# SitaoLuan/ACM-GNN

Measured on AMD Instinct MI355X. Metric: edges/sec ACM-GCN fwd+bwd on twitch-gamer, higher is better.
Workload: dtype f32; 1 GPU; twitch-gamer-shaped Chung-Lu graph: 168114 nodes, 6797557 undirected edges, nnz(A_low)=13763228, F_in=7, hidden=64, classes=2; 2-layer acmgcnp (variant=0, structure_info=0, attention LayerNorm on), dropout 0.1 (counter-based, masks regenerated in the kernels), AdamW (fused); step = fwd + NLL loss + bwd + optimizer update; parallelism=single-gpu, node_order=degree, launch=hipGraph replay of the captured step (1 consecutive steps per graph), operator_form=pattern-only P + row scale (shared by A_low and A_low^T), full=False, input_pipeline=True, checked=False

## Files before the change

acm_gnn_amd/_lib.py:

```python
import ctypes as C
import os
import threading

from . import build as _build

c_f32p = C.POINTER(C.c_float)
c_i32p = C.POINTER(C.c_int32)

ACM_OK = 0
STATUS_NAMES = {1: "ACM_EINVAL", 2: "ACM_ESHAPE", 3: "ACM_EHIP", 4: "ACM_EUNSUPPORTED", 5: "ACM_ENOMEM"}
ABI_VERSION = 28

EXPORTED_SYMBOLS = (
    "acm_version", "acm_last_error", "acm_tuning_get", "acm_tuning_set", "acm_csr_create", "acm_csr_transpose", "acm_csr_slice_rows",
    "acm_csr_destroy", "acm_csr_info", "acm_csr_build_streams", "acm_csr_build_item_streams", "acm_spmm_workspace_bytes", "acm_gemm_workspace_bytes",
    "acm_gemm", "acm_gemm_blocks", "acm_gemm_drop", "acm_proj3", "acm_gemm_split", "acm_proj_fwd", "acm_proj_fwd_at", "acm_proj_bwd_workspace_bytes", "acm_proj_bwd", "acm_spmm", "acm_spmm_v", "acm_spmm_ex", "acm_cast_bf16", "acm_conv_fwd", "acm_conv_bwd_local_workspace_bytes",
    "acm_conv_bwd_local", "acm_conv_bwd_spmm", "acm_conv_agg_fwd", "acm_conv_agg_bwd_workspace_bytes",
    "acm_conv_agg_bwd", "acm_nll_loss_workspace_bytes", "acm_nll_loss", "acm_adam_step", "acm_dropout",
    "acm_reduce_flush", "acm_conv_fwd_tail_workspace_bytes", "acm_conv_fwd_tail", "acm_shard_plan",
    "acm_conv_acmii_fwd_workspace_bytes", "acm_conv_acmii_fwd", "acm_linear_fwd", "acm_bias_act", "acm_bias_act_bwd_workspace_bytes", "acm_bias_act_bwd",
    "acm_acmii_table_bytes", "acm_acmii_table", "acm_conv_acmii_v_fwd", "acm_conv_acmii_v_bwd_workspace_bytes", "acm_conv_acmii_v_bwd",
    "acm_linear_bwd_workspace_bytes", "acm_linear_bwd", "acm_linear_fwd_add", "acm_linear_bwd_recompute",
    "acm_small_step_workspace_bytes", "acm_small_step", "acm_conv_head_fwd", "acm_conv_aggw_fwd", "acm_conv_aggw_bwd_workspace_bytes", "acm_conv_aggw_bwd",
    "acm_eval_metrics_workspace_bytes", "acm_eval_metrics",
)


class Dropout(C.Structure):
    _fields_ = [("p", C.c_float), ("tag", C.c_int32), ("seed", C.c_uint64), ("step", C.c_void_p),
                ("row_offset", C.c_int64), ("step_offset", C.c_int64)]


class CsrInfo(C.Structure):
    _fields_ = [("n_rows", C.c_int64), ("n_cols", C.c_int64), ("nnz", C.c_int64),
                ("n_items", C.c_int64), ("n_long_rows", C.c_int64), ("n_partial_slots", C.c_int64),
                ("chunk", C.c_int32), ("max_degree", C.c_int32),
                ("indptr", C.c_void_p), ("indices", C.c_void_p), ("vals", C.c_void_p),
                ("src_pos", C.c_void_p),
                ("stream_steps", C.c_int64), ("stream_slices", C.c_int64),
                ("stream_waves", C.c_int32), ("stream_long_rows", C.c_int32),
                ("item_stream_waves", C.c_int32), ("reserved", C.c_int32), ("item_stream_batches", C.c_int64)]


class ConvFwd(C.Structure):
    _fields_ = [("f_out", C.c_int32), ("n_channels", C.c_int32), ("relu_after", C.c_int32),
                ("relu_mlp", C.c_int32), ("layernorm", C.c_int32), ("scale", C.c_float),
                ("row_offset", C.c_int64),
                ("g_low", C.c_void_p), ("ld_g_low", C.c_int64),
                ("g_high", C.c_void_p), ("ld_g_high", C.c_int64),
                ("g_struc", C.c_void_p), ("ld_g_struc", C.c_int64),
                ("s_high", C.c_void_p), ("ld_s_high", C.c_int64),
                ("s_mlp", C.c_void_p), ("ld_s_mlp", C.c_int64),
                ("s_struc", C.c_void_p), ("ld_s_struc", C.c_int64),
                ("deg", C.c_void_p),
                ("att_vec", C.c_void_p * 4), ("ln_weight", C.c_void_p * 4), ("ln_bias", C.c_void_p * 4),
                ("att_mix", C.c_void_p),
                ("out", C.c_void_p), ("ld_out", C.c_int64),
                ("pre", C.c_void_p), ("ld_pre", C.c_int64),
                ("att", C.c_void_p), ("post_scale", C.c_void_p), ("ld_post_scale", C.c_int64), ("post_relu", C.c_int32),
                ("gather_bf16", C.c_int32), ("row_scale", C.c_void_p), ("post_drop", Dropout)]


class ConvBwdLocal(C.Structure):
    _fields_ = [("f_out", C.c_int32), ("n_channels", C.c_int32), ("relu_after", C.c_int32),
                ("relu_mlp", C.c_int32), ("layernorm", C.c_int32), ("scale", C.c_float),
                ("grad_out", C.c_void_p), ("ld_grad_out", C.c_int64),
                ("pre", C.c_void_p), ("ld_pre", C.c_int64),
                ("s_mlp", C.c_void_p), ("ld_s_mlp", C.c_int64),
                ("deg", C.c_void_p),
                ("att_vec", C.c_void_p * 4), ("ln_weight", C.c_void_p * 4), ("ln_bias", C.c_void_p * 4),
                ("att_mix", C.c_void_p),
                ("g_low", C.c_void_p), ("ld_g_low", C.c_int64),
                ("g_high", C.c_void_p), ("ld_g_high", C.c_int64),
                ("g_mlp", C.c_void_p), ("ld_g_mlp", C.c_int64),
                ("g_struc", C.c_void_p), ("ld_g_struc", C.c_int64),
                ("d_att_vec", C.c_void_p * 4), ("d_ln_weight", C.c_void_p * 4),
                ("d_ln_bias", C.c_void_p * 4), ("d_att_mix", C.c_void_p),
                ("post_scale", C.c_void_p), ("ld_post_scale", C.c_int64), ("post_relu", C.c_int32),
                ("g_scale", C.c_void_p), ("post_drop", Dropout), ("defer", C.c_void_p)]


class ConvBwdSpmm(C.Structure):
    _fields_ = [("f_out", C.c_int32), ("row_offset", C.c_int64),
                ("g_low", C.c_void_p), ("ld_g_low", C.c_int64),
                ("g_high", C.c_void_p), ("ld_g_high", C.c_int64),
                ("g_struc", C.c_void_p), ("ld_g_struc", C.c_int64),
                ("s_high", C.c_void_p), ("ld_s_high", C.c_int64),
                ("s_struc", C.c_void_p), ("ld_s_struc", C.c_int64),
                ("inv_deg", C.c_void_p),
                ("mask_low", C.c_void_p), ("ld_mask_low", C.c_int64),
                ("mask_high", C.c_void_p), ("ld_mask_high", C.c_int64),
                ("dz_low", C.c_void_p), ("ld_dz_low", C.c_int64),
                ("dz_high", C.c_void_p), ("ld_dz_high", C.c_int64),
                ("d_struc", C.c_void_p), ("ld_d_struc", C.c_int64), ("self_scale", C.c_void_p),
                ("gather_bf16", C.c_int32)]


class ConvAggFwd(C.Structure):
    _fields_ = [("f_in", C.c_int32), ("f_pad", C.c_int32), ("f_out", C.c_int32), ("relu_after", C.c_int32),
                ("relu_mlp", C.c_int32), ("layernorm", C.c_int32), ("scale", C.c_float),
                ("xg", C.c_void_p), ("ld_xg", C.c_int64),
                ("xs", C.c_void_p), ("ld_xs", C.c_int64),
                ("w_low", C.c_void_p), ("w_high", C.c_void_p), ("w_mlp", C.c_void_p), ("ld_w", C.c_int64),
                ("att_vec", C.c_void_p * 4), ("ln_weight", C.c_void_p * 4), ("ln_bias", C.c_void_p * 4),
                ("att_mix", C.c_void_p),
                ("out", C.c_void_p), ("ld_out", C.c_int64),
                ("agg", C.c_void_p), ("ld_agg", C.c_int64),
                ("att", C.c_void_p), ("post_scale", C.c_void_p), ("ld_post_scale", C.c_int64), ("post_relu", C.c_int32),
                ("n_channels", C.c_int32), ("sg", C.c_void_p), ("ld_sg", C.c_int64), ("sg_bf16", C.c_int32),
                ("ss", C.c_void_p), ("ld_ss", C.c_int64), ("deg", C.c_void_p),
                ("ps", C.c_void_p), ("ld_ps", C.c_int64), ("row_scale", C.c_void_p), ("post_drop", Dropout),
                ("head_stats", C.c_void_p), ("ld_head_stats", C.c_int64),
                ("next_w_low", C.c_void_p), ("next_w_high", C.c_void_p), ("next_w_mlp", C.c_void_p), ("next_ld_w", C.c_int64),
                ("next_f", C.c_int32), ("next_relu", C.c_int32),
                ("next_zlh", C.c_void_p), ("ld_next_zlh", C.c_int64), ("next_zi", C.c_void_p), ("ld_next_zi", C.c_int64),
                ("agg_given", C.c_int32), ("reserved0", C.c_int32),
                ("agg_copy", C.c_void_p), ("ld_agg_copy", C.c_int64), ("xs_copy", C.c_void_p), ("ld_xs_copy", C.c_int64),
                ("next_x", C.c_void_p), ("ld_next_x", C.c_int64), ("next_drop", Dropout)]


class ConvAggBwd(C.Structure):
    _fields_ = [("f_in", C.c_int32), ("f_pad", C.c_int32), ("f_out", C.c_int32), ("relu_after", C.c_int32),
                ("relu_mlp", C.c_int32), ("layernorm", C.c_int32), ("scale", C.c_float),
                ("grad_out", C.c_void_p), ("ld_grad_out", C.c_int64),
                ("agg", C.c_void_p), ("ld_agg", C.c_int64),
                ("xs", C.c_void_p), ("ld_xs", C.c_int64),
                ("w_low", C.c_void_p), ("w_high", C.c_void_p), ("w_mlp", C.c_void_p), ("ld_w", C.c_int64),
                ("att_vec", C.c_void_p * 4), ("ln_weight", C.c_void_p * 4), ("ln_bias", C.c_void_p * 4),
                ("att_mix", C.c_void_p),
                ("d_params", C.c_void_p), ("post_scale", C.c_void_p), ("ld_post_scale", C.c_int64), ("post_relu", C.c_int32),
                ("n_channels", C.c_int32), ("ps", C.c_void_p), ("ld_ps", C.c_int64),
                ("ss", C.c_void_p), ("ld_ss", C.c_int64), ("deg", C.c_void_p),
                ("g_struc", C.c_void_p), ("ld_g_struc", C.c_int64), ("g_struc_scale", C.c_void_p),
                ("post_drop", Dropout), ("defer", C.c_void_p),
                ("head_stats", C.c_void_p), ("ld_head_stats", C.c_int64),
                ("out", C.c_void_p), ("ld_out", C.c_int64),
                ("next_a", C.c_void_p), ("next_xg", C.c_void_p), ("ld_next_xg", C.c_int64),
                ("next_row_scale", C.c_void_p), ("next_agg", C.c_void_p), ("ld_next_agg", C.c_int64),
                ("proj_dz", C.c_void_p), ("ld_proj_dz", C.c_int64),
                ("proj_w_low", C.c_void_p), ("proj_w_high", C.c_void_p), ("proj_w_mlp", C.c_void_p), ("proj_ld_w", C.c_int64),
                ("proj_f", C.c_int32), ("proj_d_w", C.c_void_p)]


class ConvAcmiiFwd(C.Structure):
    _fields_ = [("f_in", C.c_int32), ("f_pad", C.c_int32), ("f_out", C.c_int32), ("layernorm", C.c_int32),
                ("scale", C.c_float),
                ("xg", C.c_void_p), ("ld_xg", C.c_int64), ("xs", C.c_void_p), ("ld_xs", C.c_int64),
                ("w_low", C.c_void_p), ("w_high", C.c_void_p), ("w_mlp", C.c_void_p), ("ld_w", C.c_int64),
                ("att_vec", C.c_void_p * 4), ("ln_weight", C.c_void_p * 4), ("ln_bias", C.c_void_p * 4),
                ("att_mix", C.c_void_p),
                ("out", C.c_void_p), ("ld_out", C.c_int64), ("pre", C.c_void_p), ("ld_pre", C.c_int64),
                ("att", C.c_void_p), ("zlh", C.c_void_p), ("ld_zlh", C.c_int64), ("zi", C.c_void_p), ("ld_zi", C.c_int64),
                ("post_scale", C.c_void_p), ("ld_post_scale", C.c_int64), ("post_relu", C.c_int32),
                ("row_scale", C.c_void_p), ("post_drop", Dropout),
                ("n_channels", C.c_int32), ("ps", C.c_void_p), ("ld_ps", C.c_int64), ("ss", C.c_void_p), ("ld_ss", C.c_int64),
                ("deg", C.c_void_p)]


class ConvAcmiiBwd(C.Structure):
    _fields_ = [("f_in", C.c_int32), ("table", C.c_void_p),
                ("g_low", C.c_void_p), ("ld_g_low", C.c_int64), ("g_high", C.c_void_p), ("ld_g_high", C.c_int64),
                ("g_mlp", C.c_void_p), ("ld_g_mlp", C.c_int64), ("x", C.c_void_p), ("ld_x", C.c_int64),
                ("self_offset", C.c_int64), ("row_scale", C.c_void_p),
                ("d_w_low", C.c_void_p), ("d_w_high", C.c_void_p), ("d_w_mlp", C.c_void_p), ("ld_dw", C.c_int64),
                ("defer", C.c_void_p)]


class Loss(C.Structure):
    _fields_ = [("n_classes", C.c_int32), ("labels", C.c_void_p), ("row_weight", C.c_void_p),
                ("loss", C.c_void_p), ("dlogits", C.c_void_p), ("ld_dlogits", C.c_int64)]


class ReduceSeg(C.Structure):
    _fields_ = [("partial", C.c_void_p), ("nblk", C.c_int32), ("row_stride", C.c_int32),
                ("q0", C.c_int32), ("len", C.c_int32), ("dst", C.c_void_p),
                ("inner", C.c_int32), ("col_block", C.c_int32),
                ("outer_stride", C.c_int64), ("block_stride", C.c_int64),
                ("elem_stride", C.c_int32), ("reserved", C.c_int32)]


class ReduceList(C.Structure):
    _fields_ = [("n", C.c_int32), ("cap", C.c_int32), ("segs", C.POINTER(ReduceSeg))]


class SpmmOpts(C.Structure):
    _fields_ = [("vals", C.c_void_p), ("row_scale", C.c_void_p), ("sub", C.c_void_p), ("ld_sub", C.c_int64),
                ("sub_scale", C.c_void_p), ("relu", C.c_int32), ("g_bf16", C.c_int32)]


class AdamTensor(C.Structure):
    _fields_ = [("param", C.c_void_p), ("grad", C.c_void_p), ("exp_avg", C.c_void_p), ("exp_avg_sq", C.c_void_p),
                ("step", C.c_void_p), ("numel", C.c_int64)]


class AdamConfig(C.Structure):
    _fields_ = [("lr", C.c_double), ("beta1", C.c_double), ("beta2", C.c_double), ("eps", C.c_double),
                ("weight_decay", C.c_double), ("decoupled", C.c_int32), ("also_advance", C.c_void_p),
                ("arrive", C.c_void_p), ("pending", C.c_void_p)]


SMALL_ROLES = 17
SR_W_LOW, SR_W_HIGH, SR_W_MLP, SR_V_LOW, SR_V_HIGH, SR_V_MLP, SR_V_STRUC = range(7)
SR_LNW_LOW, SR_LNW_HIGH, SR_LNW_MLP, SR_LNW_STRUC, SR_LNB_LOW, SR_LNB_HIGH, SR_LNB_MLP, SR_LNB_STRUC, SR_MIX, SR_STRUC = range(7, 17)


class SmallStep(C.Structure):
    _fields_ = [("n_classes", C.c_int32), ("n_channels", C.c_int32), ("relu_before", C.c_int32), ("layernorm", C.c_int32),
                ("scale", C.c_float), ("train", C.c_int32), ("update", C.c_int32), ("reserved0", C.c_int32),
                ("t", (AdamTensor * SMALL_ROLES) * 2),
                ("x_vals", C.c_void_p), ("xt_src_pos", C.c_void_p), ("xt_vals", C.c_void_p), ("f_in", C.c_int32), ("reserved1", C.c_int32), ("drop_in", Dropout), ("drop_hidden", Dropout),
                ("row_scale", C.c_void_p), ("labels", C.c_void_p), ("row_weight", C.c_void_p), ("loss", C.c_void_p),
                ("logits", C.c_void_p), ("att1", C.c_void_p), ("att2", C.c_void_p),
                ("lr", C.c_double), ("beta1", C.c_double), ("beta2", C.c_double), ("eps", C.c_double),
                ("weight_decay", C.c_double), ("decoupled", C.c_int32), ("also_advance", C.c_void_p), ("arrive", C.c_void_p),
                ("workspace", C.c_void_p), ("workspace_bytes", C.c_size_t)]


_lib = None
_lock = threading.Lock()


def _declare(lib):
    vp, i64, i32, sz = C.c_void_p, C.c_int64, C.c_int, C.c_size_t
    lib.acm_version.restype = C.c_int
# ... 15 lines not shown
    lib.acm_acmii_table.argtypes = [i64, i32, vp, i64, vp, vp, i64, vp, sz, vp]
    lib.acm_conv_acmii_v_fwd.argtypes = [vp, C.POINTER(ConvAcmiiFwd), vp, vp, sz, vp]
    lib.acm_conv_acmii_v_bwd_workspace_bytes.argtypes = [vp, C.POINTER(sz)]
    lib.acm_conv_acmii_v_bwd.argtypes = [vp, C.POINTER(ConvAcmiiBwd), vp, sz, vp]
    lib.acm_linear_fwd.argtypes = [i64, i64, i64, vp, i64, vp, i64, vp, i32, vp, vp, i64, vp, sz, vp]
    lib.acm_bias_act.argtypes = [i64, i32, vp, i64, vp, i32, vp, vp]
    lib.acm_linear_bwd_workspace_bytes.argtypes = [i64, i32, i32, C.POINTER(sz)]
    lib.acm_linear_bwd.argtypes = [i64, i32, i32, vp, i64, vp, i64, vp, i64, C.c_float, i32, vp, i64, vp, vp, sz, vp, vp]
    lib.acm_linear_fwd_add.argtypes = [i64, i32, i32, vp, i64, vp, i64, vp, i32, vp, vp, i64, vp, i64, vp]
    lib.acm_linear_bwd_recompute.argtypes = [i64, i32, i32, vp, i64, vp, i64, vp, i32, vp, vp, i64, vp, i64, vp, vp, sz, vp, vp]
    lib.acm_bias_act_bwd_workspace_bytes.argtypes = [i64, i32, C.POINTER(sz)]
    lib.acm_bias_act_bwd.argtypes = [i64, i32, vp, i64, vp, i64, C.c_float, i32, vp, i64, vp, vp, sz, vp, vp]
    lib.acm_spmm_workspace_bytes.argtypes = [vp, i32, C.POINTER(sz)]
    lib.acm_gemm_workspace_bytes.argtypes = [i32, i32, i64, i64, i64, C.POINTER(sz)]
    lib.acm_gemm.argtypes = [i32, i32, i64, i64, i64, vp, i64, vp, i64, vp, i64, i32, vp, sz, vp]
    lib.acm_proj_bwd_workspace_bytes.argtypes = [i64, i64, i32, C.POINTER(sz)]
    lib.acm_proj_fwd.argtypes = [i64, i64, i32, vp, i64, vp, vp, vp, i64, i32, vp, i64, vp, i64, vp]
    lib.acm_proj_fwd_at.argtypes = [i64, i64, i32, vp, i64, vp, vp, vp, i64, i32, vp, i64, i64, vp, i64, vp]
    lib.acm_proj_bwd.argtypes = [i64, i64, i32, vp, i64, vp, i64, vp, vp, vp, i64, vp, i64, vp, i64, i64, i64, vp, sz, vp, vp]
    lib.acm_gemm_split.argtypes = [i32, i32, i64, i64, i64, vp, i64, vp, i64, vp, i64, i64, vp, i64, i32, vp, sz, vp]
    lib.acm_gemm_blocks.argtypes = [i32, i32, i64, i64, i64, vp, i64, vp, i64, vp, i64, i64, i64, i32, vp, sz, vp]
    lib.acm_gemm_drop.argtypes = [i32, i32, i64, i64, i64, vp, i64, vp, i64, vp, i64, i64, i64, i32, C.POINTER(Dropout), vp, sz, vp]
    lib.acm_proj3.argtypes = [i64, i64, vp, i64, vp, vp, vp, i64, i64, i64, vp, i64, i64, vp, i64, i32, C.POINTER(Dropout), vp]
    lib.acm_spmm.argtypes = [vp, vp, i64, i32, vp, i64, vp, sz, vp]
    lib.acm_spmm_v.argtypes = [vp, vp, vp, i64, i32, vp, i64, i32, vp, sz, vp]
    lib.acm_adam_step.argtypes = [i32, vp, vp, vp]
    lib.acm_dropout.argtypes = [i64, i64, vp, i64, vp, i64, i64, vp, vp]
    lib.acm_spmm_ex.argtypes = [vp, vp, i64, i32, vp, i64, vp, vp, sz, vp]
    lib.acm_cast_bf16.argtypes = [i64, i64, vp, i64, vp, i64, vp]
    lib.acm_conv_fwd.argtypes = [vp, C.POINTER(ConvFwd), vp, sz, vp]
    lib.acm_conv_head_fwd.argtypes = [i64, C.POINTER(ConvFwd), vp]
    lib.acm_conv_aggw_bwd_workspace_bytes.argtypes = [i64, i64, C.POINTER(C.c_size_t)]
    lib.acm_conv_aggw_bwd.argtypes = [i64, i64, i64, vp, i64, vp, i64, C.POINTER(ConvBwdLocal), vp, vp, vp, i64, vp, C.c_size_t, vp]
    lib.acm_conv_aggw_fwd.argtypes = [i64, i64, i64, vp, i64, vp, i64, vp, vp, vp, i64, vp, i64, C.POINTER(ConvFwd), vp]
    lib.acm_conv_bwd_local_workspace_bytes.argtypes = [i64, i32, i32, C.POINTER(sz)]
    lib.acm_conv_bwd_local.argtypes = [i64, C.POINTER(ConvBwdLocal), vp, sz, vp]
    lib.acm_conv_bwd_spmm.argtypes = [vp, C.POINTER(ConvBwdSpmm), vp, sz, vp]
    lib.acm_conv_agg_fwd.argtypes = [vp, C.POINTER(ConvAggFwd), vp, sz, vp]
    lib.acm_conv_agg_bwd_workspace_bytes.argtypes = [i64, i32, i32, C.POINTER(sz)]
    lib.acm_conv_agg_bwd.argtypes = [i64, C.POINTER(ConvAggBwd), vp, sz, vp]
    lib.acm_nll_loss_workspace_bytes.argtypes = [i64, C.POINTER(sz)]
    lib.acm_nll_loss.argtypes = [i64, i32, vp, i64, vp, vp, vp, vp, i64, vp, sz, vp, vp]
    lib.acm_eval_metrics_workspace_bytes.argtypes = [i64, i32, C.POINTER(sz)]
    lib.acm_eval_metrics.argtypes = [i64, i32, vp, i64, vp, vp, i64, i32, i32, vp, vp, sz, vp]
    lib.acm_reduce_flush.argtypes = [vp, vp]
    lib.acm_conv_fwd_tail_workspace_bytes.argtypes = [i64, i32, i32, C.POINTER(sz)]
    lib.acm_conv_fwd_tail.argtypes = [vp, C.POINTER(ConvFwd), C.POINTER(Loss), C.POINTER(ConvBwdLocal), vp, sz, vp, sz, vp]
    lib.acm_small_step_workspace_bytes.argtypes = [vp, vp, vp, C.POINTER(sz)]
    lib.acm_small_step.argtypes = [vp, vp, vp, C.POINTER(SmallStep), vp]
    for name in EXPORTED_SYMBOLS:
        fn = getattr(lib, name)
        if name not in ("acm_version", "acm_last_error", "acm_csr_destroy"):
            fn.restype = C.c_int


def library_path():
    return os.environ.get("ACM_HIP_LIBRARY", _build.LIB_PATH)


def load(build_if_missing=True):
    global _lib
    with _lock:
        if _lib is not None:
            return _lib
        path = library_path()
        if "ACM_HIP_LIBRARY" not in os.environ and build_if_missing:
            try:
                if _build.is_stale():
                    _build.build_library()
            except Exception as exc:
                if not os.path.exists(path):
                    raise RuntimeError(f"libacm_hip.so is not built and cannot be built here: {exc}")
        if not os.path.exists(path):
            raise RuntimeError(f"libacm_hip.so not found at {path}; run `python -m acm_gnn_amd.build`")
        lib = C.CDLL(path)
        _declare(lib)
        ver = lib.acm_version()
        if ver != ABI_VERSION:
            raise RuntimeError(f"libacm_hip.so ABI version {ver} != expected {ABI_VERSION}")
        _lib = lib
        return _lib


def check(status, what=""):
    if status != ACM_OK:
        msg = load().acm_last_error().decode(errors="replace")
        raise RuntimeError(f"{what or 'libacm_hip'} failed with {STATUS_NAMES.get(status, status)}: {msg}")
```

acm_gnn_amd/csrc/acm_conv_agg.hip:

```cpp
#include "acm_conv_device.h"
#include "acm_stream_device.h"

namespace {

typedef float f32x4 __attribute__((ext_vector_type(4)));
using LG = LayGrouped<4>;

template <int FP>
__device__ __forceinline__ void load_vec(const float* __restrict__ p, float (&v)[FP]) {
#pragma unroll
    for (int q = 0; q < FP / 4; ++q) {
        const float4 t = reinterpret_cast<const float4*>(p)[q];
        v[4 * q + 0] = t.x;
        v[4 * q + 1] = t.y;
        v[4 * q + 2] = t.z;
        v[4 * q + 3] = t.w;
    }
}

template <int FP>
__device__ __forceinline__ void stage_weights(float* wlds, const float* w_low, const float* w_high,
                                              const float* w_mlp, long ld, int f_in, int F) {
    for (int idx = threadIdx.x; idx < 3 * FP * 64; idx += 256) {
        const int c = idx / (FP * 64), f = (idx / 64) % FP, m = (idx % 64) / 4, i = idx % 4;
// ... 478 lines not shown
            for (int i = 0; i < 4; ++i) {
                const int col = m + 16 * i;
                if (col < F) {
                    slab[base + (0 * K + c) * F + col] = dv[c][i];
                    slab[base + (1 * K + c) * F + col] = dgam[c][i];
                    slab[base + (2 * K + c) * F + col] = dbet[c][i];
                }
            }
    }
    if (g == 0 && m < K * K) slab[3 * f_in * F + 3 * K * F + m] = dmix1;
    __syncthreads();
    for (int q = threadIdx.x; q < npg; q += BW * 64) {
        const float v = (lds[q] + lds[npg + q]) + (lds[2 * npg + q] + lds[3 * npg + q]);
        partial[((long)(q >> 5) * gridDim.x + blockIdx.x) * 32 + (q & 31)] = v;
    }
}

template <int FP, int K, bool FULL>
__global__ __launch_bounds__(256, 2) void agg_bwd_kernel(acm_conv_agg_bwd_t p, int n_rows, float* __restrict__ partial) {
    agg_bwd_body<FP, K, FULL>(p, n_rows, partial);
}
int agg_pad(int f_in) { return f_in <= 4 ? 4 : (f_in <= 8 ? 8 : 16); }

int agg_bwd_blocks(int64_t n_rows, int n_channels, size_t lds_bytes) {
    int64_t nb = (n_rows + 15) / 16;
    const int cap = (n_channels == 3 && 3 * lds_bytes <= 160 * 1024) ? 768 : 512;
    if (nb > cap) nb = cap;
    if (nb < 1) nb = 1;
    return (int)nb;
}

template <class P>
int check_common(const P* p, const char* who) {
    ACM_REQUIRE(p->f_in >= 1 && p->f_in <= 16, ACM_EUNSUPPORTED, "%s: f_in %d outside 1..16", who, p->f_in);
    ACM_REQUIRE(p->f_out >= 1 && p->f_out <= 64, ACM_EUNSUPPORTED, "%s: f_out %d outside 1..64", who, p->f_out);
    ACM_REQUIRE(p->f_pad == agg_pad(p->f_in), ACM_ESHAPE, "%s: f_pad %d, expected %d for f_in %d", who, p->f_pad,
                agg_pad(p->f_in), p->f_in);
    ACM_REQUIRE(p->w_low && p->w_high && p->w_mlp && p->att_mix && p->xs, ACM_EINVAL, "%s: NULL pointer", who);
    ACM_REQUIRE(p->ld_w >= p->f_out, ACM_ESHAPE, "%s: ld_w too small", who);
    ACM_REQUIRE(((uintptr_t)p->xs) % 16 == 0 && (p->ld_xs * 4) % 16 == 0 && p->ld_xs >= p->f_pad, ACM_EINVAL,
                "%s: xs rows must be 16-byte aligned and f_pad long", who);
    ACM_REQUIRE(p->n_channels == 3 || p->n_channels == 4, ACM_ESHAPE, "%s: n_channels %d", who, p->n_channels);
    ACM_REQUIRE(!p->head_stats || (((uintptr_t)p->head_stats) % 16 == 0 && p->ld_head_stats % 4 == 0 &&
                                   p->ld_head_stats >= 4 * p->n_channels), ACM_EINVAL,
                "%s: head_stats rows must be 16-byte aligned and 4 * n_channels long", who);
    for (int c = 0; c < p->n_channels; ++c) {
        ACM_REQUIRE(p->att_vec[c], ACM_EINVAL, "%s: att_vec[%d] NULL", who, c);
        ACM_REQUIRE(!p->layernorm || (p->ln_weight[c] && p->ln_bias[c]), ACM_EINVAL, "%s: LayerNorm pointers NULL", who);
    }
    if (p->n_channels == 4)
        ACM_REQUIRE(p->ps && p->ss && p->deg && p->ld_ps >= p->f_out && p->ld_ss >= p->f_out, ACM_EINVAL,
                    "%s: structure-channel pointers NULL / leading dimensions too small", who);
    return ACM_OK;
}

StreamView stream_view(const AcmStreams* t) {
    StreamView sv;
    sv.ids = t->ids;
    sv.waves = t->waves;
    sv.items = t->items;
    sv.long_rows = t->long_rows;
    sv.long_index = t->long_index;
    sv.counters = t->counters;
    sv.slots = t->slots;
    sv.ids_bytes = (unsigned)((t->total_steps + ACM_STREAM_PAD_STEPS) * 512);
    sv.slots_bytes = (unsigned)(t->n_slots * 32);
    sv.n_waves = t->n_waves;
    return sv;
}

}

static int next_projection(const acm_csr_t* a, const acm_conv_agg_fwd_t* p, acm_stream_t stream) {
    if (p->next_f <= 0) return ACM_OK;
    return acm_proj_fwd(a->n_rows, p->f_out, p->next_f, p->out, p->ld_out, p->next_w_low, p->next_w_high, p->next_w_mlp,
                        p->next_ld_w, p->next_relu, p->next_zlh, p->ld_next_zlh, p->next_zi, p->ld_next_zi, stream);
}

extern "C" int acm_conv_agg_fwd(const acm_csr_t* a, const acm_conv_agg_fwd_t* p, void* workspace,
                                size_t workspace_bytes, acm_stream_t stream) {
    ACM_REQUIRE(a && p, ACM_EINVAL, "acm_conv_agg_fwd: NULL argument");
    int st = check_common(p, "acm_conv_agg_fwd");
    if (st != ACM_OK) return st;
    ACM_REQUIRE((p->xg || p->agg_given) && p->out && p->agg && p->att, ACM_EINVAL, "acm_conv_agg_fwd: NULL tensor pointer");
    ACM_REQUIRE((p->agg_given || (((uintptr_t)p->xg) % 16 == 0 && (p->ld_xg * 4) % 16 == 0 && p->ld_xg >= p->f_pad)) &&
                    ((uintptr_t)p->agg) % 16 == 0 && (p->ld_agg * 4) % 16 == 0 && p->ld_agg >= p->f_pad &&
                    ((uintptr_t)p->att) % 16 == 0, ACM_EINVAL,
                "acm_conv_agg_fwd: xg / agg rows must be 16-byte aligned and f_pad long");
    if (p->n_channels == 4) {
        const int64_t ld_max = p->ld_ps > p->ld_ss ? p->ld_ps : p->ld_ss;
        ACM_REQUIRE(a->n_rows * ld_max < (int64_t)INT32_MAX, ACM_EUNSUPPORTED,
                    "acm_conv_agg_fwd: too many rows for 32-bit offsets into ps / ss");
    }
    if (p->next_f != 0) {
        ACM_REQUIRE(p->next_f >= 1 && p->next_f <= 2, ACM_EUNSUPPORTED, "acm_conv_agg_fwd: next_f %d (fused next projection: 1 or 2)", p->next_f);
        ACM_REQUIRE(p->next_w_low && p->next_w_high && p->next_w_mlp && p->next_zlh && p->next_zi && p->next_ld_w >= p->next_f &&
                        p->ld_next_zlh >= 2 * p->next_f && p->ld_next_zi >= p->next_f, ACM_EINVAL,
                    "acm_conv_agg_fwd: fused next projection: NULL pointer / leading dimension too small");
    }
    if (a->n_rows == 0) return ACM_OK;
    hipStream_t s = (hipStream_t)stream;
    bool next_done = false;
    ACM_REQUIRE(!p->agg_copy || (p->agg_given && p->xs_copy && ((uintptr_t)p->agg_copy) % 16 == 0 && ((uintptr_t)p->xs_copy) % 16 == 0 &&
                                 (p->ld_agg_copy * 4) % 16 == 0 && (p->ld_xs_copy * 4) % 16 == 0 && p->ld_agg_copy >= p->f_pad &&
                                 p->ld_xs_copy >= p->f_pad && p->agg_copy != p->agg && p->xs_copy != p->xs), ACM_EINVAL,
                "acm_conv_agg_fwd: agg_copy / xs_copy need agg_given, 16-byte aligned rows of f_pad floats, no aliasing");
    ACM_REQUIRE(!p->next_x || (p->agg_copy && p->ld_next_x >= p->f_in && p->next_drop.p >= 0.f && p->next_drop.p < 1.f &&
                               (p->next_drop.p == 0.f || p->next_drop.step)), ACM_EINVAL,
                "acm_conv_agg_fwd: next_x needs agg_copy / xs_copy (xs is refilled in place), ld_next_x >= f_in and a valid next_drop");
    if (!p->agg_given) {
        const double avg = (double)a->nnz / (double)(a->n_rows > 0 ? a->n_rows : 1);
        const bool fused = acm_tuning().agg_fused != 0 && p->n_channels == 3 && p->f_pad <= 8 && avg > 12.0 && avg <= 160.0 &&
                           ((uintptr_t)p->xg) % 16 == 0 && (p->ld_xg * sizeof(float)) % 16 == 0 &&
                           (a->n_long == 0 || a->long_index != nullptr) &&
                           a->n_multi == 0;
        if (fused) {
            const CsrView cv = acm_view(a);
            int grid = (int)((a->n_items + 15) / 16);
            if (grid > 3072) grid = 3072;
            const bool full = p->f_out == 64;
            if (p->f_pad == 4) {
                if (full) hipLaunchKernelGGL((agg_fused_kernel<4, true>), dim3(grid), dim3(256), 0, s, *p, cv);
                else hipLaunchKernelGGL((agg_fused_kernel<4, false>), dim3(grid), dim3(256), 0, s, *p, cv);
            } else {
                if (full) hipLaunchKernelGGL((agg_fused_pair_kernel<true>), dim3(grid), dim3(256), 0, s, *p, cv);
                else hipLaunchKernelGGL((agg_fused_pair_kernel<false>), dim3(grid), dim3(256), 0, s, *p, cv);
            }
            ACM_CHECK_HIP(hipGetLastError());
            return next_projection(a, p, stream);
        }
    }
    acm_spmm_opts_t o = {nullptr, p->row_scale, nullptr, 0, nullptr, 0, 0};
    const bool epi16 = p->f_out == 64 && (acm_tuning().rows16 & ACM_ROWS16_EPI) != 0;
    bool defer = !p->agg_given && p->n_channels == 3 && a->n_long > 0 && a->long_index != nullptr && !epi16;
    if (!p->agg_given) {
        st = acm_spmm_internal(a, p->xg, p->ld_xg, p->f_pad, p->agg, p->ld_agg, &o, workspace, workspace_bytes, stream, &defer);
        if (st != ACM_OK) return st;
    }
    if (p->n_channels == 4) {
        ACM_REQUIRE(p->sg, ACM_EINVAL, "acm_conv_agg_fwd: sg is NULL");
        o.g_bf16 = p->sg_bf16;
        st = acm_spmm_ex(a, p->sg, p->ld_sg, p->f_out, p->ps, p->ld_ps, &o, workspace, workspace_bytes, stream);
        if (st != ACM_OK) return st;
    }
    if (epi16 && !defer) {
        st = acm_agg_epi16(p, a->n_rows, &next_done, s);
        if (st == ACM_OK) return next_done ? ACM_OK : next_projection(a, p, stream);
        if (st > 0) return st;
    }
    int grid = (int)((a->n_rows + 15) / 16);
    if (grid > 2048) grid = 2048;
    const CsrView cv = acm_view(a);
#define ACM_EPI(FPv)                                                                                           \
    do {                                                                                                       \
        if (p->n_channels == 3)                                                                                \
            hipLaunchKernelGGL((agg_epilogue_kernel<FPv, 3>), dim3(grid), dim3(256), 0, s, *p, (int)a->n_rows, cv, \
                               defer ? (const float*)workspace : nullptr);                                     \
        else                                                                                                   \
            hipLaunchKernelGGL((agg_epilogue_kernel<FPv, 4>), dim3(grid), dim3(256), 0, s, *p, (int)a->n_rows, cv, \
                               (const float*)nullptr);                                                         \
    } while (0)
    if (p->f_pad == 4) ACM_EPI(4);
    else if (p->f_pad == 8) ACM_EPI(8);
    else ACM_EPI(16);
#undef ACM_EPI
    ACM_CHECK_HIP(hipGetLastError());
    if (p->next_x) {
        st = acm_dropout(a->n_rows, p->f_in, p->next_x, p->ld_next_x, const_cast<float*>(p->xs), p->ld_xs, p->f_pad, &p->next_drop, stream);
        if (st != ACM_OK) return st;
    }
    return next_projection(a, p, stream);
}

extern "C" int acm_conv_agg_bwd_workspace_bytes(int64_t n_rows, int f_in, int f_out, size_t* bytes) {
    ACM_REQUIRE(bytes, ACM_EINVAL, "acm_conv_agg_bwd_workspace_bytes: NULL argument");
    ACM_REQUIRE(f_in >= 1 && f_in <= 16 && f_out >= 1 && f_out <= 64, ACM_EUNSUPPORTED,
                "acm_conv_agg_bwd_workspace_bytes: f_in %d f_out %d unsupported", f_in, f_out);
    const size_t npg = ((size_t)3 * f_in * f_out + 12 * (size_t)f_out + 16 + 31) / 32 * 32 + (size_t)6 * f_out;
    *bytes = (size_t)agg_bwd_blocks(n_rows, 3, 0) * npg * sizeof(float);
    return ACM_OK;
}

extern "C" int acm_conv_agg_bwd(int64_t n_rows, const acm_conv_agg_bwd_t* p, void* workspace,
                                size_t workspace_bytes, acm_stream_t stream) {
    ACM_REQUIRE(p, ACM_EINVAL, "acm_conv_agg_bwd: NULL argument");
    int st = check_common(p, "acm_conv_agg_bwd");
    if (st != ACM_OK) return st;
    ACM_REQUIRE((p->grad_out || p->proj_dz) && p->agg && p->d_params, ACM_EINVAL, "acm_conv_agg_bwd: NULL tensor pointer");
    ACM_REQUIRE(p->n_channels == 3 || (p->g_struc && p->ld_g_struc >= p->f_out), ACM_EINVAL,
                "acm_conv_agg_bwd: g_struc is NULL / too narrow");
    {
        int64_t ld_max = 64;
        for (int64_t ld : {p->ld_grad_out, p->ld_agg, p->ld_xs, p->ld_head_stats, p->ld_post_scale, p->ld_ps, p->ld_ss, p->ld_g_struc, p->ld_out})
            ld_max = ld > ld_max ? ld : ld_max;
        ACM_REQUIRE(n_rows * ld_max < (int64_t)INT32_MAX, ACM_EUNSUPPORTED, "acm_conv_agg_bwd: too many rows for 32-bit offsets");
    }
    ACM_REQUIRE(((uintptr_t)p->agg) % 16 == 0 && (p->ld_agg * 4) % 16 == 0 && p->ld_agg >= p->f_pad, ACM_EINVAL,
                "acm_conv_agg_bwd: agg rows must be 16-byte aligned and f_pad long");
    size_t need = 0;
    acm_conv_agg_bwd_workspace_bytes(n_rows, p->f_in, p->f_out, &need);
    ACM_REQUIRE(workspace && workspace_bytes >= need, ACM_ENOMEM, "acm_conv_agg_bwd: workspace %zu B < required %zu B",
                workspace_bytes, need);
    const int K = p->n_channels;
    const int npg = 3 * p->f_in * p->f_out + 3 * K * p->f_out + K * K;
    const size_t lds_w = ((size_t)3 * p->f_pad * 64 + 3 * K * 64 + 32 * p->f_pad) * sizeof(float),
                 lds_s = (size_t)4 * npg * sizeof(float);
    const size_t lds = lds_w > lds_s ? lds_w : lds_s;
    ACM_REQUIRE(lds <= 64 * 1024, ACM_EUNSUPPORTED, "acm_conv_agg_bwd: %zu B of LDS needed", lds);
    int nblk = agg_bwd_blocks(n_rows, p->n_channels, lds);
    hipStream_t s = (hipStream_t)stream;
    float* partial = (float*)workspace;
    if (p->next_agg) {
        const acm_csr_t* na = p->next_a;
        ACM_REQUIRE(na && p->next_xg, ACM_EINVAL, "acm_conv_agg_bwd: next_agg without next_a / next_xg");
        ACM_REQUIRE(p->f_pad == 8 && p->f_out == 64, ACM_EUNSUPPORTED, "acm_conv_agg_bwd: the carried gather needs f_pad 8 and f_out 64");
        const AcmStreams* t = na->streams;
        const int gw = 4;
        ACM_REQUIRE(t && t->n_waves >= gw && t->n_waves % gw == 0 && t->n_waves <= 256 * gw, ACM_EINVAL,
                    "acm_conv_agg_bwd: next_a needs id streams for a multiple of four waves <= 1024 (acm_csr_build_streams)");
        ACM_REQUIRE(na->vals == nullptr && p->ld_next_xg == 8 && ((uintptr_t)p->next_xg) % 16 == 0 &&
                        na->n_cols * 32 < (int64_t)0xFFFFFFE0u && ((uintptr_t)p->next_agg) % 16 == 0 &&
                        (p->ld_next_agg * 4) % 16 == 0 && p->ld_next_agg >= 8, ACM_EINVAL,
                    "acm_conv_agg_bwd: carried gather: pattern-only operator, 32-byte rows of next_xg, 16-byte aligned next_agg");
        ACM_REQUIRE(p->next_agg != p->agg && p->next_xg != p->xs, ACM_EINVAL, "acm_conv_agg_bwd: next_agg / next_xg alias agg / xs");
        GatherRole gr;
        gr.sv = stream_view(t);
        gr.xg = p->next_xg;
        gr.xg_bytes = (unsigned)(na->n_cols * 32);
        gr.row_scale = p->next_row_scale;
        gr.agg = p->next_agg;
        gr.ld_agg = (long)p->ld_next_agg;
        ACM_REQUIRE(t->n_waves / gw <= agg_bwd_blocks(n_rows, 3, 0), ACM_EUNSUPPORTED,
                    "acm_conv_agg_bwd: %d stream waves for %lld rows (the workspace holds one slab per 16 rows)", t->n_waves, (long long)n_rows);
        nblk = t->n_waves / gw;
        {
            const int nb16 = acm_agg_bwd16(p, n_rows, partial, agg_bwd_blocks(n_rows, 3, 0), s, &gr, nblk);
            if (nb16 < 0) return -nb16;
            if (nb16 > 0) {
                const int off2 = (npg + 31) / 32 * 32, n2 = p->proj_dz ? 3 * p->f_out * p->proj_f : 0;
                const acm_reduce_seg_t segs[2] = {{partial, nb16, 32, 0, npg, p->d_params, npg, 0, 0, 0, nb16 * 32, 0},
                                                  {partial, nb16, 32, off2, n2, p->proj_d_w, n2 > 0 ? n2 : 1, 0, 0, 0, nb16 * 32, 0}};
                return acm_reduce_emit(p->defer, segs, n2 > 0 ? 2 : 1, s);
            }
        }
        ACM_REQUIRE(false, ACM_EUNSUPPORTED, "acm_conv_agg_bwd: the carried gather (next_agg) needs the sixteen-rows-per-wave backward "
                    "(head_stats, the forward's `out` behind a fused ReLU or no post-op at all, acm_tuning_t.rows16 bit 2)");
    }
    if (!p->next_agg) {
        const int nb16 = acm_agg_bwd16(p, n_rows, partial, nblk, s, nullptr, 0);
        if (nb16 < 0) return -nb16;
        if (nb16 > 0) {
            const int off2 = (npg + 31) / 32 * 32, n2 = p->proj_dz ? 3 * p->f_out * p->proj_f : 0;
            const acm_reduce_seg_t segs[2] = {{partial, nb16, 32, 0, npg, p->d_params, npg, 0, 0, 0, nb16 * 32, 0},
                                              {partial, nb16, 32, off2, n2, p->proj_d_w, n2 > 0 ? n2 : 1, 0, 0, 0, nb16 * 32, 0}};
            return acm_reduce_emit(p->defer, segs, n2 > 0 ? 2 : 1, s);
        }
    }
    ACM_REQUIRE(!p->proj_dz, ACM_EUNSUPPORTED, "acm_conv_agg_bwd: proj_dz needs the sixteen-rows-per-wave kernel (three channels, "
                "f_pad 8, f_out 64, head_stats, `out`, proj_f <= 2); run acm_proj_bwd and pass grad_out");
#define ACM_BWDK(FPv)                                                                                                  \
    do {                                                                                                              \
        if (K == 3 && p->f_out == 64)                                                                                  \
            hipLaunchKernelGGL((agg_bwd_kernel<FPv, 3, true>), dim3(nblk), dim3(256), lds, s, *p, (int)n_rows, partial); \
        else if (K == 3)                                                                                              \
            hipLaunchKernelGGL((agg_bwd_kernel<FPv, 3, false>), dim3(nblk), dim3(256), lds, s, *p, (int)n_rows, partial); \
        else if (p->f_out == 64)                                                                                      \
            hipLaunchKernelGGL((agg_bwd_kernel<FPv, 4, true>), dim3(nblk), dim3(256), lds, s, *p, (int)n_rows, partial); \
        else                                                                                                          \
            hipLaunchKernelGGL((agg_bwd_kernel<FPv, 4, false>), dim3(nblk), dim3(256), lds, s, *p, (int)n_rows, partial); \
    } while (0)
    if (p->f_pad == 4) ACM_BWDK(4);
    else if (p->f_pad == 8) ACM_BWDK(8);
    else ACM_BWDK(16);
#undef ACM_BWDK
    ACM_CHECK_HIP(hipGetLastError());
    const acm_reduce_seg_t seg = {partial, nblk, 32, 0, npg, p->d_params, npg, 0, 0, 0, nblk * 32, 0};
    return acm_reduce_emit(p->defer, &seg, 1, s);
}
```

acm_gnn_amd/csrc/acm_conv_agg16.hip:

```cpp
#include "acm_conv_device.h"
#include "acm_stream_device.h"
#include "acm_rows16_device.h"

namespace {

#define ACM_E16_NEXT_LDS (64 * 8)


template <int NC, int FP, bool LN, bool NEXT>
__device__ __forceinline__ void epi16_body(const acm_conv_agg_fwd_t& p, int n_rows) {
    constexpr int KB = FP / 4;
    __shared__ __attribute__((aligned(16))) float ulds[NC * 64 + (NEXT ? ACM_E16_NEXT_LDS : 0)];
    const int lane = threadIdx.x & 63, m = lane & 15, g = lane >> 4;
#pragma unroll
    for (int c = 0; c < NC; ++c) {
        if ((threadIdx.x >> 6) == (c & 3)) {
            float u = p.att_vec[c][lane];
            if (LN) u *= p.ln_weight[c][lane];
            ulds[c * 64 + lane] = u;
        }
    }
    if (NEXT) {
        float* nlds = ulds + NC * 64;
        for (int idx = threadIdx.x; idx < ACM_E16_NEXT_LDS; idx += 256) {
            const int col = idx >> 3, j = idx & 7, c = j / p.next_f, q = j % p.next_f;
            const float* w = c == 0 ? p.next_w_low : (c == 1 ? p.next_w_high : p.next_w_mlp);
            nlds[idx] = (c < 3) ? w[(long)col * p.next_ld_w + q] : 0.f;
        }
    }
    float c0[NC];
#pragma unroll
    for (int c = 0; c < NC; ++c) c0[c] = LN ? acm_group_sum<64>(p.ln_bias[c][lane] * p.att_vec[c][lane]) : 0.f;
    float wreg[3][KB][4];
#pragma unroll
    for (int c = 0; c < 3; ++c) {
        const float* w = c == 0 ? p.w_low : (c == 1 ? p.w_high : p.w_mlp);
#pragma unroll
        for (int kb = 0; kb < KB; ++kb)
#pragma unroll
            for (int t = 0; t < 4; ++t)
                wreg[c][kb][t] = (4 * kb + g < p.f_in) ? w[(long)(4 * kb + g) * p.ld_w + 16 * t + m] : 0.f;
    }
    float mixm[NC * NC];
#pragma unroll
    for (int q = 0; q < NC * NC; ++q) mixm[q] = p.att_mix[q];
    __syncthreads();
    const AcmDropCtx dc = acm_drop_ctx(p.post_drop);
    AcmDropCtx ndc = dc;
    if (p.next_x) ndc = acm_drop_ctx(p.next_drop);
    const float lo_a = p.relu_after ? 0.f : -INFINITY, lo_m = p.relu_mlp ? 0.f : -INFINITY;
    const float lo_post = p.post_relu ? 0.f : -INFINITY;
    const unsigned ld_agg = (unsigned)p.ld_agg, ld_xs = (unsigned)p.ld_xs, ld_out = (unsigned)p.ld_out;
    const int wave = blockIdx.x * 4 + (threadIdx.x >> 6), nwaves = gridDim.x * 4;

    int base = wave * 16;
    if (base >= n_rows) return;
    float nP[KB], nx[KB], nr[KB];
    {
        const unsigned rr = (unsigned)min(base + m, n_rows - 1);
#pragma unroll
        for (int kb = 0; kb < KB; ++kb) {
            nP[kb] = p.agg[rr * ld_agg + 4 * kb + g], nx[kb] = p.xs[rr * ld_xs + 4 * kb + g];
            nr[kb] = (p.next_x && 4 * kb + g < p.f_in) ? p.next_x[(long)rr * p.ld_next_x + 4 * kb + g] : 0.f;
        }
    }
    for (; base < n_rows; base += nwaves * 16) {
        const int row = base + m;
        const bool valid = row < n_rows;
        const unsigned rr = (unsigned)(valid ? row : n_rows - 1);
        float P[KB], x[KB], xraw[KB];
#pragma unroll
        for (int kb = 0; kb < KB; ++kb) P[kb] = nP[kb], x[kb] = nx[kb], xraw[kb] = nr[kb];
        f32x4 D[NC][4];
        if (NC == 4) {
            const float dg = p.deg[rr];
#pragma unroll
            for (int t = 0; t < 4; ++t) {
                const f32x4 ps = *reinterpret_cast<const f32x4*>(p.ps + rr * (unsigned)p.ld_ps + 16 * t + 4 * g);
                const f32x4 ss = *reinterpret_cast<const f32x4*>(p.ss + rr * (unsigned)p.ld_ss + 16 * t + 4 * g);
                D[NC - 1][t] = dg * ps - ss;
            }
        }
        {
            const int nb = base + nwaves * 16;
            const unsigned r2 = (unsigned)min(nb + m, n_rows - 1);
#pragma unroll
            for (int kb = 0; kb < KB; ++kb) {
                nP[kb] = p.agg[r2 * ld_agg + 4 * kb + g], nx[kb] = p.xs[r2 * ld_xs + 4 * kb + g];
                nr[kb] = (p.next_x && 4 * kb + g < p.f_in) ? p.next_x[(long)r2 * p.ld_next_x + 4 * kb + g] : 0.f;
            }
        }
        if (p.agg_copy && valid) {
#pragma unroll
// ... 29 lines not shown
                for (int r = 0; r < 4; ++r) D[c][t][r] = fmaxf(D[c][t][r], lo);
            float dot = 0.f;
            if (LN) {
                float s = 0.f;
#pragma unroll
                for (int t = 0; t < 4; ++t) s += (D[c][t][0] + D[c][t][1]) + (D[c][t][2] + D[c][t][3]);
                const float mu = row4_sum(s) * (1.0f / 64.0f);
                float q = 0.f;
#pragma unroll
                for (int t = 0; t < 4; ++t) {
                    const f32x4 u = *reinterpret_cast<const f32x4*>(ulds + c * 64 + 16 * t + 4 * gq);
#pragma unroll
                    for (int r = 0; r < 4; ++r) {
                        const float d = D[c][t][r] - mu;
                        q = fmaf(d, d, q);
                        dot = fmaf(d, u[r], dot);
                    }
                }
                mean[c] = mu;
                rstd[c] = acm_rsqrt(row4_sum(q) * (1.0f / 64.0f) + ACM_LN_EPS);
                dot = fmaf(rstd[c], row4_sum(dot), c0[c]);
            } else {
#pragma unroll
                for (int t = 0; t < 4; ++t) {
                    const f32x4 u = *reinterpret_cast<const f32x4*>(ulds + c * 64 + 16 * t + 4 * gq);
#pragma unroll
                    for (int r = 0; r < 4; ++r) dot = fmaf(D[c][t][r], u[r], dot);
                }
                mean[c] = 0.f;
                rstd[c] = 1.f;
                dot = row4_sum(dot);
            }
            gs[c] = acm_rcp(1.0f + acm_exp(-dot));
        }
        float al[NC];
        {
            float lg[NC], mx = -INFINITY, den = 0.f;
#pragma unroll
            for (int j = 0; j < NC; ++j) {
                float a = 0.f;
#pragma unroll
                for (int c = 0; c < NC; ++c) a = fmaf(gs[c], mixm[c * NC + j], a);
                lg[j] = a * (1.0f / NC);
                mx = fmaxf(mx, lg[j]);
            }
#pragma unroll
            for (int j = 0; j < NC; ++j) {
                lg[j] = acm_exp(lg[j] - mx);
                den += lg[j];
            }
            const float inv = acm_rcp(den);
#pragma unroll
            for (int j = 0; j < NC; ++j) al[j] = lg[j] * inv;
        }
        if (valid) {
            if (p.head_stats && g == 0) {
                float hv[4 * NC];
#pragma unroll
                for (int c = 0; c < NC; ++c) hv[c] = mean[c], hv[NC + c] = rstd[c], hv[2 * NC + c] = gs[c], hv[3 * NC + c] = al[c];
                float* hs = p.head_stats + rr * (unsigned)p.ld_head_stats;
#pragma unroll
                for (int q = 0; q < NC; ++q) reinterpret_cast<float4*>(hs)[q] = make_float4(hv[4 * q], hv[4 * q + 1], hv[4 * q + 2], hv[4 * q + 3]);
            }
            if (g == 1) *reinterpret_cast<float4*>(p.att + (size_t)rr * 4) = make_float4(al[0], al[1], al[2], NC == 4 ? al[NC - 1] : 0.f);
        }
        const float a0 = al[0] * p.scale, a1 = al[1] * p.scale, a2 = al[2] * p.scale, a3 = al[NC - 1] * p.scale;
        float z8[6] = {0.f, 0.f, 0.f, 0.f, 0.f, 0.f};
        f32x4 o[4];
#pragma unroll
        for (int t = 0; t < 4; ++t)
#pragma unroll
            for (int r = 0; r < 4; ++r) {
                float v = fmaf(a2, D[2][t][r], fmaf(a1, D[1][t][r], a0 * D[0][t][r]));
                if (NC == 4) v = fmaf(a3, D[NC - 1][t][r], v);
                o[t][r] = fmaxf(v, lo_post);
            }
        if (p.post_scale) {
#pragma unroll
            for (int t = 0; t < 4; ++t) {
                const f32x4 s = *reinterpret_cast<const f32x4*>(p.post_scale + rr * (unsigned)p.ld_post_scale + 16 * t + 4 * g);
                o[t] *= s;
            }
        }
        if (dc.on) {
#pragma unroll
            for (int r = 0; r < 4; ++r) {
                unsigned w[4];
                acm_philox7(dc, row, 4 * g + r, w);
#pragma unroll
                for (int t = 0; t < 4; ++t) o[t][r] *= (w[t] >= dc.thresh) ? dc.inv_keep : 0.f;
            }
        }
        if (valid) {
#pragma unroll
            for (int t = 0; t < 4; ++t) *reinterpret_cast<f32x4*>(p.out + rr * ld_out + 16 * t + 4 * g) = o[t];
        }
        if (NEXT) {
            const float* nlds = ulds + NC * 64;
#pragma unroll
            for (int t = 0; t < 4; ++t)
#pragma unroll
                for (int r = 0; r < 4; ++r) {
                    const float4 wa = *reinterpret_cast<const float4*>(nlds + (16 * t + 4 * gq + r) * 8);
                    const float2 wb = *reinterpret_cast<const float2*>(nlds + (16 * t + 4 * gq + r) * 8 + 4);
                    z8[0] = fmaf(o[t][r], wa.x, z8[0]); z8[1] = fmaf(o[t][r], wa.y, z8[1]);
                    z8[2] = fmaf(o[t][r], wa.z, z8[2]); z8[3] = fmaf(o[t][r], wa.w, z8[3]);
                    z8[4] = fmaf(o[t][r], wb.x, z8[4]); z8[5] = fmaf(o[t][r], wb.y, z8[5]);
                }
            const int nf = p.next_f;
#pragma unroll
            for (int j = 0; j < 6; ++j) {
                z8[j] = row4_sum(z8[j]);
                if (p.next_relu) z8[j] = fmaxf(z8[j], 0.f);
            }
            if (valid && g == 2) {
#pragma unroll
                for (int j = 0; j < 6; ++j) {
                    if (j < 2 * nf) p.next_zlh[(size_t)rr * p.ld_next_zlh + j] = z8[j];
                    else if (j < 3 * nf) p.next_zi[(size_t)rr * p.ld_next_zi + (j - 2 * nf)] = z8[j];
                }
            }
        }
    }
}

template <int NC, int FP, bool LN, bool NEXT>
__global__ __launch_bounds__(256) void agg_epi16_kernel(acm_conv_agg_fwd_t p, int n_rows) {
    epi16_body<NC, FP, LN, NEXT>(p, n_rows);
}

#define ACM_B16_TS 68

template <int NC, int FP, bool PROJ>
struct B16Lds {
    static constexpr int KB = FP / 4;
    static constexpr int PS = 2 * FP + 1;
    static constexpr int TILES = 4 * 16 * ACM_B16_TS, PX = 4 * 16 * PS + 16 - (4 * 16 * PS) % 16;
    static constexpr int HL = 3 * NC * 64, UL = NC * 64, WL = 3 * KB * 4 * 64, PW = PROJ ? 512 : 0;
    static constexpr int FRONT = TILES + PX + HL + UL + WL + PW;
    static constexpr int NPG0 = 3 * FP * 64 + 3 * NC * 64 + NC * NC;
    static constexpr int SLAB = ((NPG0 + 31) & ~31) + (PROJ ? 6 * 64 : 0);
    static constexpr int TOTAL = (FRONT > 4 * SLAB ? FRONT : 4 * SLAB) + 64;
    static_assert(TOTAL * 4 <= 64 * 1024, "static LDS of one workgroup");
};

template <int NC, int FP, bool LN, bool OUT_MASK, bool PROJ, bool GATHER>
__device__ __forceinline__ void bwd16_body(const acm_conv_agg_bwd_t& p, int n_rows, float* __restrict__ partial, const GatherRole* gr) {
    using L = B16Lds<NC, FP, PROJ>;
    constexpr int KB = L::KB, PS = L::PS;
    __shared__ __attribute__((aligned(16))) float lds[L::TOTAL];
    const int lane = threadIdx.x & 63, m = lane & 15, g = lane >> 4, wv = threadIdx.x >> 6;
    float* gt = lds + wv * (16 * ACM_B16_TS);
    float* px = lds + L::TILES + wv * 16 * PS;
    float* hl = lds + L::TILES + L::PX;
    float* ul = hl + L::HL;
    float* wl = ul + L::UL;
    float* pw = wl + L::WL;
    const int f_in = p.f_in;
    float c1[NC];
#pragma unroll
    for (int c = 0; c < NC; ++c) {
        const float av = p.att_vec[c][lane];
        const float gw = LN ? p.ln_weight[c][lane] : 1.f, gb = LN ? p.ln_bias[c][lane] : 0.f;
        const float u = av * gw;
        if (wv == (c & 3)) {
            hl[c * 64 + lane] = av, hl[NC * 64 + c * 64 + lane] = gw, hl[2 * NC * 64 + c * 64 + lane] = gb;
            ul[c * 64 + lane] = u;
        }
        c1[c] = __builtin_bit_cast(float, __builtin_amdgcn_readfirstlane(__builtin_bit_cast(int, acm_group_sum<64>(u) * (1.0f / 64.0f))));
    }
    for (int idx = threadIdx.x; idx < 3 * KB * 4 * 64; idx += blockDim.x) {
        const int e = idx >> 6, l2 = idx & 63, c = e / (4 * KB), kb = (e >> 2) % KB, t = e & 3, f = 4 * kb + (l2 >> 4);
        const float* w = c == 0 ? p.w_low : (c == 1 ? p.w_high : p.w_mlp);
        wl[idx] = f < f_in ? w[(long)f * p.ld_w + 16 * t + (l2 & 15)] : 0.f;
    }
    const int nq = PROJ ? 3 * p.proj_f : 0;
    if (PROJ) {
        for (int idx = threadIdx.x; idx < 512; idx += blockDim.x) {
            const int col = idx >> 3, j = idx & 7, c = j / p.proj_f, q = j % p.proj_f;
            const float* w = c == 0 ? p.proj_w_low : (c == 1 ? p.proj_w_high : p.proj_w_mlp);
            pw[idx] = (c < 3) ? w[(long)col * p.proj_ld_w + q] : 0.f;
        }
    }
    float mixm[NC * NC];
#pragma unroll
    for (int q = 0; q < NC * NC; ++q) mixm[q] = p.att_mix[q];
    __syncthreads();
    if (GATHER && wv >= 4) {
        stream_gather_role(*gr, __builtin_amdgcn_readfirstlane(blockIdx.x * 4 + (wv - 4)));
        __syncthreads();
        __syncthreads();
        return;
    }
    const float lo_a = p.relu_after ? 0.f : -INFINITY, lo_m = p.relu_mlp ? 0.f : -INFINITY;
    constexpr bool out_mask = OUT_MASK;
    const float post_gain = p.post_drop.p > 0.f ? 1.0f / (1.0f - p.post_drop.p) : 1.f;
    const unsigned ld_agg = (unsigned)p.ld_agg, ld_xs = (unsigned)p.ld_xs, ld_go = (unsigned)p.ld_grad_out,
                   ld_out = (unsigned)p.ld_out, ld_hs = (unsigned)p.ld_head_stats;
    const int wave = blockIdx.x * 4 + wv, nwaves = gridDim.x * 4;
    const float wq = g == 0 ? 1.f : 0.f;
    const float fsel = m < FP ? 1.f : 0.f;

    f32x4 acc[3][4], acc2[4];
#pragma unroll
    for (int t = 0; t < 4; ++t) acc2[t] = (f32x4){0.f, 0.f, 0.f, 0.f};
    const unsigned ld_pz = (unsigned)p.ld_proj_dz;
    constexpr int NDM = NC == 3 ? 9 : NC;
    float pA[NC], pS[NC], dmx[NDM];
#pragma unroll
    for (int c = 0; c < NC; ++c) pS[c] = pA[c] = 0.f;
#pragma unroll
    for (int q = 0; q < NDM; ++q) dmx[q] = 0.f;
#pragma unroll
    for (int c = 0; c < 3; ++c)
#pragma unroll
        for (int t = 0; t < 4; ++t) acc[c][t] = (f32x4){0.f, 0.f, 0.f, 0.f};

    int base = wave * 16;
    float nP[KB], nx[KB];
    f32x4 ngo[4], nou[4], nst[NC];
#define ACM_B16_LOAD(BASE)                                                                              \
    do {                                                                                                \
        const unsigned r2 = (unsigned)min((BASE) + m, n_rows - 1);                                      \
        _Pragma("unroll") for (int kb = 0; kb < KB; ++kb)                                               \
            nP[kb] = p.agg[r2 * ld_agg + 4 * kb + g], nx[kb] = p.xs[r2 * ld_xs + 4 * kb + g];           \
    } while (0)
#pragma unroll
    for (int kb = 0; kb < KB; ++kb) nP[kb] = nx[kb] = 0.f;
    if (base < n_rows) ACM_B16_LOAD(base);
    for (; base < n_rows; base += nwaves * 16) {
        const bool valid = base + m < n_rows;
        float P[KB], x[KB];
#pragma unroll
        for (int kb = 0; kb < KB; ++kb) P[kb] = nP[kb], x[kb] = nx[kb];
        float dzr[6], dza[4];
        const unsigned r1 = (unsigned)min(base + m, n_rows - 1);
        float dgs = 0.f;
        {
#pragma unroll
            for (int t = 0; t < 4; ++t) {
                if (!PROJ) ngo[t] = *reinterpret_cast<const f32x4*>(p.grad_out + r1 * ld_go + 16 * t + 4 * g);
                if (out_mask || PROJ) nou[t] = *reinterpret_cast<const f32x4*>(p.out + r1 * ld_out + 16 * t + 4 * g);
            }
#pragma unroll
            for (int q = 0; q < NC; ++q) nst[q] = *reinterpret_cast<const f32x4*>(p.head_stats + r1 * ld_hs + 4 * q);
            if (NC == 4) dgs = p.deg[r1];
            if (PROJ) {
#pragma unroll
                for (int j = 0; j < 6; ++j) dzr[j] = (j < nq && valid) ? p.proj_dz[r1 * ld_pz + j] : 0.f;
#pragma unroll
                for (int s = 0; s < 4; ++s) {
                    const int rs = base + 4 * g + s;
                    dza[s] = (m < nq && rs < n_rows) ? p.proj_dz[(unsigned)min(rs, n_rows - 1) * ld_pz + min(m, 5)] : 0.f;
                }
            }
        }
        ACM_B16_LOAD(base + nwaves * 16);
        const int gq = acm_opaque(g), mq = acm_opaque(m);
#pragma unroll
        for (int kb = 0; kb < KB; ++kb) px[mq * PS + 4 * kb + gq] = P[kb], px[mq * PS + FP + 4 * kb + gq] = x[kb];
        constexpr bool RECOMP = NC == 4;
        f32x4 D[RECOMP ? 1 : 3][4];
        const int lq = acm_opaque(lane);
#define ACM_B16_PROJECT_C(CH, DST)                                                                                      \
        _Pragma("unroll") for (int kb = 0; kb < KB; ++kb) {                                                             \
            const float opc = (CH) == 0 ? P[kb] : ((CH) == 1 ? x[kb] - P[kb] : x[kb]);                                  \
            _Pragma("unroll") for (int t = 0; t < 4; ++t)                                                               \
                DST[t] = __builtin_amdgcn_mfma_f32_16x16x4f32(wl[(((CH) * KB + kb) * 4 + t) * 64 + lq], opc,            \
                                                              kb == 0 ? (f32x4){0.f, 0.f, 0.f, 0.f} : DST[t], 0, 0, 0); \
        }
        if (!RECOMP) {
#pragma unroll
            for (int kb = 0; kb < KB; ++kb) {
                const float op[3] = {P[kb], x[kb] - P[kb], x[kb]};
#pragma unroll
                for (int c = 0; c < 3; ++c)
#pragma unroll
                    for (int t = 0; t < 4; ++t)
                        D[RECOMP ? 0 : c][t] = __builtin_amdgcn_mfma_f32_16x16x4f32(wl[((c * KB + kb) * 4 + t) * 64 + lq], op[c],
                                                                                kb == 0 ? (f32x4){0.f, 0.f, 0.f, 0.f} : D[RECOMP ? 0 : c][t], 0, 0, 0);
            }
        }
        f32x4 dO[4];
        const float gate = valid ? post_gain : 0.f;
        if (PROJ) {
#pragma unroll
            for (int t = 0; t < 4; ++t) *reinterpret_cast<f32x4*>(gt + mq * ACM_B16_TS + 16 * t + 4 * gq) = nou[t];
#pragma unroll
            for (int s = 0; s < 4; ++s)
#pragma unroll
                for (int t = 0; t < 4; ++t)
                    acc2[t] = __builtin_amdgcn_mfma_f32_16x16x4f32(dza[s], gt[(4 * gq + s) * ACM_B16_TS + 16 * t + mq], acc2[t], 0, 0, 0);
#pragma unroll
            for (int t = 0; t < 4; ++t)
#pragma unroll
                for (int r = 0; r < 4; ++r) {
                    const float4 wa = *reinterpret_cast<const float4*>(pw + (16 * t + 4 * gq + r) * 8);
                    const float2 wb = *reinterpret_cast<const float2*>(pw + (16 * t + 4 * gq + r) * 8 + 4);
                    float v = dzr[0] * wa.x;
                    v = fmaf(dzr[1], wa.y, v), v = fmaf(dzr[2], wa.z, v), v = fmaf(dzr[3], wa.w, v);
                    v = fmaf(dzr[4], wb.x, v), v = fmaf(dzr[5], wb.y, v);
                    dO[t][r] = out_mask ? ((nou[t][r] != 0.f) ? v * gate : 0.f) : v;
                }
        } else {
#pragma unroll
            for (int t = 0; t < 4; ++t)
#pragma unroll
                for (int r = 0; r < 4; ++r)
                    dO[t][r] = out_mask ? ((nou[t][r] != 0.f) ? ngo[t][r] * gate : 0.f) : (valid ? ngo[t][r] : 0.f);
        }
        float mean[NC], rstd[NC], gsig[NC], al[NC];
        {
            float hv[4 * NC];
#pragma unroll
            for (int q = 0; q < NC; ++q)
#pragma unroll
                for (int r = 0; r < 4; ++r) hv[4 * q + r] = nst[q][r];
#pragma unroll
            for (int c = 0; c < NC; ++c) mean[c] = hv[c], rstd[c] = hv[NC + c], gsig[c] = hv[2 * NC + c], al[c] = hv[3 * NC + c];
        }
        float dal[NC], ds[NC];
        if (NC == 4) {
            float part = 0.f;
#pragma unroll
            for (int t = 0; t < 4; ++t) {
                const f32x4 ps = *reinterpret_cast<const f32x4*>(p.ps + r1 * (unsigned)p.ld_ps + 16 * t + 4 * g);
                const f32x4 ss = *reinterpret_cast<const f32x4*>(p.ss + r1 * (unsigned)p.ld_ss + 16 * t + 4 * g);
#pragma unroll
                for (int r = 0; r < 4; ++r) part = fmaf(dO[t][r], fmaxf(fmaf(dgs, ps[r], -ss[r]), 0.f), part);
            }
            dal[NC - 1] = p.scale * row4_sum(part);
        }
#pragma unroll
        for (int c = 0; c < 3; ++c) {
            const float lo = c < 2 ? lo_a : lo_m;
            float part = 0.f;
            if (RECOMP) ACM_B16_PROJECT_C(c, D[0])
#pragma unroll
            for (int t = 0; t < 4; ++t)
#pragma unroll
                for (int r = 0; r < 4; ++r) {
                    D[RECOMP ? 0 : c][t][r] = fmaxf(D[RECOMP ? 0 : c][t][r], lo);
                    part = fmaf(dO[t][r], D[RECOMP ? 0 : c][t][r], part);
                }
            dal[c] = p.scale * row4_sum(part);
        }
        {
            float dot = 0.f;
#pragma unroll
            for (int j = 0; j < NC; ++j) dot = fmaf(al[j], dal[j], dot);
            float dlg[NC];
#pragma unroll
            for (int j = 0; j < NC; ++j) dlg[j] = al[j] * (dal[j] - dot);
#pragma unroll
            for (int c = 0; c < NC; ++c) {
                float dg = 0.f;
#pragma unroll
                for (int j = 0; j < NC; ++j) {
                    dg = fmaf(dlg[j], mixm[c * NC + j], dg);
                    if (NC == 3) dmx[(c * NC + j) % NDM] = fmaf(wq * gsig[c], dlg[j] * (1.0f / NC), dmx[(c * NC + j) % NDM]);
                }
                ds[c] = dg * (1.0f / NC) * gsig[c] * (1.f - gsig[c]);
                pS[c] = fmaf(wq, ds[c], pS[c]);
            }
            if (NC == 4) {
                const float gsel = valid ? (g == 0 ? gsig[0] : (g == 1 ? gsig[1] : (g == 2 ? gsig[2] : gsig[NC - 1]))) : 0.f;
#pragma unroll
                for (int j = 0; j < NC; ++j) dmx[j % NDM] = fmaf(gsel, dlg[j] * (1.0f / NC), dmx[j % NDM]);
// ... 56 lines not shown
                    if (valid) *reinterpret_cast<f32x4*>(p.g_struc + r1 * (unsigned)p.ld_g_struc + 16 * t + 4 * g) = dg1 * G;
                } else {
                    *reinterpret_cast<f32x4*>(gt + mq * ACM_B16_TS + 16 * t + 4 * gq) = G;
                }
            }
#undef ACM_B16_H
            if (c < 3) {
#pragma unroll
                for (int s = 0; s < 4; ++s) {
                    const float ap = px[(4 * gq + s) * PS + (mq & (FP - 1))], ax = px[(4 * gq + s) * PS + FP + (mq & (FP - 1))];
                    const float aop = fsel * (c == 0 ? ap : (c == 1 ? ax - ap : ax));
#pragma unroll
                    for (int t = 0; t < 4; ++t)
                        acc[c < 3 ? c : 0][t] = __builtin_amdgcn_mfma_f32_16x16x4f32(aop, gt[(4 * gq + s) * ACM_B16_TS + 16 * t + mq], acc[c < 3 ? c : 0][t], 0, 0, 0);
                }
            }
        }
    }
#undef ACM_B16_PROJECT_C
#undef ACM_B16_LOAD
    const int npg0 = 3 * f_in * 64 + 3 * NC * 64 + NC * NC;
    const int off2 = (npg0 + 31) & ~31;
    const int npg = PROJ ? off2 + 64 * nq : npg0;
    const int mycol = 16 * (m >> 2) + 4 * g + (m & 3);
    float dv[NC], dgam[NC], dbet[NC];
#pragma unroll
    for (int c = 0; c < NC; ++c) {
        pS[c] = acm_group_sum<64>(pS[c]);
        const float v = hl[c * 64 + mycol], gm = hl[NC * 64 + c * 64 + mycol], bt = hl[2 * NC * 64 + c * 64 + mycol];
        dv[c] = fmaf(gm, pA[c], bt * pS[c]);
        dgam[c] = v * pA[c];
        dbet[c] = v * pS[c];
    }
#pragma unroll
    for (int q = 0; q < NDM; ++q) dmx[q] = NC == 3 ? acm_group_sum<64>(dmx[q]) : acm_group_sum<16>(dmx[q]);
    __syncthreads();
    float* slab = lds + wv * npg;
#pragma unroll
    for (int c = 0; c < 3; ++c)
#pragma unroll
        for (int t = 0; t < 4; ++t)
#pragma unroll
            for (int r = 0; r < 4; ++r) {
                const int f = 4 * g + r;
                if (f < f_in) slab[(c * f_in + f) * 64 + 16 * t + m] = acc[c][t][r];
            }
    {
        const int b2 = 3 * f_in * 64;
#pragma unroll
        for (int c = 0; c < NC; ++c) {
            slab[b2 + (0 * NC + c) * 64 + mycol] = dv[c];
            slab[b2 + (1 * NC + c) * 64 + mycol] = dgam[c];
            slab[b2 + (2 * NC + c) * 64 + mycol] = dbet[c];
        }
    }
    if (NC == 3) {
        if (lane < 9) {
            float v = dmx[0];
#pragma unroll
            for (int q = 1; q < 9; ++q) v = lane == q ? dmx[q % NDM] : v;
            slab[3 * f_in * 64 + 9 * 64 + lane] = v;
        }
    } else if (m == 0) {
#pragma unroll
        for (int j = 0; j < NC; ++j) slab[3 * f_in * 64 + 3 * NC * 64 + g * NC + j] = dmx[j % NDM];
    }
    if (PROJ) {
#pragma unroll
        for (int t = 0; t < 4; ++t)
#pragma unroll
            for (int r = 0; r < 4; ++r) {
                const int j = 4 * g + r, col = 16 * t + m;
                if (j < nq) slab[off2 + (j / p.proj_f) * 64 * p.proj_f + col * p.proj_f + j % p.proj_f] = acc2[t][r];
            }
    }
    __syncthreads();
    for (int q = threadIdx.x; q < npg; q += 256) {
        float v = (lds[q] + lds[npg + q]) + (lds[2 * npg + q] + lds[3 * npg + q]);
        if (PROJ && q >= npg0 && q < off2) v = 0.f;
        partial[((long)(q >> 5) * gridDim.x + blockIdx.x) * 32 + (q & 31)] = v;
    }
}

template <int NC, int FP, bool LN, bool OUT_MASK, bool PROJ>
__global__ __launch_bounds__(256) __attribute__((amdgpu_waves_per_eu(2, 2))) void agg_bwd16_kernel(acm_conv_agg_bwd_t p, int n_rows, float* __restrict__ partial) {
    bwd16_body<NC, FP, LN, OUT_MASK, PROJ, false>(p, n_rows, partial, nullptr);
}
template <int NC, bool LN, bool PROJ>
__global__ __launch_bounds__(512) __attribute__((amdgpu_waves_per_eu(2, 2))) void agg_bwd16_gather_kernel(acm_conv_agg_bwd_t p, int n_rows, float* __restrict__ partial,
                                                                                                   GatherRole gr) {
    bwd16_body<NC, 8, LN, true, PROJ, true>(p, n_rows, partial, &gr);
}

}

int acm_agg_epi16(const acm_conv_agg_fwd_t* p, int64_t n_rows, bool* next_done, hipStream_t s) {
    *next_done = false;
    const int NC = p->n_channels, FP = p->f_pad;
    if ((NC != 3 && NC != 4) || (FP != 4 && FP != 8 && FP != 16) || p->f_out != 64 || !(acm_tuning().rows16 & ACM_ROWS16_EPI)) return -1;
    int64_t ld_max = 64;
    for (int64_t ld : {p->ld_agg, p->ld_xs, p->ld_out, p->ld_head_stats, p->ld_post_scale, p->ld_agg_copy, p->ld_xs_copy, p->ld_ps, p->ld_ss})
        ld_max = ld > ld_max ? ld : ld_max;
    if (n_rows * ld_max >= (int64_t)INT32_MAX) return -1;
    if ((((uintptr_t)p->out) % 16) != 0 || (p->ld_out % 4) != 0) return -1;
    if (p->post_scale && ((((uintptr_t)p->post_scale) % 16) != 0 || (p->ld_post_scale % 4) != 0)) return -1;
    if (NC == 4 && ((((uintptr_t)p->ps) % 16) != 0 || (((uintptr_t)p->ss) % 16) != 0 || p->ld_ps % 4 != 0 || p->ld_ss % 4 != 0)) return -1;
    const bool next = p->next_f > 0;
    int grid = (int)((n_rows + 63) / 64);
    if (grid > 1024) grid = 1024;
#define ACM_E16_L(NCv, FPv)                                                                                                   \
    do {                                                                                                                     \
        if (p->layernorm) {                                                                                                  \
            if (next) hipLaunchKernelGGL((agg_epi16_kernel<NCv, FPv, true, true>), dim3(grid), dim3(256), 0, s, *p, (int)n_rows);   \
            else hipLaunchKernelGGL((agg_epi16_kernel<NCv, FPv, true, false>), dim3(grid), dim3(256), 0, s, *p, (int)n_rows);       \
        } else {                                                                                                             \
            if (next) hipLaunchKernelGGL((agg_epi16_kernel<NCv, FPv, false, true>), dim3(grid), dim3(256), 0, s, *p, (int)n_rows);  \
            else hipLaunchKernelGGL((agg_epi16_kernel<NCv, FPv, false, false>), dim3(grid), dim3(256), 0, s, *p, (int)n_rows);      \
        }                                                                                                                    \
    } while (0)
#define ACM_E16(NCv)                            \
    do {                                        \
        if (FP == 4) ACM_E16_L(NCv, 4);         \
        else if (FP == 8) ACM_E16_L(NCv, 8);    \
        else ACM_E16_L(NCv, 16);                \
    } while (0)
    if (NC == 3) ACM_E16(3);
    else ACM_E16(4);
#undef ACM_E16
#undef ACM_E16_L
    ACM_CHECK_HIP(hipGetLastError());
    *next_done = next;
    return ACM_OK;
}

int acm_agg_bwd16(const acm_conv_agg_bwd_t* p, int64_t n_rows, float* partial, int max_blocks, hipStream_t s, const GatherRole* gr,
                  int gather_blocks) {
    const int NC = p->n_channels, FP = p->f_pad;
    if ((NC != 3 && NC != 4) || (FP != 4 && FP != 8 && FP != 16) || p->f_out != 64 || !p->head_stats ||
        !(acm_tuning().rows16 & ACM_ROWS16_BWD))
        return 0;
    const bool out_mask = p->out != nullptr && p->post_relu && !p->post_scale;
    const bool no_post = !p->post_relu && !p->post_scale && !(p->post_drop.p > 0.f);
    if (!out_mask && !no_post) return 0;
    const bool proj = p->proj_dz != nullptr;
    if ((proj || gr) && (FP != 8 || !out_mask)) return 0;
    if (proj && (!p->out || p->proj_f < 1 || p->proj_f > 2 || !p->proj_w_low || !p->proj_w_high || !p->proj_w_mlp || !p->proj_d_w ||
                 p->ld_proj_dz < 3 * p->proj_f || p->proj_ld_w < p->proj_f || n_rows * p->ld_proj_dz >= (int64_t)INT32_MAX))
        return 0;
    for (const void* q : {(const void*)(proj ? nullptr : p->grad_out), (const void*)p->out, (const void*)p->head_stats,
                          (const void*)(NC == 4 ? p->ps : nullptr), (const void*)(NC == 4 ? p->ss : nullptr),
                          (const void*)(NC == 4 ? p->g_struc : nullptr)})
        if (((uintptr_t)q) % 16 != 0) return 0;
    if ((!proj && p->ld_grad_out % 4 != 0) || ((out_mask || proj) && p->ld_out % 4 != 0) || p->ld_head_stats % 4 != 0) return 0;
    if (NC == 4 && (p->ld_ps % 4 != 0 || p->ld_ss % 4 != 0 || p->ld_g_struc % 4 != 0 || !p->deg)) return 0;
    acm_conv_agg_bwd_t q = *p;
    if (!out_mask && !proj) q.out = nullptr;
    int grid = (int)((n_rows + 63) / 64);
    int cap = 512;
    if (cap > max_blocks) cap = max_blocks;
    if (grid > cap) grid = cap;
    if (gr) {
        if (gather_blocks < 1 || gather_blocks > max_blocks) return 0;
        grid = gather_blocks;
    }
    const bool ln = p->layernorm != 0;
#define ACM_B16_BASE(NCv, FPv)                                                                                                     \
    do {                                                                                                                          \
        if (ln) {                                                                                                                 \
            if (out_mask) hipLaunchKernelGGL((agg_bwd16_kernel<NCv, FPv, true, true, false>), dim3(grid), dim3(256), 0, s, q, (int)n_rows, partial);   \
            else hipLaunchKernelGGL((agg_bwd16_kernel<NCv, FPv, true, false, false>), dim3(grid), dim3(256), 0, s, q, (int)n_rows, partial);           \
        } else {                                                                                                                  \
            if (out_mask) hipLaunchKernelGGL((agg_bwd16_kernel<NCv, FPv, false, true, false>), dim3(grid), dim3(256), 0, s, q, (int)n_rows, partial);  \
            else hipLaunchKernelGGL((agg_bwd16_kernel<NCv, FPv, false, false, false>), dim3(grid), dim3(256), 0, s, q, (int)n_rows, partial);          \
        }                                                                                                                         \
    } while (0)
#define ACM_B16_CARRY(NCv)                                                                                                          \
    do {                                                                                                                          \
        if (gr) {                                                                                                                 \
            if (ln) { if (proj) hipLaunchKernelGGL((agg_bwd16_gather_kernel<NCv, true, true>), dim3(grid), dim3(512), 0, s, q, (int)n_rows, partial, *gr);   \
                      else hipLaunchKernelGGL((agg_bwd16_gather_kernel<NCv, true, false>), dim3(grid), dim3(512), 0, s, q, (int)n_rows, partial, *gr); }       \
            else { if (proj) hipLaunchKernelGGL((agg_bwd16_gather_kernel<NCv, false, true>), dim3(grid), dim3(512), 0, s, q, (int)n_rows, partial, *gr);     \
                   else hipLaunchKernelGGL((agg_bwd16_gather_kernel<NCv, false, false>), dim3(grid), dim3(512), 0, s, q, (int)n_rows, partial, *gr); }         \
        } else {                                                                                                                  \
            if (ln) hipLaunchKernelGGL((agg_bwd16_kernel<NCv, 8, true, true, true>), dim3(grid), dim3(256), 0, s, q, (int)n_rows, partial);                   \
            else hipLaunchKernelGGL((agg_bwd16_kernel<NCv, 8, false, true, true>), dim3(grid), dim3(256), 0, s, q, (int)n_rows, partial);                     \
        }                                                                                                                         \
    } while (0)
    if (proj || gr) {
        if (NC == 3) ACM_B16_CARRY(3);
        else ACM_B16_CARRY(4);
    } else if (NC == 3) {
        if (FP == 4) ACM_B16_BASE(3, 4);
        else if (FP == 8) ACM_B16_BASE(3, 8);
        else ACM_B16_BASE(3, 16);
    } else {
        if (FP == 4) ACM_B16_BASE(4, 4);
        else if (FP == 8) ACM_B16_BASE(4, 8);
        else ACM_B16_BASE(4, 16);
    }
#undef ACM_B16_BASE
#undef ACM_B16_CARRY
    if (hipGetLastError() != hipSuccess) return -ACM_EHIP;
    return grid;
}
```

acm_gnn_amd/csrc/acm_csr.cpp:

```cpp
#include <stdarg.h>
#include <stdio.h>
#include <string.h>

#include <stdlib.h>

#include <algorithm>
#include <functional>
#include <new>
#include <queue>
#include <string>
#include <utility>
#include <vector>

#include "acm_common.h"

static thread_local char g_err[512] = "";

void acm_set_error(const char* fmt, ...) {
    va_list ap;
    va_start(ap, fmt);
    vsnprintf(g_err, sizeof(g_err), fmt, ap);
    va_end(ap);
}

extern "C" int acm_version(void) { return ACM_ABI_VERSION; }
extern "C" const char* acm_last_error(void) { return g_err; }

namespace {
const acm_tuning_t kTuningDefaults = {0, 0, -1, 7, 1, 7, {0}};
struct TuningField { const char* name; int32_t acm_tuning_t::*field; };
const TuningField kTuningFields[] = {{"chunk", &acm_tuning_t::chunk},           {"wide_form", &acm_tuning_t::wide_form},
                                     {"bwd_split", &acm_tuning_t::bwd_split},   {"rows16", &acm_tuning_t::rows16},
                                     {"agg_fused", &acm_tuning_t::agg_fused},   {"gemm_forms", &acm_tuning_t::gemm_forms}};
const char* const kHostKeys[] = {"rewrites", "implicit", "relabel", "pipeline", "csr_features", "small_step"};

const char* tuning_invalid(const acm_tuning_t& t) {
    if (t.chunk != 0 && (t.chunk < 8 || t.chunk > 4096 || (t.chunk & (t.chunk - 1)))) return "chunk";
    if (t.wide_form < 0 || t.wide_form > 3) return "wide_form";
    if (t.bwd_split < -1 || t.bwd_split > 1) return "bwd_split";
    if (t.rows16 < 0 || t.rows16 > 7) return "rows16";
    if (t.agg_fused < 0 || t.agg_fused > 1) return "agg_fused";
    if (t.gemm_forms < 0 || t.gemm_forms > 15) return "gemm_forms";
    return nullptr;
}

acm_tuning_t tuning_from_environment() {
    acm_tuning_t t = kTuningDefaults;
    const char* env = getenv("ACM_TUNING");
    if (!env) return t;
    std::string text(env);
    size_t pos = 0;
    while (pos < text.size()) {
        size_t end = text.find(',', pos);
        if (end == std::string::npos) end = text.size();
        const std::string item = text.substr(pos, end - pos);
        pos = end + 1;
        if (item.empty()) continue;
        const size_t eq = item.find('=');
        const std::string key = item.substr(0, eq), val = eq == std::string::npos ? "" : item.substr(eq + 1);
        bool known = false;
        for (const char* h : kHostKeys) known = known || key == h;
        for (const TuningField& f : kTuningFields) {
            if (key != f.name) continue;
            known = true;
            char* stop = nullptr;
            const long v = strtol(val.c_str(), &stop, 0);
            acm_tuning_t probe = t;
            probe.*(f.field) = (int32_t)v;
            if (val.empty() || *stop || tuning_invalid(probe)) fprintf(stderr, "libacm_hip: ACM_TUNING: bad value '%s' ignored\n", item.c_str());
            else t = probe;
        }
        if (!known) fprintf(stderr, "libacm_hip: ACM_TUNING: unknown key '%s' ignored\n", key.c_str());
    }
    return t;
}
const acm_tuning_t g_tuning_loaded = tuning_from_environment();
acm_tuning_t g_tuning = g_tuning_loaded;
}

const acm_tuning_t& acm_tuning() { return g_tuning; }

extern "C" int acm_tuning_get(acm_tuning_t* out) {
    ACM_REQUIRE(out, ACM_EINVAL, "acm_tuning_get: NULL argument");
    *out = g_tuning;
    return ACM_OK;
}

extern "C" int acm_tuning_set(const acm_tuning_t* in) {
    if (!in) {
        g_tuning = g_tuning_loaded;
        return ACM_OK;
    }
    const char* bad = tuning_invalid(*in);
    ACM_REQUIRE(!bad, ACM_EINVAL, "acm_tuning_set: field '%s' out of range", bad);
    g_tuning = *in;
    for (int32_t& r : g_tuning.reserved) r = 0;
    return ACM_OK;
}

namespace {

void free_streams(AcmStreams* t) {
    if (!t) return;
    for (void* q : {(void*)t->ids, (void*)t->waves, (void*)t->items, (void*)t->long_rows,
                    (void*)t->long_index, (void*)t->counters, (void*)t->slots})
        if (q) (void)hipFree(q);
    delete t;
}
// ... 571 lines not shown
```

acm_gnn_amd/functional/__init__.py:

```python
from .. import _lib, tuning
from ..graph import CsrGraph, FilterOperators, SparseFeatures, _device_ctx, _require_cuda, _stream
from ._launch import KernelTimer, _Timed, set_kernel_timer
from ._context import (CallContext, DeferredReductions, InputPipeline, Tape, TapeBroken, _ambient,
                       deferred_reductions, deferred_reductions_as, fused_loss_tail, input_pipeline, on_tape)
from .ops import (DropoutState, _drop_spec, agg_pad_width, cast_bf16, dropout, eval_metrics, eval_metrics_buffers,
                  gemm, gemm_drop_supported, gemm_split, masked_nll, mm, nll_loss_and_grad, proj3, proj_bwd,
                  proj_bwd_supported, proj_fwd, spmm, spmm_v)
from .linear import residual_add_linear, residual_add_supported, residual_linear
from ._conv_shared import AcmConfig, _flat_views, _gather_rows, _ptr_array
from .conv_agg import AGG_WIDE_MIN_DEGREE, _AcmAggWide, agg_wide_supported
from .conv_literal import _AcmAcmii
from .conv import _conv_route, acm_conv, in_drop_supported
```

acm_gnn_amd/functional/_context.py:

```python
import bisect
import ctypes as C
import threading

import torch

from .. import _lib, tuning
from ._launch import _F32, _Timed, _vp, launch


class DeferredReductions:
    CAP = 96

    def __init__(self):
        self._segs = (_lib.ReduceSeg * self.CAP)()
        self._list = _lib.ReduceList(0, self.CAP, C.cast(self._segs, C.POINTER(_lib.ReduceSeg)))
        self._keep = []
        self.outputs = []
        self._allreduce = []

    def pointer(self):
        return C.addressof(self._list)

    def hold(self, workspace, outputs, keep=None):
        self._keep.append(workspace)
        self._keep.extend(outputs if keep is None else keep)
        self.outputs.extend((t.data_ptr(), t.numel() * t.element_size()) for t in outputs if t is not None)

    @property
    def pending(self):
        return int(self._list.n)

    def all_adopted(self, tensors):
        ptrs = sorted(t.data_ptr() for t in tensors if t is not None)
        for a, nb in self.outputs:
            i = bisect.bisect_left(ptrs, a)
            if i == len(ptrs) or ptrs[i] >= a + nb:
                return False
        return True

    def allreduce(self, tensor, group):
        self._allreduce.append((tensor, group))

    def flush(self):
        if self._list.n:
            launch("acm_reduce_flush", "reduce_flush", self._keep[0].device, C.byref(self._list))
        if self._allreduce:
            import torch.distributed as dist
            pending, self._allreduce = self._allreduce, []
            group = pending[0][1]
            coalesce = (len(pending) > 1 and all(g is group for _, g in pending) and hasattr(dist, "_coalescing_manager")
                        and dist.get_backend(group) == "nccl")
            with _Timed("all_reduce/gradients", sum(t.numel() * t.element_size() for t, _ in pending)):
                if coalesce:
                    with dist._coalescing_manager(group=group, device=pending[0][0].device, async_ops=False):
                        for t, _ in pending:
                            dist.all_reduce(t, group=group)
                else:
                    for t, g in pending:
                        dist.all_reduce(t, group=g)
        self._keep.clear()

    @property
    def collectives_pending(self):
        return bool(self._allreduce)

    def flushed(self):
        assert self._list.n == 0 and not self._allreduce
        self._keep.clear()

    def discard(self):
        self._list.n = 0
        self._keep.clear()
        self._allreduce = []


def _sum_over_ranks(flat, group, defer):
    if defer is not None:
        defer.allreduce(flat, group)
    else:
        import torch.distributed as dist
        dist.all_reduce(flat, group=group)


class CallContext:
    __slots__ = ("defer", "tail", "pipe", "next_proj", "pre_proj", "hidden_private")

    def __init__(self, defer=None, tail=None, pipe=None):
        self.defer, self.tail, self.pipe = defer, tail, pipe
        self.next_proj = self.pre_proj = None
        self.hidden_private = None

    @classmethod
    def from_ambient(cls):
        a = _ambient()
        return cls(a.defer, a.tail, a.pipe)

    def defer_ptr(self):
        return self.defer.pointer() if self.defer is not None else None


_TLS = threading.local()


def _ambient():
    c = getattr(_TLS, "call", None)
    if c is None:
        c = _TLS.call = CallContext()
    return c


def _call_or_ambient(call):
    return call if call is not None else CallContext.from_ambient()


class TapeBroken(RuntimeError):
    """A step cannot run on a Tape (see there): something other than this package's Functions sits between them."""


class _TapeCtx:

    def __init__(self, needs_input_grad):
        self.needs_input_grad = needs_input_grad
        self.saved_tensors = ()
        self.non_differentiable = ()

    def save_for_backward(self, *tensors):
        self.saved_tensors = tensors

    def mark_non_differentiable(self, *tensors):
        self.non_differentiable = tuple(id(t) for t in tensors)

    def release(self):
        self.__dict__.clear()
        self.saved_tensors = ()

    def set_materialize_grads(self, value):
        pass


class Tape:

    def __init__(self):
        self.records = []
        self.produced = {}
        self.ctx_of = {}

    def run(self, fn, args):
        needs = []
        for a in args:
            if not isinstance(a, torch.Tensor):
                needs.append(False)
            elif id(a) in self.produced:
                needs.append(True)
            elif a.grad_fn is not None:
                raise TapeBroken(f"{fn.__name__}: an argument was computed by torch operations from tensors that need gradients")
            else:
                needs.append(bool(a.requires_grad))
        ctx = _TapeCtx(tuple(needs))
        with torch.no_grad():
            out = fn.forward(ctx, *args)
        outs = out if isinstance(out, tuple) else (out,)
        if not any(needs):
            return out
        for o in outs:
            if isinstance(o, torch.Tensor) and o.is_floating_point() and id(o) not in ctx.non_differentiable:
                o.requires_grad_(True)
                self.ctx_of[id(o)] = ctx
                self.produced[id(o)] = o
        self.records.append((fn, ctx, args, outs))
        return out

    def producer(self, t):
        return self.ctx_of.get(id(t)) if self.produced.get(id(t)) is t else None
# ... 162 lines not shown
                return False
        gcns = getattr(model, "gcns", None)
        if not gcns or len(gcns) != 2 or not getattr(model, "fused_dropout", False) or getattr(model, "dropout", 0) <= 0:
            return False
        l0 = gcns[0]
        try:
            cfg = l0._config()
            f_in, f = l0.weight_low.shape
        except AttributeError:
            return False
        if cfg.relu_before or f != 64 or not 4 < f_in <= 8 or x.dim() != 2 or x.shape[1] != f_in:
            return False
        if not ops.implicit or getattr(ops, "general", False) or int(getattr(ops, "hops", 1)) != 1:
            return False
        if ops.sharded:
            xf = ops.x_full
            if (not ops.uniform or xf is None or xf.dtype != _F32 or xf.dim() != 2 or xf.shape != (ops.low.n_cols, f_in)
                    or xf.device != x.device or xf.requires_grad):
                return False
        if x.dtype != _F32 or x.device != l0.weight_low.device or x.requires_grad:
            return False
        n, nnz = ops.low.n_rows, ops.low.nnz
        min_rows = tuning.HOST.pipeline
        if n != x.shape[0] or n < max(min_rows, 32) or not 12.0 * n < nnz <= 160.0 * n:
            return False
        if x.device.type == "cuda" and torch.cuda.is_current_stream_capturing():
            return False
        gw = 4
        if not ops.low.build_streams(n_waves=max(gw, min(256 * gw, gw * ((n + 15) // 16)))):
            return False
        return ops.low.stream_waves % gw == 0 and gw <= ops.low.stream_waves <= min(256 * gw, gw * ((n + 15) // 16))

    def table(self):
        return self.filled[0]

    def local_table(self):
        return self.filled[0][self.row_offset:self.row_offset + self.x_rows.shape[0]]

    def agg(self):
        return self.filled[1]

    def _drop_into(self, dst, step_offset):
        d = self.state.spec(self.p, self.tag, 0)
        d.step_offset = int(step_offset)
        n, c = self.x.shape
        launch("acm_dropout", f"dropout/{n}x{c}", self.x.device, n, c, _vp(self.x), self.x.stride(0), _vp(dst), dst.stride(0), 8, C.byref(d))

    def stale(self):
        return (not self.primed or (self.x._version, self.x_rows._version) != self._x_version or self.next_table_ready
                or self.state.host_steps != self._host_steps)

    def prime(self):
        from .ops import spmm
        self._drop_into(self.filled[0], 0)
        spmm(self.ops.low, self.filled[0], out=self.filled[1], row_scale=self.ops.row_scale)
        self.primed = True
        self._x_version = (self.x._version, self.x_rows._version)
        self._host_steps = self.state.host_steps
        self.next_table_ready = self.next_agg_ready = self.adopted = False

    def refill_spec(self, p):
        if self.filled[0].shape[0] != self.x_rows.shape[0] or self.next_table_ready or self.x.stride(1) != 1:
            return False
        d = self.state.spec(self.p, self.tag, 0)
        d.step_offset = 1
        p.next_x, p.ld_next_x, p.next_drop = self.x.data_ptr(), self.x.stride(0), d
        return True

    def make_next(self):
        if not self.adopted:
            return False
        if not self.next_table_ready:
            self._drop_into(self.filled[0], 1)
            self.next_table_ready = True
        return True

    def end_step(self):
        if not (self.next_table_ready and self.next_agg_ready):
            self.primed = False
        self.next_table_ready = self.next_agg_ready = self.adopted = False
        self._host_steps = self.state.host_steps


def _next_proj_request(call, f, dev, row_local_only=False):
    nxt, call.next_proj = call.next_proj, None
    if nxt is None or not row_local_only or not (tuning.kernel()["rows16"] & tuning.ROWS16_EPI):
        return None
    try:
        w3 = (nxt.weight_low, nxt.weight_high, nxt.weight_mlp)
        cfg = nxt._config()
    except AttributeError:
        return None
    f2 = w3[0].shape[1]
    ok = (f2 <= 2 and all(w.dtype == _F32 and w.is_contiguous() and w.device == dev and
                                                   tuple(w.shape) == (f, f2) for w in w3))
    return (w3, bool(cfg.relu_before), f2, cfg.n_channels == 4 and f2 == 2) if ok else None


def _take_pre_proj(call, x, w3, relu):
    pre, call.pre_proj = call.pre_proj, None
    if pre is None or not isinstance(x, torch.Tensor):
        return None
    out, zlh, zi, ptrs, prelu = pre
    if (x.data_ptr() == out.data_ptr() and x.shape == out.shape and x.stride() == out.stride() and prelu == bool(relu)
            and tuple(w.data_ptr() for w in w3) == ptrs):
        return zlh, zi
    return None
```

acm_gnn_amd/functional/_conv_shared.py:

```python
import ctypes as C

import torch

from .. import _lib
from .. import functional as _pkg
from ..graph import SparseFeatures
from ._context import _call_or_ambient, _sum_over_ranks
from ._launch import _F32, _Timed, _as_f32c, _vp, launch
from .ops import _drop_now, _drop_spec, cast_bf16, spmm


class AcmConfig:

    __slots__ = ("n_channels", "relu_before", "relu_after", "relu_mlp", "layernorm", "scale", "gather_bf16")

    def __init__(self, model_type, variant, structure_info, attn_layernorm, gather_dtype="fp32"):
        if gather_dtype not in ("fp32", "bf16"):
            raise ValueError("gather_dtype must be 'fp32' or 'bf16'")
        self.gather_bf16 = gather_dtype == "bf16"
        plus = model_type in ("acmgcnp", "acmgcnpp", "acmgcn+", "acmgcn++")
        if model_type == "acmsgc":
            self.n_channels, self.relu_before, self.relu_after, self.relu_mlp = 3, False, False, False
            self.layernorm = False
        elif model_type == "acmsnowball":
            self.n_channels = 3
            self.relu_before, self.relu_after, self.relu_mlp = bool(variant), not bool(variant), True
            self.layernorm = False
        else:
            self.n_channels = 4 if (plus and structure_info) else 3
            self.relu_before = bool(variant)
            self.relu_after = not bool(variant)
            self.relu_mlp = True
            self.layernorm = bool(attn_layernorm) and plus
        self.scale = 1.0 if self.n_channels == 4 else 3.0


def _ptr_array(tensors):
    n = len(tensors)
    return _VP4(*[tensors[i].data_ptr() if i < n and tensors[i] is not None else None for i in range(4)])


_VP4 = C.c_void_p * 4


def _gather_rows(ops, local):
    if not ops.sharded:
        return local
    import torch.distributed as dist
    world = dist.get_world_size(ops.group)
    n_max = ops.n_gathered // world
    local = local.contiguous()
    if local.shape[0] != n_max:
        buf = local.new_zeros(n_max, local.shape[1])
        buf[: local.shape[0]] = local
        local = buf
    full = torch.empty(world * n_max, local.shape[1], dtype=local.dtype, device=local.device)
    with _Timed(f"all_gather/{n_max}x{local.shape[1]}", local.numel() * local.element_size()):
        dist.all_gather_into_tensor(full, local, group=ops.group)
    return full


def _hop_buffer(t_like, width):
    pitch = width if width > 8 else (8 if width > 4 else (4 if width > 2 else width))
    return torch.empty(t_like.shape[0], pitch, dtype=_F32, device=t_like.device)[:, :width]


def _low_product(ops, t_local, transpose=False, out=None):
    if out is None:
        out = _hop_buffer(t_local, t_local.shape[1])
    if transpose:
        if ops.implicit:
            scaled = _hop_buffer(t_local, t_local.shape[1])
            torch.mul(t_local, ops.row_scale[:, None], out=scaled)
            return spmm(ops.low_t, _pkg._gather_rows(ops, scaled), out=out)
        return spmm(ops.low_t, _pkg._gather_rows(ops, t_local), out=out)
    return spmm(ops.low, _pkg._gather_rows(ops, t_local), out=out, row_scale=ops.row_scale if ops.implicit else None)


def _flat_views(flat, nw, k, f, layernorm):
    if layernorm:
        parts = flat[nw:].split([f] * (3 * k) + [k * k])
        d_vec = [t.view(f, 1) for t in parts[:k]]
        d_lnw, d_lnb = list(parts[k:2 * k]), list(parts[2 * k:3 * k])
    else:
        parts = flat[nw:].split([f] * k + [k * k])
        d_vec, d_lnw, d_lnb = [t.view(f, 1) for t in parts[:k]], [], []
    d_mix = parts[-1].view(k, k)
    return d_vec, d_lnw, d_lnb, d_mix


# ... 42 lines not shown
def _pack_head(vecs, lnw, lnb, mix):
    return (mix, *vecs, *lnw, *lnb)


def _unpack_head(saved, cfg, at):
    k = cfg.n_channels
    nln = k if cfg.layernorm else 0
    v, w, b = at + 1, at + 1 + k, at + 1 + k + nln
    return list(saved[v:w]), list(saved[w:b]), list(saved[b:b + nln]), saved[at]


def _reduce_replicated(flat, ops, defer):
    if ops.sharded:
        _sum_over_ranks(flat, ops.group, defer)


def _struc_grad(ops, cfg, gs):
    n, f = gs.shape
    gsg = _pkg._gather_rows(ops, gs)
    low_t = ops.low_t
    d_struc = torch.empty(n, f, dtype=_F32, device=gs.device)
    ws = low_t.workspace(f)
    o = _lib.SpmmOpts()
    o.sub, o.ld_sub = gs.data_ptr(), gs.stride(0)
    o.sub_scale = None if ops.implicit else ops.inv_deg.data_ptr()
    if cfg.gather_bf16 and 8 < f <= 64 and f % 2 == 0:
        gsg = cast_bf16(gsg)
        o.g_bf16 = 1
    launch("acm_spmm_ex", f"spmm_sub/{f}", gs.device, low_t.handle, _vp(gsg), gsg.stride(0), f, _vp(d_struc), d_struc.stride(0), C.byref(o),
           _vp(ws), ws.numel() * 4)
    return d_struc


_NONE4 = (None,) * 4
_NO_GRADS = (None,) * 28


def _grads(d_x, d_w3, d_vec, d_struc, d_mix, d_lnw, d_lnb):
    pad = (None,) * (4 - len(d_vec))
    return (d_x, *d_w3, *d_vec, *pad, d_struc, d_mix, *((*d_lnw, *pad) if d_lnw else _NONE4),
            *((*d_lnb, *pad) if d_lnb else _NONE4), *_NO_GRADS[:10])


def _k3_setup(cfg, ops, k, f, n, dev, f_in_w, pre, zi, vecs, lnw, lnb, mix, grad_out, post_relu, post_scale, post_drop,
              fb=None):
    four = k == 4
    fb = f if fb is None else fb
    g, gs = _narrow_tables(n, fb, f, dev, packed=four and f == 2 and fb == 2)
    dz = torch.empty(n, 3 * f, dtype=_F32, device=dev)
    if four and gs is None:
        gs = torch.empty(n, f, dtype=_F32, device=dev)
    nw, nln = 3 * f_in_w * f, (k * f if cfg.layernorm else 0)
    flat = torch.empty(nw + k * f + 2 * nln + k * k, dtype=_F32, device=dev)
    d_vec, d_lnw, d_lnb, d_mix = _flat_views(flat, nw, k, f, cfg.layernorm)

    q = _lib.ConvBwdLocal()
    q.f_out = f
    _set_head(q, cfg, vecs, lnw, lnb, mix)
    q.grad_out, q.ld_grad_out = grad_out.data_ptr(), grad_out.stride(0)
    q.pre, q.ld_pre = pre.data_ptr(), pre.stride(0)
    q.s_mlp, q.ld_s_mlp = zi.data_ptr(), zi.stride(0)
    general = bool(getattr(ops, "general", False))
    ones = ops.zeros(n, 1).new_ones(n) if (four and general) else None
    q.deg = None if (not four or ops.implicit) else (ones if general else ops.deg).data_ptr()
    if ops.implicit:
        q.g_scale = ops.row_scale.data_ptr()
    q.g_low, q.ld_g_low = g.data_ptr(), g.stride(0)
    q.g_high, q.ld_g_high = g.data_ptr() + 4 * fb, g.stride(0)
    q.g_mlp, q.ld_g_mlp = dz.data_ptr() + 8 * f, dz.stride(0)
    if four:
        q.g_struc, q.ld_g_struc = gs.data_ptr(), gs.stride(0)
    q.d_att_vec, q.d_ln_weight, q.d_ln_bias = _ptr_array(d_vec), _ptr_array(d_lnw), _ptr_array(d_lnb)
    q.d_att_mix = d_mix.data_ptr()
    _set_post(q, post_relu, post_scale, post_drop, ops.row_offset)
    return dict(q=q, g=g, dz=dz, gs=gs, flat=flat, nw=nw, d_vec=d_vec, d_lnw=d_lnw, d_lnb=d_lnb, d_mix=d_mix,
                general=general, ones=ones, grad_out=grad_out)


def _conv_prologue(ctx, x, w_low, ops, post_relu, post_scale, post_drop, call, in_drop):
    ctx.set_materialize_grads(False)
    ctx.call = _call_or_ambient(call)
    ctx.in_drop = in_drop if (in_drop is not None and in_drop[0] > 0) else None
    sparse_x = isinstance(x, SparseFeatures)
    if not sparse_x:
        x = _as_f32c(x, "input")
    n, f = x.shape[0], w_low.shape[1]
    if post_scale is not None:
        post_scale = _as_f32c(post_scale, "post_scale")
        if tuple(post_scale.shape) != (n, f):
            raise ValueError(f"post_scale must be [{n}, {f}]")
    ctx.post_relu, ctx.post_scale = bool(post_relu), post_scale
    ctx.post_drop = post_drop if (post_drop is not None and post_drop[0] > 0) else None
    if n != ops.n_local:
        raise ValueError(f"input has {n} rows but the graph operator has {ops.n_local}")
    ctx.x_width = x.shape[1]
    if x.shape[1] != w_low.shape[0] and (sparse_x or x.shape[1] < w_low.shape[0]):
        raise ValueError(f"input has {x.shape[1]} columns but the weights have {w_low.shape[0]} rows")
    return x


def _gathered_input(ctx, x, ops, f_in, f, fp, agg_holder, pregathered, agg_first):
    n, call = x.shape[0], ctx.call
    if ctx.in_drop is not None:
        x = _drop_now(x, _drop_spec(ctx.in_drop, ops.row_offset))
    if agg_holder is not None and (ops.sharded or call.pipe is not None or not agg_first or ctx.in_drop is not None):
        agg_holder = None
    if x.shape[1] == fp:
        xpad = x
    else:
        xpad = agg_holder.get("xpad") if agg_holder is not None else None
        if xpad is None or tuple(xpad.shape) != (n, fp):
            xpad = torch.nn.functional.pad(x[:, :f_in], (0, fp - f_in))
            if agg_holder is not None:
                agg_holder["xpad"] = xpad
    agg_given = agg_holder.get("agg") if agg_holder is not None else None
    if agg_given is not None and tuple(agg_given.shape) != (n, fp):
        agg_given = None
    pipe = call.pipe
    ctx.pipe = None
    if (pipe is not None and pipe.primed and agg_first and fp == 8 and f == 64 and ops is pipe.ops
            and xpad.data_ptr() == pipe.local_table().data_ptr() and agg_holder is None):
        agg_given = pipe.agg()
        ctx.pipe = pipe
        pipe.adopted = True
    if agg_given is not None:
        xg = xpad
    elif (pregathered is not None and pregathered[0].data_ptr() == xpad.data_ptr()
            and pregathered[1].shape[1] == fp and pregathered[1].shape[0] == ops.n_gathered):
        xg = pregathered[1]
    else:
        xg = _pkg._gather_rows(ops, xpad)
    return x, xpad, xg, agg_given, agg_holder


def _struc_rows(ops, struc_low, n):
    if ops.deg is None:
        raise RuntimeError("structure_info=1 needs adj_low_unnormalized")
    s_local = _as_f32c(struc_low, "struc_low")
    if s_local.shape[0] != n:
        raise ValueError("struc_low rows != local nodes")
    return s_local, _pkg._gather_rows(ops, s_local)
```

acm_gnn_amd/functional/conv_agg.py:

```python
import ctypes as C

import torch

from .. import _lib, tuning
from .. import functional as _pkg
from ._context import _call_or_ambient, _next_proj_request
from ._conv_shared import _NO_GRADS, _conv_prologue, _flat_views, _gathered_input, _grads, _head_params, _k3_setup, \
    _narrow_tables, _pack_head, _reduce_replicated, _set_head, _set_post, _struc_grad, _struc_rows, _unpack_head
from ._launch import EUNSUPPORTED, _F32, _as_f32c, _vp, _workspace, launch
from .ops import _drop_spec, cast_bf16, gemm, proj_bwd, spmm


class _AcmAggFirst(torch.autograd.Function):

    @staticmethod
    def forward(ctx, x, w_low, w_high, w_mlp, v_low, v_high, v_mlp, v_struc, struc_low, att_mix, lnw_low, lnw_high, lnw_mlp,
                lnw_struc, lnb_low, lnb_high, lnb_mlp, lnb_struc, ops, cfg, post_relu, post_scale, post_drop, call, tail_layer,
                agg_holder, in_drop, pregathered):
        x = _conv_prologue(ctx, x, w_low, ops, post_relu, post_scale, post_drop, call, in_drop)
        call = ctx.call
        ctx.agg_first = True
        dev, n = x.device, x.shape[0]
        f_in, f = w_low.shape
        k = cfg.n_channels
        four = k == 4
        fp = 4 if f_in <= 4 else (8 if f_in <= 8 else 16)
        x, xpad, xg, agg_given, agg_holder = _gathered_input(ctx, x, ops, f_in, f, fp, agg_holder, pregathered, True)
        wl, wh, wm = (_as_f32c(t, "weight") for t in (w_low, w_high, w_mlp))
        if four:
            s_local, s_gath = _struc_rows(ops, struc_low, n)
        vecs, lnw, lnb, mix = _head_params(cfg, (v_low, v_high, v_mlp, v_struc), att_mix, (lnw_low, lnw_high, lnw_mlp, lnw_struc),
                                           (lnb_low, lnb_high, lnb_mlp, lnb_struc))
        out = torch.empty(n, f, dtype=_F32, device=dev)
        att = torch.empty(n, 4, dtype=_F32, device=dev)
        p = _lib.ConvAggFwd()
        p.f_in, p.f_pad, p.f_out = f_in, fp, f
        _set_head(p, cfg, vecs, lnw, lnb, mix)
        p.xg, p.ld_xg = xg.data_ptr(), xg.stride(0)
        p.xs, p.ld_xs = xpad.data_ptr(), xpad.stride(0)
        p.w_low, p.w_high, p.w_mlp, p.ld_w = wl.data_ptr(), wh.data_ptr(), wm.data_ptr(), f
        agg = agg_given if agg_given is not None else torch.empty(n, fp, dtype=_F32, device=dev)
        p.agg_given = int(agg_given is not None)
        refill = False
        if ctx.pipe is not None:
            p.agg_copy, p.ld_agg_copy = ctx.pipe.saved[1].data_ptr(), ctx.pipe.saved[1].stride(0)
            p.xs_copy, p.ld_xs_copy = ctx.pipe.saved[0].data_ptr(), ctx.pipe.saved[0].stride(0)
            refill = ctx.pipe.refill_spec(p)
        p.out, p.ld_out = out.data_ptr(), out.stride(0)
        p.agg, p.ld_agg = agg.data_ptr(), agg.stride(0)
        p.att = att.data_ptr()
        if ops.implicit:
            p.row_scale = ops.row_scale.data_ptr()
        extra = ()
        if four:
            ps = torch.empty(n, f, dtype=_F32, device=dev)
            if cfg.gather_bf16 and f % 2 == 0 and f > 8:
                sgt = cast_bf16(s_gath)
                p.sg_bf16 = 1
            else:
                sgt = s_gath
            p.sg, p.ld_sg = sgt.data_ptr(), sgt.stride(0)
            p.ss, p.ld_ss = s_local.data_ptr(), s_local.stride(0)
            p.deg = ops.deg.data_ptr()
            p.ps, p.ld_ps = ps.data_ptr(), ps.stride(0)
            extra = (ps, s_local)
        _set_post(p, ctx.post_relu, ctx.post_scale, ctx.post_drop, ops.row_offset)
        stats = torch.empty(n, 4 * k, dtype=_F32, device=dev) if any(ctx.needs_input_grad) else None
        if stats is not None:
            p.head_stats, p.ld_head_stats = stats.data_ptr(), stats.stride(0)
        ctx.head_stats = stats
        nxt = _next_proj_request(call, f, dev, row_local_only=f == 64 and (agg_given is not None or four))
        if nxt is not None:
            n_w3, n_relu, f2, n_pack = nxt
            n_zlh, _ = _narrow_tables(n, f2, f2, dev, n_pack)
            n_zi = torch.empty(n, f2, dtype=_F32, device=dev)
            p.next_w_low, p.next_w_high, p.next_w_mlp = (w.data_ptr() for w in n_w3)
            p.next_ld_w, p.next_f, p.next_relu = n_w3[0].stride(0), f2, int(n_relu)
            p.next_zlh, p.ld_next_zlh = n_zlh.data_ptr(), n_zlh.stride(0)
            p.next_zi, p.ld_next_zi = n_zi.data_ptr(), n_zi.stride(0)
        ws = ops.low.workspace(max(fp, f) if four else fp)
        launch("acm_conv_agg_fwd", f"conv_agg_{'epi' if agg_given is not None else 'fwd'}/F{f}k{k}i{f_in}", dev, ops.low.handle, C.byref(p),
               _vp(ws), ws.numel() * 4)
        if refill:
            ctx.pipe.next_table_ready = True
        if agg_holder is not None and agg_given is None:
            agg_holder["agg"] = agg
        if nxt is not None:
            call.pre_proj = (out, n_zlh, n_zi, tuple(w.data_ptr() for w in n_w3), n_relu)
        ctx.ops, ctx.cfg, ctx.f_in = ops, cfg, f_in
        ctx.out_mask = bool(ctx.post_relu) and ctx.post_scale is None
        if ctx.pipe is not None:
            xpad, agg = ctx.pipe.saved[0], ctx.pipe.saved[1]
        ctx.save_for_backward(xpad, agg, wl, wh, wm, *_pack_head(vecs, lnw, lnb, mix), *extra, *((out,) if ctx.out_mask else ()))
        ctx.mark_non_differentiable(att)
        return out, att

    @staticmethod
    def backward(ctx, grad_out, _grad_att):
        if grad_out is None:
            return _NO_GRADS
        ops, cfg, f_in = ctx.ops, ctx.cfg, ctx.f_in
        k = cfg.n_channels
        four = k == 4
        saved = ctx.saved_tensors
        out_fwd = None
        if ctx.out_mask:
            out_fwd, saved = saved[-1], saved[:-1]
        xpad, agg, wl, wh, wm = saved[:5]
        vecs, lnw, lnb, mix = _unpack_head(saved, cfg, 5)
        dev = xpad.device
        n, f, fp = xpad.shape[0], wl.shape[1], xpad.shape[1]
        lazy, ctx.lazy = getattr(ctx, "lazy", None), None
        if lazy is not None and (grad_out is not lazy["placeholder"] and grad_out.data_ptr() != lazy["placeholder"].data_ptr()):
            raise RuntimeError("acm_conv: the hidden activation marked private (CallContext.hidden_private) received a gradient "
                               "from somewhere else as well")
        fuse_proj = (lazy is not None and fp == 8 and f == 64 and out_fwd is not None and ctx.post_scale is None
                     and ctx.head_stats is not None)
        defer = ctx.call.defer
        if lazy is not None and not fuse_proj:
            proj_bwd(lazy["x"], lazy["dz"], lazy["w3"], lazy["d_w"], defer=defer, dx_out=lazy["placeholder"])
            lazy = None
        grad_out = _as_f32c(grad_out, "grad_out")
        nw = 3 * f_in * f
        d_params = torch.empty(nw + 3 * k * f + k * k, dtype=_F32, device=dev)
        q = _lib.ConvAggBwd()
        q.f_in, q.f_pad, q.f_out = f_in, fp, f
        _set_head(q, cfg, vecs, lnw, lnb, mix)
        q.grad_out, q.ld_grad_out = grad_out.data_ptr(), grad_out.stride(0)
        if lazy is not None:
            dz2, w32 = lazy["dz"], lazy["w3"]
            q.grad_out = None
            q.proj_dz, q.ld_proj_dz = dz2.data_ptr(), dz2.stride(0)
            q.proj_w_low, q.proj_w_high, q.proj_w_mlp = (w.data_ptr() for w in w32)
            q.proj_ld_w, q.proj_f = w32[0].stride(0), w32[0].shape[1]
            q.proj_d_w = lazy["d_w"].data_ptr()
        q.agg, q.ld_agg = agg.data_ptr(), agg.stride(0)
        if ctx.head_stats is not None:
            q.head_stats, q.ld_head_stats = ctx.head_stats.data_ptr(), ctx.head_stats.stride(0)
        q.xs, q.ld_xs = xpad.data_ptr(), xpad.stride(0)
        q.w_low, q.w_high, q.w_mlp, q.ld_w = wl.data_ptr(), wh.data_ptr(), wm.data_ptr(), f
        q.d_params = d_params.data_ptr()
        _set_post(q, ctx.post_relu, ctx.post_scale, ctx.post_drop, ops.row_offset)
        if out_fwd is not None:
            q.out, q.ld_out = out_fwd.data_ptr(), out_fwd.stride(0)
        if four:
            ps, s_local = saved[-2], saved[-1]
            gs = torch.empty(n, f, dtype=_F32, device=dev)
            q.ps, q.ld_ps = ps.data_ptr(), ps.stride(0)
            q.ss, q.ld_ss = s_local.data_ptr(), s_local.stride(0)
            q.deg = ops.deg.data_ptr()
            q.g_struc, q.ld_g_struc = gs.data_ptr(), gs.stride(0)
            q.g_struc_scale = None if ops.implicit else ops.deg.data_ptr()
        ws = _workspace(dev, "acm_conv_agg_bwd_workspace_bytes", n, f_in, f)
        q.defer = defer.pointer() if defer is not None else None
        pipe = ctx.pipe
        carry = pipe is not None and pipe.next_table_ready and not pipe.next_agg_ready
        if carry:
            q.next_a = ops.low.handle
            q.next_xg, q.ld_next_xg = pipe.table().data_ptr(), pipe.table().stride(0)
            q.next_row_scale = ops.row_scale.data_ptr()
            q.next_agg, q.ld_next_agg = pipe.agg().data_ptr(), pipe.agg().stride(0)
        st = launch("acm_conv_agg_bwd", f"conv_agg_bwd{'+gather' if carry else ''}{'+proj' if lazy is not None else ''}/F{f}k{k}i{f_in}", dev, n,
                    C.byref(q), _vp(ws), ws.numel() * 4, unsupported_ok=lazy is not None or carry)
        if st == EUNSUPPORTED:
            if lazy is not None:
                proj_bwd(lazy["x"], lazy["dz"], lazy["w3"], lazy["d_w"], defer=defer, dx_out=lazy["placeholder"])
                q.grad_out, q.proj_dz, lazy = grad_out.data_ptr(), None, None
            if carry:
                q.next_a, q.next_xg, q.next_row_scale, q.next_agg = None, None, None, None
                spmm(ops.low, pipe.table(), out=pipe.agg(), row_scale=ops.row_scale)
            launch("acm_conv_agg_bwd", f"conv_agg_bwd/F{f}k{k}i{f_in}", dev, n, C.byref(q), _vp(ws), ws.numel() * 4)
        if carry:
            pipe.next_agg_ready = True
        if defer is not None:
            defer.hold(ws, [d_params] + ([lazy["d_w"]] if lazy is not None else []),
                       keep=[d_params] + ([lazy["d_w"]._base if lazy["d_w"]._base is not None else lazy["d_w"]] if lazy is not None else []))
        d_struc = _struc_grad(ops, cfg, gs) if four else None
        _reduce_replicated(d_params, ops, defer)
        d_w = d_params[:nw].view(3, f_in, f)
        d_vec, d_lnw, d_lnb, d_mix = _flat_views(d_params, nw, k, f, True)
        if not cfg.layernorm:
            d_lnw = d_lnb = []
        return _grads(None, (d_w[0], d_w[1], d_w[2]), d_vec, d_struc, d_mix, d_lnw, d_lnb)


AGG_WIDE_MIN_DEGREE = 12


def agg_wide_supported(x, ops, cfg, f_in, f_out, post_scale=None, call=None, tail_layer=False):
    from ..graph import FilterOperators
    if not (tuning.HOST.rewrites & tuning.REWRITE_AGG_FIRST) or not isinstance(ops, FilterOperators):
        return False
    if not isinstance(x, torch.Tensor) or x.layout != torch.strided or x.dim() != 2 or x.dtype != _F32 or x.requires_grad:
        return False
    if cfg.relu_before or cfg.n_channels != 3 or f_out != 64 or not 16 < f_in <= 128 or x.shape[1] != f_in:
        return False
    if getattr(ops, "general", False) or int(getattr(ops, "hops", 1)) != 1 or x.shape[0] != ops.n_local:
        return False
    if tail_layer:
        return False
    if ops.sharded:
        import torch.distributed as dist
        return ops.n_gathered // dist.get_world_size(ops.group) >= 8192
    if x.shape[0] < 8192:
        return False
    return ops.low.nnz >= AGG_WIDE_MIN_DEGREE * x.shape[0]


class _AcmAggWide(torch.autograd.Function):

    @staticmethod
    def forward(ctx, x, w_low, w_high, w_mlp, v_low, v_high, v_mlp, v_struc, struc_low, att_mix, lnw_low, lnw_high, lnw_mlp,
                lnw_struc, lnb_low, lnb_high, lnb_mlp, lnb_struc, ops, cfg, post_relu, post_scale, post_drop, call, tail_layer,
                agg_holder, in_drop, pregathered):
        ctx.set_materialize_grads(False)
        call = ctx.call = _call_or_ambient(call)
        call.next_proj = None
        x = _as_f32c(x, "input")
        dev = x.device
        n, f_in = x.shape
        f, k = w_low.shape[1], 3
        fp = -(-f_in // 4) * 4
        spec = _drop_spec(in_drop, ops.row_offset) if (in_drop is not None and in_drop[0] > 0) else None
        if spec is not None or ops.sharded:
            agg_holder = None
        agg = None
        if spec is not None:
            xd = torch.empty(n, fp, dtype=_F32, device=dev)
            launch("acm_dropout", f"dropout/{n}x{f_in}", dev, n, f_in, _vp(x), x.stride(0), _vp(xd), xd.stride(0), fp, C.byref(spec))
        elif fp == f_in:
            xd = x
        else:
            xd = agg_holder.get("xpad") if agg_holder is not None else None
            if xd is None or tuple(xd.shape) != (n, fp):
                xd = torch.nn.functional.pad(x, (0, fp - f_in))
                if agg_holder is not None:
                    agg_holder["xpad"], agg_holder["agg"] = xd, None
        if agg_holder is not None:
            agg = agg_holder.get("agg")
            if agg is not None and tuple(agg.shape) != (n, fp):
                agg = None
        if agg is None:
            agg = spmm(ops.low, _pkg._gather_rows(ops, xd), row_scale=ops.row_scale if ops.implicit else None)
            if agg_holder is not None:
                agg_holder["agg"] = agg
        w3 = [_as_f32c(w, "weight") for w in (w_low, w_high, w_mlp)]
        vecs, lnw, lnb, mix = _head_params(cfg, (v_low, v_high, v_mlp), att_mix, (lnw_low, lnw_high, lnw_mlp),
                                           (lnb_low, lnb_high, lnb_mlp))
        if post_scale is not None:
            post_scale = _as_f32c(post_scale, "post_scale")
# ... 83 lines not shown
```

acm_gnn_amd/functional/conv_literal.py:

```python
import ctypes as C

import torch

from .. import _lib, tuning
from .. import functional as _pkg
from ..graph import SparseFeatures
from ._context import _current_tape, _take_pre_proj
from ._conv_shared import _NO_GRADS, _chan_block, _conv_prologue, _flat_views, _gathered_input, _grads, _head_params, _hop_buffer, \
    _k3_setup, _low_product, _narrow_tables, _pack_head, _reduce_replicated, _set_head, _set_post, _struc_grad, _struc_rows, \
    _unpack_head
from ._launch import _F32, _as_f32c, _capturing, _vp, _workspace, _workspace_bytes, launch
from .ops import _drop_now, _drop_spec, cast_bf16, gemm, gemm_drop_supported, gemm_split, proj3, proj_bwd, proj_bwd_supported, \
    proj_fwd, spmm, spmm_v


def _literal_project(ctx, x, w3, ops, cfg):
    call, hops = ctx.call, ctx.hops
    sparse_x = isinstance(x, SparseFeatures)
    n, dev = x.shape[0], w3[0].device
    f_in, f = w3[0].shape
    four = cfg.n_channels == 4
    use_proj = (not sparse_x and f <= 5 and f_in <= 64
                and w3[0].stride(0) == w3[1].stride(0) == w3[2].stride(0))
    fb = ctx.fb = _chan_block(f)
    ldz = 3 * f
    if f in (2, 4, 8):
        ldz = -(-3 * f // (2 * f)) * (2 * f)
    elif fb != f:
        ldz = -(-(2 * fb + f) // 4) * 4
    pre = _take_pre_proj(call, x, w3, cfg.relu_before) if use_proj else None
    drop_spec = _drop_spec(ctx.in_drop, ops.row_offset) if ctx.in_drop is not None else None
    two_tables = (use_proj or f in (2, 4, 8) or hops > 1) and not sparse_x
    pack4 = four and f == 2 and fb == 2 and two_tables and not ops.sharded and not getattr(ops, "general", False)
    done3 = False
    if pre is None and not sparse_x:
        if two_tables:
            zlh, _ = _narrow_tables(n, fb, f, dev, pack4)
            zi = torch.empty(n, f, dtype=_F32, device=dev)
            done3 = proj3(x, w3, fb, zlh, zi, relu=cfg.relu_before, x_drop=drop_spec)
        else:
            z = torch.empty(n, ldz, dtype=_F32, device=dev)[:, : 2 * fb + f]
            done3 = proj3(x, w3, fb, z, relu=cfg.relu_before, x_drop=drop_spec)
            zlh, zi = z[:, : 2 * fb], z[:, 2 * fb:]
        if done3:
            ctx.in_drop_used = drop_spec is not None
    if (not done3 and drop_spec is not None
            and (pre is not None or use_proj or two_tables or sparse_x or not gemm_drop_supported(n, f_in, 2 * fb + f))):
        if sparse_x:
            raise NotImplementedError("in_drop with CSR features: the caller applies the dropout to the values")
        x, pre = _drop_now(x, drop_spec), None
        drop_spec = None
    if done3:
        pass
    elif pre is not None:
        zlh, zi = pre
    elif use_proj:
        zlh, _ = _narrow_tables(n, fb, f, dev, pack4)
        zi = torch.empty(n, f, dtype=_F32, device=dev)
        proj_fwd(x, w3, zlh, zi, relu=cfg.relu_before, h_col=fb)
    else:
        if fb != f:
            zpad = w3[0].new_zeros(w3[0].shape[0], fb - f)
            wcat = torch.cat((w3[0], zpad, w3[1], zpad, w3[2]), dim=1).contiguous()
        else:
            wcat = torch.cat(w3, dim=1).contiguous()
        if two_tables:
            zlh, _ = _narrow_tables(n, fb, f, dev, pack4)
            zi = torch.empty(n, f, dtype=_F32, device=dev)
            gemm_split(x, wcat, zlh, zi, relu=cfg.relu_before)
        else:
            z = torch.empty(n, ldz, dtype=_F32, device=dev)[:, : 2 * fb + f]
            if sparse_x:
                spmm_v(x.csr, x.values, wcat, relu=cfg.relu_before, out=z)
            else:
                gemm(x, wcat, relu=cfg.relu_before, out=z, a_drop=drop_spec)
                ctx.in_drop_used = drop_spec is not None
            zlh, zi = z[:, : 2 * fb], z[:, 2 * fb:]
    if hops > 2:
        t = zlh[:, :f]
        for hop in range(hops - 1):
            t = _low_product(ops, t, out=zlh[:, :f] if hop == hops - 2 else None)
        zg = _pkg._gather_rows(ops, zlh) if ops.sharded else zlh
    elif hops > 1:
        zc = torch.empty(n, 2 * fb, dtype=_F32, device=dev)
        _low_product(ops, zlh[:, :f], out=zc[:, :f])
        zc[:, fb:fb + f] = zlh[:, fb:fb + f]
        zg = _pkg._gather_rows(ops, zc)
    else:
        zg = _pkg._gather_rows(ops, zlh) if ops.sharded else zlh
    return x, zlh, zi, zg


class _AcmLiteral(torch.autograd.Function):

    @staticmethod
    def forward(ctx, x, w_low, w_high, w_mlp, v_low, v_high, v_mlp, v_struc, struc_low, att_mix, lnw_low, lnw_high, lnw_mlp,
                lnw_struc, lnb_low, lnb_high, lnb_mlp, lnb_struc, ops, cfg, post_relu, post_scale, post_drop, call, tail_layer,
                agg_holder, in_drop, pregathered):
        x = _conv_prologue(ctx, x, w_low, ops, post_relu, post_scale, post_drop, call, in_drop)
        call, post_scale = ctx.call, ctx.post_scale
        sparse_x = isinstance(x, SparseFeatures)
        dev, n = x.device, x.shape[0]
        f_in, f = w_low.shape
        k = cfg.n_channels
        four = k == 4
        general = bool(getattr(ops, "general", False))
        hops = ctx.hops = int(getattr(ops, "hops", 1))
        if hops > 1 and (cfg.relu_before or cfg.relu_after or four or general):
            raise NotImplementedError("hops > 1 is the ACM-SGC chain: model_type 'acmsgc' only")
        if general and ops.sharded:
            raise NotImplementedError("general operator pairs are not row-sharded")
        zero_padded = x.shape[1] != f_in
        if zero_padded:
# ... 144 lines not shown
        q.defer = defer.pointer() if defer is not None else None
        launch("acm_conv_bwd_local", f"conv_bwd_local/F{f}k{k}", dev, n, C.byref(q), _vp(ws), ws.numel() * 4)
        if defer is not None:
            defer.hold(ws, [d_mix, *d_vec, *d_lnw, *d_lnb], keep=[st3["flat"]])
    return x, (wl, wh, wm), zlh, st3


def _literal_backward(ctx, grad_out):
    x, w3, zlh, s = _k3_backward(ctx, grad_out)
    ops, cfg, defer = ctx.ops, ctx.cfg, ctx.call.defer
    g, dz, gs, flat, nw, ones = s["g"], s["dz"], s["gs"], s["flat"], s["nw"], s["ones"]
    k, fb, dev = cfg.n_channels, ctx.fb, dz.device
    four = k == 4
    n, (f_in_w, f) = dz.shape[0], w3[0].shape
    d_struc = torch.empty(n, f, dtype=_F32, device=dev) if four else None
    r = _lib.ConvBwdSpmm()
    r.f_out, r.row_offset = f, ops.row_offset
    if s["general"]:
        t_l = spmm(ops.low.transpose(), g[:, :f])
        t_h = spmm(ops.high.transpose(), g[:, fb:fb + f])
        zero = ops.zeros(n, f)
        low_t = ops.eye
        r.g_low, r.ld_g_low = t_l.data_ptr(), t_l.stride(0)
        r.g_high, r.ld_g_high = zero.data_ptr(), zero.stride(0)
        r.s_high, r.ld_s_high = t_h.data_ptr(), t_h.stride(0)
        if four:
            t_s = spmm(ops.un.transpose(), gs)
            r.g_struc, r.ld_g_struc = t_s.data_ptr(), t_s.stride(0)
            r.s_struc, r.ld_s_struc = zero.data_ptr(), zero.stride(0)
            r.inv_deg = ones.data_ptr()
            r.d_struc, r.ld_d_struc = d_struc.data_ptr(), d_struc.stride(0)
    else:
        gg = _pkg._gather_rows(ops, g)
        gsg = _pkg._gather_rows(ops, gs) if four else None
        low_t = ops.low_t
        if cfg.gather_bf16 and 8 < f <= 64 and f % 2 == 0 and fb == f:
            gb = cast_bf16(gg[:, : 2 * f])
            r.gather_bf16 = 1
            r.g_low, r.ld_g_low = gb.data_ptr(), gb.stride(0)
            r.g_high, r.ld_g_high = gb.data_ptr() + 2 * f, gb.stride(0)
            if four:
                gsg = cast_bf16(gsg)
        else:
            r.g_low, r.ld_g_low = gg.data_ptr(), gg.stride(0)
            r.g_high, r.ld_g_high = gg.data_ptr() + 4 * fb, gg.stride(0)
        r.s_high, r.ld_s_high = g.data_ptr() + 4 * fb, g.stride(0)
        if four:
            r.g_struc, r.ld_g_struc = gsg.data_ptr(), gsg.stride(0)
            r.s_struc, r.ld_s_struc = gs.data_ptr(), gs.stride(0)
            r.inv_deg = None if ops.implicit else ops.inv_deg.data_ptr()
            r.d_struc, r.ld_d_struc = d_struc.data_ptr(), d_struc.stride(0)
        if ops.implicit:
            r.self_scale = ops.self_scale.data_ptr()
    if cfg.relu_before:
        r.mask_low, r.ld_mask_low = zlh.data_ptr(), zlh.stride(0)
        r.mask_high, r.ld_mask_high = zlh.data_ptr() + 4 * fb, zlh.stride(0)
    r.dz_low, r.ld_dz_low = dz.data_ptr(), dz.stride(0)
    r.dz_high, r.ld_dz_high = dz.data_ptr() + 4 * f, dz.stride(0)
    ws2 = low_t.workspace((k - 1) * f)
    launch("acm_conv_bwd_spmm", f"conv_bwd_spmm/F{f}k{k}", dev, low_t.handle, C.byref(r), _vp(ws2), ws2.numel() * 4)
    if ctx.hops > 2 and ops.implicit:
        sc = _hop_buffer(dz, f)
        torch.mul(dz[:, :f], ops.row_scale[:, None], out=sc)
        for hop in range(ctx.hops - 2):
            sc = spmm(ops.low_t, _pkg._gather_rows(ops, sc), out=_hop_buffer(dz, f), row_scale=ops.row_scale)
        spmm(ops.low_t, _pkg._gather_rows(ops, sc), out=dz[:, :f])
    elif ctx.hops > 1:
        t = dz[:, :f]
        last = ctx.hops - 2
        for hop in range(ctx.hops - 1):
            t = _low_product(ops, t, transpose=True, out=dz[:, :f] if (hop == last and hop > 0) else None)
        if last == 0:
            dz[:, :f] = t

    if ctx.sparse_x is not None:
        xs = ctx.sparse_x
        xt = xs.csr_t
        d_wcat = spmm_v(xt, xs.values.index_select(0, xt.src_pos), dz, out=flat[:nw].view(f_in_w, 3 * f))
        d_x = None
    elif (ctx.needs_input_grad[0] and proj_bwd_supported(3 * f)
          and w3[0].stride(0) == w3[1].stride(0) == w3[2].stride(0)):
        d_wcat = flat[:nw].view(3, f_in_w, f)
        prod = getattr(ctx, "lazy_producer", None)
        if (prod is not None and f <= 2 and f_in_w == 64 and x.shape[1] == 64 and getattr(prod, "lazy", None) is None
                and all(w.stride(0) == f and w.is_contiguous() for w in w3)):
            d_x = torch.empty(n, x.shape[1], dtype=_F32, device=dev)
            prod.lazy = dict(dz=dz, w3=w3, d_w=d_wcat, x=x, placeholder=d_x)
        else:
            d_x = proj_bwd(x, dz, w3, d_wcat, defer=defer)
    else:
        d_wcat = gemm(x, dz, trans_a=True, col_blocks=3,
                      out=flat[:nw].view(3, f_in_w, f),
                      a_drop=_drop_spec(ctx.in_drop, ops.row_offset) if getattr(ctx, "in_drop_used", False) else None)
        d_x = gemm(dz, torch.cat(w3, dim=1), trans_b=True) if ctx.needs_input_grad[0] else None
    if d_x is not None and d_x.shape[1] != ctx.x_width:
        d_x = torch.nn.functional.pad(d_x, (0, ctx.x_width - d_x.shape[1]))
    _reduce_replicated(flat, ops, defer)
    if d_wcat.dim() == 3:
        d_w3 = (d_wcat[0], d_wcat[1], d_wcat[2])
    else:
        d_w3 = tuple(d_wcat[:, i * f:(i + 1) * f] for i in range(3))
    return _grads(d_x, d_w3, s["d_vec"], d_struc, s["d_mix"], s["d_lnw"], s["d_lnb"])


class _AcmAcmii(torch.autograd.Function):

    @staticmethod
    def forward(ctx, x, w_low, w_high, w_mlp, v_low, v_high, v_mlp, v_struc, struc_low, att_mix, lnw_low, lnw_high, lnw_mlp,
                lnw_struc, lnb_low, lnb_high, lnb_mlp, lnb_struc, ops, cfg, post_relu, post_scale, post_drop, call, tail_layer,
                agg_holder, in_drop, pregathered):
        x = _conv_prologue(ctx, x, w_low, ops, post_relu, post_scale, post_drop, call, in_drop)
        dev, n = x.device, x.shape[0]
        f_in, f = w_low.shape
        k = cfg.n_channels
        four = k == 4
        fp = 8
        zero_padded = x.shape[1] != f_in
        x, xpad, xg, _, _ = _gathered_input(ctx, x, ops, f_in, f, fp, agg_holder, pregathered, False)
        w3 = wl, wh, wm = tuple(_as_f32c(t, "weight") for t in (w_low, w_high, w_mlp))
        x = x[:, :f_in].contiguous() if zero_padded else x
        if four:
            s_local, s_gath = _struc_rows(ops, struc_low, n)
        vecs, lnw, lnb, mix = _head_params(cfg, (v_low, v_high, v_mlp, v_struc), att_mix, (lnw_low, lnw_high, lnw_mlp, lnw_struc),
                                           (lnb_low, lnb_high, lnb_mlp, lnb_struc))
        out = torch.empty(n, f, dtype=_F32, device=dev)
        att = torch.empty(n, 4, dtype=_F32, device=dev)
        zlh = torch.empty(n, 2 * f, dtype=_F32, device=dev)
        zi = torch.empty(n, f, dtype=_F32, device=dev)
        pre = torch.empty(n, (k - 1) * f, dtype=_F32, device=dev)
        p = _lib.ConvAcmiiFwd()
        p.f_in, p.f_pad, p.f_out = f_in, fp, f
        _set_head(p, cfg, vecs, lnw, lnb, mix)
        if four:
            ps = spmm(ops.low, s_gath, row_scale=ops.row_scale if ops.implicit else None, bf16=cfg.gather_bf16)
            p.ps, p.ld_ps = ps.data_ptr(), ps.stride(0)
            p.ss, p.ld_ss = s_local.data_ptr(), s_local.stride(0)
            p.deg = ops.deg.data_ptr()
        p.xg, p.ld_xg = xg.data_ptr(), xg.stride(0)
        p.xs, p.ld_xs = xpad.data_ptr(), xpad.stride(0)
        p.w_low, p.w_high, p.w_mlp, p.ld_w = wl.data_ptr(), wh.data_ptr(), wm.data_ptr(), f
        p.out, p.ld_out = out.data_ptr(), out.stride(0)
        p.pre, p.ld_pre = pre.data_ptr(), pre.stride(0)
        p.att = att.data_ptr()
        p.zlh, p.ld_zlh = zlh.data_ptr(), zlh.stride(0)
        p.zi, p.ld_zi = zi.data_ptr(), zi.stride(0)
        if ops.implicit:
            p.row_scale = ops.row_scale.data_ptr()
        _set_post(p, ctx.post_relu, ctx.post_scale, ctx.post_drop, ops.row_offset)
        ws = _workspace(dev, "acm_conv_acmii_fwd_workspace_bytes", ops.low.handle)
        ctx.mask_table = None
        if (ops.implicit and not ctx.needs_input_grad[0] and n > 0 and xg.shape[0] == ops.low.n_cols
                and (tuning.HOST.rewrites & tuning.REWRITE_ACMII_MASK) != 0
                and (getattr(ops.low, "item_stream_waves", 0) > 0
                     or (not _capturing(dev) and ops.low.build_item_streams()))):
            ng = xg.shape[0]
            tb = _workspace_bytes("acm_acmii_table_bytes", ng)
            table = torch.empty(tb // 4, dtype=torch.int32, device=dev)
            st = launch("acm_acmii_table", f"acmii_table/{ng}x{f_in}", dev, ng, f_in, xg.data_ptr(), xg.stride(0), wl.data_ptr(), wh.data_ptr(),
                        f, table.data_ptr(), tb, unsupported_ok=True)
            if st == 0:
                if ops.low.n_long_rows == 0:
                    p.zlh, p.ld_zlh = None, 0
                st = launch("acm_conv_acmii_v_fwd", f"conv_acmii_v_fwd/F{f}i{f_in}", dev, ops.low.handle, C.byref(p), table.data_ptr(), _vp(ws),
                            ws.numel() * 4, unsupported_ok=True)
                if st == 0:
                    ctx.mask_table, ctx.mask_x = table, xpad
                    ctx.mask_self_offset = 0
                    if ops.sharded:
                        import torch.distributed as dist
                        ctx.mask_self_offset = dist.get_rank(ops.group) * (ops.n_gathered // dist.get_world_size(ops.group))
                else:
                    p.zlh, p.ld_zlh = zlh.data_ptr(), zlh.stride(0)
        if ctx.mask_table is None:
# ... 37 lines not shown
```

acm_gnn_amd/layers.py:

```python
import math

import torch
import torch.nn as nn
import torch.nn.functional as F
from torch.nn.parameter import Parameter

from . import functional as AF
from . import tuning
from .graph import FilterOperators, SparseFeatures, operators_for

_TORCH_DROPOUT = F.dropout

DEFAULT_ATTN_LAYERNORM = True
_PLUS_LITERAL = ("acmgcn+", "acmgcn++")
_PLUS = ("acmgcnp", "acmgcnpp") + _PLUS_LITERAL


def _default_device():
    return torch.device("cuda:0" if torch.cuda.is_available() else "cpu")


class GraphConvolution(nn.Module):
    def __init__(self, in_features, out_features, nnodes, model_type, output_layer=0, variant=False,
                 structure_info=0, attn_layernorm=None, gather_dtype=None):
# ... 23 lines not shown
        self.reset_parameters()

    def reset_parameters(self):
        bound_w = 1.0 / math.sqrt(self.weight_mlp.size(1))
        bound_v = 1.0 / math.sqrt(self.att_vec_mlp.size(1))
        bound_m = 1.0 / math.sqrt(self.att_vec.size(1))
        for p in (self.weight_low, self.weight_high, self.weight_mlp, self.struc_low):
            p.data.uniform_(-bound_w, bound_w)
        for p in (self.att_vec_high, self.att_vec_low, self.att_vec_mlp, self.att_struc_low):
            p.data.uniform_(-bound_v, bound_v)
        self.att_vec.data.uniform_(-bound_m, bound_m)
        for ln in (self.layer_norm_low, self.layer_norm_high, self.layer_norm_mlp,
                   self.layer_norm_struc_low, self.layer_norm_struc_high):
            ln.reset_parameters()

    def _config(self):
        return AF.AcmConfig(self.model_type, self.variant, self.structure_info, self.attn_layernorm, self.gather_dtype)

    def _param_dict(self):
        p = self._parameters
        m = self._modules
        try:
            lo, hi, ml, sl = (m[k]._parameters for k in ("layer_norm_low", "layer_norm_high", "layer_norm_mlp", "layer_norm_struc_low"))
            return {
                "weight_low": p["weight_low"], "weight_high": p["weight_high"], "weight_mlp": p["weight_mlp"],
                "att_vec_low": p["att_vec_low"], "att_vec_high": p["att_vec_high"], "att_vec_mlp": p["att_vec_mlp"],
                "att_struc_low": p["att_struc_low"], "struc_low": p["struc_low"], "att_vec": p["att_vec"],
                "layer_norm_low.weight": lo["weight"], "layer_norm_low.bias": lo["bias"],
                "layer_norm_high.weight": hi["weight"], "layer_norm_high.bias": hi["bias"],
                "layer_norm_mlp.weight": ml["weight"], "layer_norm_mlp.bias": ml["bias"],
                "layer_norm_struc_low.weight": sl["weight"], "layer_norm_struc_low.bias": sl["bias"],
            }
        except KeyError:
            pass
        return {
            "weight_low": self.weight_low, "weight_high": self.weight_high, "weight_mlp": self.weight_mlp,
            "att_vec_low": self.att_vec_low, "att_vec_high": self.att_vec_high, "att_vec_mlp": self.att_vec_mlp,
            "att_struc_low": self.att_struc_low, "struc_low": self.struc_low, "att_vec": self.att_vec,
            "layer_norm_low.weight": self.layer_norm_low.weight, "layer_norm_low.bias": self.layer_norm_low.bias,
            "layer_norm_high.weight": self.layer_norm_high.weight, "layer_norm_high.bias": self.layer_norm_high.bias,
            "layer_norm_mlp.weight": self.layer_norm_mlp.weight, "layer_norm_mlp.bias": self.layer_norm_mlp.bias,
            "layer_norm_struc_low.weight": self.layer_norm_struc_low.weight,
            "layer_norm_struc_low.bias": self.layer_norm_struc_low.bias,
        }

    CSR_CHECK_MIN_ELEMENTS = 1 << 24

    def _csr_input(self, x):
        if F.dropout is not _TORCH_DROPOUT:
            return x
        twin = SparseFeatures.known_twin(x)
        if twin is not None:
            return twin
        if not self.training:
            if getattr(x, "_acm_csr_twin", None) is None and getattr(self, "_csr_refused", None) == tuple(x.shape):
                return x
            out = SparseFeatures.auto(x)
            if out is not x:
                self._csr_ref = out
            else:
                self._csr_refused = tuple(x.shape)
            return out
        ref = getattr(self, "_csr_ref", None)
        if (ref is None or x.requires_grad or x.dtype != torch.float32 or x.dim() != 2
                or x.numel() < self.CSR_CHECK_MIN_ELEMENTS or tuning.HOST.csr_features <= 0
                or (x.is_cuda and torch.cuda.is_current_stream_capturing())):
            return x
        out = ref.twin_of_masked(x)
        return x if out is None else out

    def forward(self, input, adj_low, adj_high=None, adj_low_unnormalized=None, post_relu=False, post_scale=None,
                post_drop=None, rows_permuted=False, call=None, input_drop=None):
        mt = self.model_type
        if mt == "mlp":
            return AF.mm(input, self.weight_mlp)
        if mt in ("sgc", "gcn"):
            if isinstance(adj_low, torch.Tensor) and adj_low.layout != torch.strided:
                raise RuntimeError("model_type 'sgc'/'gcn' multiplies with torch.mm: adj_low must be dense")
            return AF.mm(adj_low, AF.mm(input, self.weight_low))
        cfg = self._config()
        if isinstance(input, torch.Tensor) and input.layout != torch.strided:
            input = SparseFeatures.from_torch(input)
        elif (isinstance(input, torch.Tensor) and input_drop is None and not rows_permuted
                and not (isinstance(adj_low, FilterOperators) and adj_low.sharded)):
            input = self._csr_input(input)
        if isinstance(adj_low, FilterOperators):
            ops = adj_low
        else:
            ops = operators_for(adj_low, adj_high, adj_low_unnormalized if cfg.n_channels == 4 else None)
        params = self._param_dict()
        raw_input = input
        translate = ops.perm is not None and not rows_permuted
        if ops.perm is not None:
            if cfg.n_channels == 4:
                params["struc_low"] = self.struc_low.index_select(0, ops.perm)
            if translate:
                input = input.permute_rows(ops.perm) if isinstance(input, SparseFeatures) else input.index_select(0, ops.perm)
                if post_scale is not None:
                    post_scale = post_scale.index_select(0, ops.perm)
        tail_layer = (bool(self.output_layer) and not post_relu and post_scale is None and post_drop is None
                      and not translate)
        holder = self._eval_agg_holder(raw_input, ops) if (input_drop is None or input_drop[0] <= 0) else None
        if input_drop is not None and not AF.in_drop_supported(input, ops, cfg, self.in_features, self.out_features):
            p_in, tag_in, st_in = input_drop
            input = AF.dropout(input, p_in, st_in, tag=tag_in, row_offset=ops.row_offset)
            input_drop = None
        out, att = AF.acm_conv(input, params, ops, cfg, post_relu, post_scale, post_drop, call=call,
                               tail_layer=tail_layer, agg_holder=holder, in_drop=input_drop)
        if translate:
            out = out.index_select(0, ops.inv_perm)
        d = self.__dict__
        d["_att_raw"], d["_att_inv"], d["_att_k"] = att, ops.inv_perm, cfg.n_channels
        return out

    def _eval_agg_holder(self, x, ops):
        if not isinstance(x, torch.Tensor) or x.requires_grad or x.grad_fn is not None or not self.eval_agg_cache:
            return None
        key = (x.data_ptr(), x._version, tuple(x.shape), tuple(x.stride()))
        role = "train" if (self.training and torch.is_grad_enabled()) else "eval"
        slots = self.__dict__.setdefault("_eval_agg", {})
        cached = slots.get(role)
        if cached is None or cached[0] != key or cached[3] is not ops:
            cached = (key, x, {"agg": None}, ops)
            slots[role] = cached
        return cached[2]

    def held_entries(self):
        return list(self.__dict__.get("_eval_agg", {}).values())

    def _att_col(self, c):
        if self._att_raw is None:
            return 0
        if self._att_inv is not None:
            self._att_raw, self._att_inv = self._att_raw.index_select(0, self._att_inv), None
        return self._att_raw[:, c:c + 1]

    att_low = property(lambda self: self._att_col(0))
    att_high = property(lambda self: self._att_col(1))
    att_mlp = property(lambda self: self._att_col(2))

    @property
    def att_struc_vec_low(self):
        if self._att_raw is None or self._att_k != 4:
            raise AttributeError("att_struc_vec_low exists after a forward with structure_info (layers.py:111)")
        return self._att_col(3)

    def __repr__(self):
        return f"{self.__class__.__name__} ({self.in_features} -> {self.out_features})"


class MLP(nn.Module):

    def __init__(self, in_channels, hidden_channels, out_channels, num_layers, dropout=0.5):
        super().__init__()
        self.lins, self.bns = nn.ModuleList(), nn.ModuleList()
        if num_layers == 1:
            self.lins.append(nn.Linear(in_channels, out_channels))
            self.bns.append(nn.BatchNorm1d(out_channels))
        else:
            self.lins.append(nn.Linear(in_channels, hidden_channels))
            self.bns.append(nn.BatchNorm1d(hidden_channels))
            for _ in range(num_layers - 2):
                self.lins.append(nn.Linear(hidden_channels, hidden_channels))
                self.bns.append(nn.BatchNorm1d(hidden_channels))
            self.lins.append(nn.Linear(hidden_channels, out_channels))
        self.dropout = dropout

# ... 12 lines not shown
```

acm_gnn_amd/models.py:

```python
import torch
import torch.nn as nn
import torch.nn.functional as F

from . import functional as AF
from .graph import FilterOperators, SparseFeatures
from .layers import GraphConvolution, MLP

_TORCH_DROPOUT = F.dropout

_TWO_LAYER = ("acmgcn", "acmgcnp", "acmgcnpp")


class GCN(nn.Module):
    def __init__(self, nfeat, nhid, nclass, nlayers, nnodes, dropout, model_type, structure_info,
                 variant=False, init_layers_X=1, attn_layernorm=None, gather_dtype=None):
        super().__init__()
        self.model_type, self.structure_info = model_type, structure_info
        self.nlayers, self.nnodes, self.dropout = nlayers, nnodes, dropout
        if model_type == "acmgcnpp":
            self.mlpX = MLP(nfeat, nhid, nhid, num_layers=init_layers_X, dropout=0)
        self.gcns, self.mlps = nn.ModuleList(), nn.ModuleList()
        kw = dict(model_type=model_type, variant=variant, structure_info=structure_info,
                  attn_layernorm=attn_layernorm, gather_dtype=gather_dtype)
        if model_type in _TWO_LAYER:
# ... 4 lines not shown
        elif model_type == "acmsnowball":
            for k in range(nlayers):
                self.gcns.append(GraphConvolution(k * nhid + nfeat, nhid, nnodes, model_type=model_type, variant=variant,
                                                  attn_layernorm=attn_layernorm, gather_dtype=gather_dtype))
            self.gcns.append(GraphConvolution(nlayers * nhid + nfeat, nclass, nnodes, model_type=model_type,
                                              variant=variant, attn_layernorm=attn_layernorm, gather_dtype=gather_dtype))
        else:
            raise ValueError(f"GCN: unsupported model_type {model_type!r} "
                             "(acmgcn | acmgcnp | acmgcnpp | acmsgc | acmsnowball)")
        dev = self.gcns[0].weight_low.device
        self.fea_param = nn.Parameter(torch.zeros(1, 1, device=dev))
        self.xX_param = nn.Parameter(torch.zeros(1, 1, device=dev))
        self.fused_dropout = False
        self.dropout_state = None
        self.reset_parameters()

    def _ones_like_hidden(self, n, f, device):
        key = (n, f, str(device))
        if getattr(self, "_ones_key", None) != key:
            self._ones_key, self._ones = key, torch.ones(n, f, device=device)
        return self._ones

    def reset_parameters(self):
        if self.model_type == "acmgcnpp":
            self.mlpX.reset_parameters()

    def _residual(self, x, adj_low, drop=None, call=None, pipe=None):
        ops = adj_low if isinstance(adj_low, FilterOperators) else None
        group = ops.group if (ops is not None and ops.sharded) else None
        if len(self.mlpX.lins) == 1 and self.mlpX.lins[0].out_features <= 256:
            lin = self.mlpX.lins[0]
            return AF.residual_linear(x, lin.weight, lin.bias, relu=True, drop=drop, group=group, call=call, pipe=pipe)
        if group is not None:
            raise NotImplementedError("row-sharded acmgcnpp supports init_layers_X = 1 with nhid <= 256 (the torch fallback "
                                      "does not reduce its gradients over the ranks)")
        if isinstance(x, SparseFeatures):
            raise NotImplementedError("CSR features with init_layers_X > 1 or nhid > 256")
        f_in = self.mlpX.lins[0].in_features
        out = F.relu(self.mlpX(x if x.shape[1] == f_in else x[:, :f_in], input_tensor=True))
        if drop is not None and drop[0] > 0:
            out = AF.dropout(out, drop[0], drop[2], tag=drop[1], row_offset=drop[3])
        return out

    def _forward_fused_dropout(self, x, adj_low, adj_high, adj_low_unnormalized, call):
        p = self.dropout
        if self.dropout_state is None:
            dev = x.values.device if isinstance(x, SparseFeatures) else x.device
            self.dropout_state = AF.DropoutState(dev)
        st = self.dropout_state
        off = adj_low.row_offset if isinstance(adj_low, FilterOperators) else 0
        kw = {}
        if isinstance(x, SparseFeatures):
            x = x.with_values(AF.dropout(x.values.reshape(-1, 1), p, st, tag=0).reshape(-1))
        else:
            nfeat = x.shape[1]
            pad = AF.agg_pad_width(nfeat)
            ops = adj_low if isinstance(adj_low, FilterOperators) else None
            piped = (call.pipe is not None and call.pipe.primed and call.pipe.ops is ops and call.pipe.state is st
                     and call.pipe.x_rows.data_ptr() == x.data_ptr() and call.pipe.x_rows.shape == x.shape
                     and torch.is_grad_enabled())
            if piped:
                x = call.pipe.local_table()
                if ops.sharded:
                    ops._pregathered = (x, call.pipe.table())
            elif ops is not None and ops.sharded and ops.uniform and ops.x_full is not None and nfeat <= 16:
                xg = AF.dropout(ops.x_full, p, st, tag=0, pad_to=pad, row_offset=0)
                x = xg[off:off + x.shape[0]]
                ops._pregathered = (x, xg)
            elif (self.model_type in ("acmgcn", "acmgcnp", "acmsgc") and pad == nfeat and not x.requires_grad
                    and AF.in_drop_supported(x, ops, self.gcns[0]._config(), nfeat, self.gcns[0].out_features)
                    if ops is not None else False):
                kw = {"input_drop": (p, 0, st)}
            else:
                x = AF.dropout(x, p, st, tag=0, pad_to=pad, row_offset=off)
        if self.model_type == "acmsgc":
            return self.gcns[0](x, adj_low, adj_high, adj_low_unnormalized, rows_permuted=self._rows_permuted, call=call, **kw)
        xx = None
        lin = self.mlpX.lins[0] if (self.model_type == "acmgcnpp" and len(self.mlpX.lins) == 1) else None
        add_fused = lin is not None and AF.residual_add_supported(x, lin.weight)
        if self.model_type == "acmgcnpp" and not add_fused:
            xx = self._residual(x, adj_low, drop=(p, 2, st, off), call=call,
                                pipe=call.pipe if (not isinstance(x, SparseFeatures) and piped) else None)
        call.next_proj = self.gcns[1] if self.model_type != "acmgcnpp" else None
        fea = self.gcns[0](x, adj_low, adj_high, adj_low_unnormalized, post_relu=True, post_drop=(p, 1, st), **kw,
                           rows_permuted=self._rows_permuted, call=call)
        call.next_proj = None
        if add_fused:
            ops_ = adj_low if isinstance(adj_low, FilterOperators) else None
            xr = x
            if call.pipe is not None and x.data_ptr() == call.pipe.local_table().data_ptr() and call.pipe.adopted:
                xr = call.pipe.saved[0]
            fea = AF.residual_add_linear(fea, xr, lin.weight, lin.bias, relu=True, drop=(p, 2, st, off),
                                         group=ops_.group if (ops_ is not None and ops_.sharded) else None, call=call)
        elif self.model_type == "acmgcnpp":
            fea = fea + xx
        else:
            call.hidden_private = fea
        try:
            return self.gcns[1](fea, adj_low, adj_high, adj_low_unnormalized, rows_permuted=self._rows_permuted, call=call)
        finally:
            call.hidden_private = None

    def _forward_snowball(self, x, adj_low, adj_high, fused, call):
        if isinstance(x, SparseFeatures):
            raise NotImplementedError("acmsnowball concatenates the input with the hidden blocks: dense features only")
        p, st = self.dropout, self.dropout_state
        off = adj_low.row_offset if isinstance(adj_low, FilterOperators) else 0
        if fused:
            x = AF.dropout(x, p, st, tag=0, row_offset=off)
        else:
            x = F.dropout(x, p, training=self.training)
        blocks = []
        for k in range(self.nlayers):
            inp = x if k == 0 else torch.cat([x] + blocks, 1)
            if fused:
                h = self.gcns[k](inp, adj_low, adj_high, None, post_relu=True, post_drop=(p, 1 + k, st), rows_permuted=self._rows_permuted, call=call)
            else:
                scale = None
                if self.training and p > 0:
                    scale = F.dropout(self._ones_like_hidden(x.shape[0], self.gcns[k].out_features, x.device), p, training=True)
                h = self.gcns[k](inp, adj_low, adj_high, None, post_relu=True, post_scale=scale, rows_permuted=self._rows_permuted, call=call)
            blocks.append(h)
        return self.gcns[-1](torch.cat([x] + blocks, 1), adj_low, adj_high, None, rows_permuted=self._rows_permuted, call=call)

    def auto_csr(self, x, ops):
        if not isinstance(x, torch.Tensor) or F.dropout is not _TORCH_DROPOUT or self.model_type == "acmsnowball":
            return x
        if ops is not None and ops.sharded:
            return x
        if self.model_type == "acmgcnpp" and not (len(self.mlpX.lins) == 1 and self.mlpX.lins[0].out_features <= 256):
            return x
        return SparseFeatures.auto(x)

    def forward(self, x, adj_low, adj_high=None, adj_low_unnormalized=None, rows_permuted=False, call=None):
        call = AF.CallContext.from_ambient() if call is None else call
        ops = adj_low if isinstance(adj_low, FilterOperators) else None
        if ops is None and isinstance(adj_low, torch.Tensor):
            from .graph import operators_for
            four = self.structure_info and self.model_type in ("acmgcnp", "acmgcnpp")
            ops = adj_low = operators_for(adj_low, adj_high, adj_low_unnormalized if four else None)
        self.__dict__["_rows_permuted"] = ops is not None and ops.perm is not None
        if not rows_permuted:
            x = self.auto_csr(x, ops)
        if self._rows_permuted and not rows_permuted:
            x = x.permute_rows(ops.perm) if isinstance(x, SparseFeatures) else x.index_select(0, ops.perm)
            return self._forward(x, adj_low, adj_high, adj_low_unnormalized, call).index_select(0, ops.inv_perm)
        return self._forward(x, adj_low, adj_high, adj_low_unnormalized, call)

    def _forward(self, x, adj_low, adj_high, adj_low_unnormalized, call):
        fused = self.fused_dropout and self.training and self.dropout > 0
        if fused and self.dropout_state is None:
            dev = x.values.device if isinstance(x, SparseFeatures) else x.device
            self.dropout_state = AF.DropoutState(dev)
        if self.model_type == "acmsnowball":
            return self._forward_snowball(x, adj_low, adj_high, fused, call)
        if fused:
            return self._forward_fused_dropout(x, adj_low, adj_high, adj_low_unnormalized, call)
        drop = lambda t: F.dropout(t, self.dropout, training=self.training)
        if isinstance(x, SparseFeatures):
            x = x.with_values(drop(x.values))
        else:
            x = drop(x)
        if self.model_type == "acmsgc":
            return self.gcns[0](x, adj_low, adj_high, adj_low_unnormalized, rows_permuted=self._rows_permuted, call=call)
        if self.model_type == "acmgcnpp":
            xx = drop(self._residual(x, adj_low, call=call))
        scale = None
        if self.training and self.dropout > 0:
            ones = self._ones_like_hidden(x.shape[0], self.gcns[0].out_features, x.device)
            scale = drop(ones)
        call.next_proj = self.gcns[1] if self.model_type != "acmgcnpp" else None
        fea = self.gcns[0](x, adj_low, adj_high, adj_low_unnormalized, post_relu=True, post_scale=scale,
                           rows_permuted=self._rows_permuted, call=call)
        call.next_proj = None
        if self.model_type == "acmgcnpp":
            fea = fea + xx
        else:
            call.hidden_private = fea
        try:
            return self.gcns[1](fea, adj_low, adj_high, adj_low_unnormalized, rows_permuted=self._rows_permuted, call=call)
        finally:
            call.hidden_private = None
```

acm_gnn_amd/tuning.py:

```python
import contextlib
import ctypes as C
import os
import threading

KERNEL_KEYS = ("chunk", "wide_form", "bwd_split", "rows16", "agg_fused", "gemm_forms")
HOST_DEFAULTS = {"rewrites": 15, "implicit": 1, "relabel": -1, "pipeline": 8192, "csr_features": 256, "small_step": 16384}
HOST_RANGES = {"rewrites": (0, 15), "implicit": (0, 1), "relabel": (-1, 1), "pipeline": (0, 1 << 31), "csr_features": (0, 1 << 31),
               "small_step": (0, 16384)}

REWRITE_AGG_FIRST = 1
REWRITE_ACMII_RECOMPUTE = 2
REWRITE_ACMII_MASK = 4
REWRITE_AGGW_FUSED = 8
ROWS16_EPI, ROWS16_BWD, ROWS16_LOCAL = 1, 2, 4
GEMM_ROWS, GEMM_BX3, GEMM_BX3_WIDE, GEMM_ROWS_ALWAYS = 1, 2, 4, 8


class Tuning(C.Structure):
    _fields_ = [(k, C.c_int32) for k in KERNEL_KEYS] + [("reserved", C.c_int32 * 10)]


class _Host:
    __slots__ = tuple(HOST_DEFAULTS)

    def __init__(self, **kw):
        for k, v in HOST_DEFAULTS.items():
            setattr(self, k, int(kw.get(k, v)))

    def as_dict(self):
        return {k: getattr(self, k) for k in HOST_DEFAULTS}


def parse(text):
    kern, host = {}, {}
    for item in (text or "").split(","):
        item = item.strip()
        if not item:
            continue
        key, sep, val = item.partition("=")
        if not sep:
            raise ValueError(f"ACM_TUNING: '{item}' is not key=value")
        try:
            v = int(val, 0)
        except ValueError:
            raise ValueError(f"ACM_TUNING: '{item}': the value must be an integer") from None
        if key in KERNEL_KEYS:
            kern[key] = v
        elif key in HOST_DEFAULTS:
            lo, hi = HOST_RANGES[key]
            if not lo <= v <= hi:
                raise ValueError(f"ACM_TUNING: {key}={v} outside {lo}..{hi}")
            host[key] = v
        else:
            raise ValueError(f"ACM_TUNING: unknown key '{key}' (known: {', '.join(KERNEL_KEYS + tuple(HOST_DEFAULTS))})")
    return kern, host


def parse_lenient(text, report=None):
    import sys
    report = report or (lambda msg: sys.stderr.write(f"acm_gnn_amd: {msg} (ignored)\n"))
    kern, host = {}, {}
    for item in (text or "").split(","):
        if not item.strip():
            continue
        try:
            k, h = parse(item)
        except ValueError as exc:
            report(str(exc))
            continue
        kern.update(k)
        host.update(h)
    return kern, host


LEGACY_ENV = ("ACM_GATHER_DTYPE", "ACM_EVAL_AGG_CACHE", "ACM_CHUNK", "ACM_WIDE_FORM", "ACM_BWD_SPLIT", "ACM_AGG_FUSED", "ACM_PIPELINE",
              "ACM_IMPLICIT", "ACM_RELABEL", "ACM_REWRITES", "ACM_ROWS16", "ACM_GEMM_FORMS")


def _report_legacy(environ, report=None):
    import sys
    report = report or (lambda msg: sys.stderr.write(f"acm_gnn_amd: {msg}\n"))
    found = [k for k in LEGACY_ENV if k in environ]
    if found:
        report(f"{', '.join(found)}: environment switches of earlier rounds are no longer read; use ACM_TUNING=\"key=value,...\"")
    return found


_LOADED_HOST = parse_lenient(os.environ.get("ACM_TUNING", ""))[1]
_report_legacy(os.environ)
HOST = _Host(**_LOADED_HOST)
_lock = threading.RLock()
_kernel_cache = None
_kernel_touched = False


def kernel():
# ... 100 lines not shown
```

include/acm_hip.h:

```cpp
#ifndef ACM_HIP_H
#define ACM_HIP_H

#include <stddef.h>
#include <stdint.h>

#ifdef __cplusplus
extern "C" {
#endif

#define ACM_ABI_VERSION 28

typedef enum {
    ACM_OK = 0,
    ACM_EINVAL = 1,
    ACM_ESHAPE = 2,
    ACM_EHIP = 3,
    ACM_EUNSUPPORTED = 4,
    ACM_ENOMEM = 5,
} acm_status_t;

typedef struct acm_csr acm_csr_t;
typedef void* acm_stream_t;

int acm_version(void);
const char* acm_last_error(void);

typedef struct {
    int32_t chunk;
    int32_t wide_form;
    int32_t bwd_split;
    int32_t rows16;
    int32_t agg_fused;
    int32_t gemm_forms;
    int32_t reserved[10];
} acm_tuning_t;
int acm_tuning_get(acm_tuning_t* out);
int acm_tuning_set(const acm_tuning_t* in);

int acm_csr_create(int64_t n_rows, int64_t n_cols, int64_t nnz,
                   const int32_t* indptr_dev, const int32_t* indices_dev,
                   const float* vals_dev, int chunk, acm_csr_t** out);
int acm_csr_transpose(const acm_csr_t* a, int chunk, acm_csr_t** out);
int acm_csr_slice_rows(const acm_csr_t* a, int64_t row_begin, int64_t row_end,
                       int chunk, acm_csr_t** out);
void acm_csr_destroy(acm_csr_t* a);

int acm_shard_plan(int64_t n_rows, const int64_t* indptr_host, int world, int64_t row_cost,
                   int64_t* bounds_host);

typedef struct {
    int64_t n_rows, n_cols, nnz;
    int64_t n_items;
    int64_t n_long_rows;
    int64_t n_partial_slots;
    int32_t chunk;
    int32_t max_degree;
    const int32_t* indptr;
    const int32_t* indices;
    const float* vals;
    const int32_t* src_pos;
    int64_t stream_steps;
    int64_t stream_slices;
    int32_t stream_waves;
    int32_t stream_long_rows;
    int32_t item_stream_waves;
    int32_t reserved;
    int64_t item_stream_batches;
} acm_csr_info_t;
int acm_csr_info(const acm_csr_t* a, acm_csr_info_t* info);

int acm_csr_build_streams(acm_csr_t* a, int n_waves, int lmax);

int acm_csr_build_item_streams(acm_csr_t* a, int n_waves);

int acm_spmm_workspace_bytes(const acm_csr_t* a, int width, size_t* bytes);

int acm_gemm_workspace_bytes(int transA, int transB, int64_t M, int64_t N, int64_t K,
                             size_t* bytes);
int acm_gemm(int transA, int transB, int64_t M, int64_t N, int64_t K,
             const float* A, int64_t lda, const float* B, int64_t ldb,
             float* C, int64_t ldc, int relu, void* workspace, size_t workspace_bytes,
             acm_stream_t stream);

int acm_gemm_blocks(int transA, int transB, int64_t M, int64_t N, int64_t K,
                    const float* A, int64_t lda, const float* B, int64_t ldb,
                    float* C, int64_t ldc, int64_t c_col_block, int64_t c_block_stride, int relu,
                    void* workspace, size_t workspace_bytes, acm_stream_t stream);

typedef struct {
    float    p;
    int32_t  tag;
    uint64_t seed;
    const int64_t* step;
    int64_t  row_offset;
    int64_t  step_offset;
} acm_dropout_t;

int acm_dropout(int64_t n_rows, int64_t n_cols, const float* src, int64_t ld_src,
                float* dst, int64_t ld_dst, int64_t dst_cols, const acm_dropout_t* d, acm_stream_t stream);

int acm_gemm_drop(int transA, int transB, int64_t M, int64_t N, int64_t K,
                  const float* A, int64_t lda, const float* B, int64_t ldb,
                  float* C, int64_t ldc, int64_t c_col_block, int64_t c_block_stride, int relu,
                  const acm_dropout_t* a_drop, void* workspace, size_t workspace_bytes, acm_stream_t stream);

int acm_proj3(int64_t n_rows, int64_t K, const float* X, int64_t ldx,
              const float* w_low, const float* w_high, const float* w_mlp, int64_t ld_w, int64_t f, int64_t f_block,
              float* C, int64_t ldc, int64_t split_col, float* C2, int64_t ldc2, int relu,
// ... 132 lines not shown
    const float* ln_bias[4];
    const float* att_mix;
    float* g_low;   int64_t ld_g_low;
    float* g_high;  int64_t ld_g_high;
    float* g_mlp;   int64_t ld_g_mlp;
    float* g_struc; int64_t ld_g_struc;
    float* d_att_vec[4];
    float* d_ln_weight[4];
    float* d_ln_bias[4];
    float* d_att_mix;
    const float* post_scale; int64_t ld_post_scale;
    int32_t post_relu;
    const float* g_scale;
    acm_dropout_t post_drop;
    acm_reduce_list_t* defer;
} acm_conv_bwd_local_t;

int acm_conv_bwd_local_workspace_bytes(int64_t n_rows, int f_out, int n_channels, size_t* bytes);
int acm_conv_bwd_local(int64_t n_rows, const acm_conv_bwd_local_t* p,
                       void* workspace, size_t workspace_bytes, acm_stream_t stream);

int acm_conv_aggw_bwd_workspace_bytes(int64_t n_rows, int64_t f_pad, size_t* bytes);
int acm_conv_aggw_bwd(int64_t n_rows, int64_t f_in, int64_t f_pad, const float* agg, int64_t ld_agg, const float* xs,
                      int64_t ld_xs, const acm_conv_bwd_local_t* p, float* d_w_low, float* d_w_high, float* d_w_mlp,
                      int64_t ld_dw, void* workspace, size_t workspace_bytes, acm_stream_t stream);

typedef struct {
    int32_t f_out;
    int64_t row_offset;
    const float* g_low;   int64_t ld_g_low;
    const float* g_high;  int64_t ld_g_high;
    const float* g_struc; int64_t ld_g_struc;
    const float* s_high;  int64_t ld_s_high;
    const float* s_struc; int64_t ld_s_struc;
    const float* inv_deg;
    const float* mask_low;  int64_t ld_mask_low;
    const float* mask_high; int64_t ld_mask_high;
    float* dz_low;   int64_t ld_dz_low;
    float* dz_high;  int64_t ld_dz_high;
    float* d_struc;  int64_t ld_d_struc;
    const float* self_scale;
    int32_t gather_bf16;
} acm_conv_bwd_spmm_t;

int acm_conv_bwd_spmm(const acm_csr_t* a_low_t, const acm_conv_bwd_spmm_t* p,
                      void* workspace, size_t workspace_bytes, acm_stream_t stream);


typedef struct {
    int32_t f_in, f_pad;
    int32_t f_out, relu_after, relu_mlp, layernorm;
    float   scale;
    const float* xg; int64_t ld_xg;
    const float* xs; int64_t ld_xs;
    const float* w_low; const float* w_high; const float* w_mlp; int64_t ld_w;
    const float* att_vec[4];
    const float* ln_weight[4];
    const float* ln_bias[4];
    const float* att_mix;
    float* out; int64_t ld_out;
    float* agg; int64_t ld_agg;
    float* att;
    const float* post_scale; int64_t ld_post_scale;
    int32_t post_relu;
    int32_t n_channels;
    const void*  sg; int64_t ld_sg;
    int32_t sg_bf16;
    const float* ss; int64_t ld_ss;
    const float* deg;
    float* ps; int64_t ld_ps;
    const float* row_scale;
    acm_dropout_t post_drop;
    float* head_stats; int64_t ld_head_stats;
    const float* next_w_low; const float* next_w_high; const float* next_w_mlp; int64_t next_ld_w;
    int32_t next_f, next_relu;
    float* next_zlh; int64_t ld_next_zlh;
    float* next_zi;  int64_t ld_next_zi;
    int32_t agg_given;
    int32_t reserved0;
    float* agg_copy; int64_t ld_agg_copy;
    float* xs_copy;  int64_t ld_xs_copy;
    const float* next_x; int64_t ld_next_x;
    acm_dropout_t next_drop;
} acm_conv_agg_fwd_t;

int acm_conv_agg_fwd(const acm_csr_t* a_low, const acm_conv_agg_fwd_t* p,
                     void* workspace, size_t workspace_bytes, acm_stream_t stream);

typedef struct {
    int32_t f_in, f_pad, f_out, relu_after, relu_mlp, layernorm;
    float   scale;
    const float* grad_out; int64_t ld_grad_out;
    const float* agg; int64_t ld_agg;
    const float* xs;  int64_t ld_xs;
    const float* w_low; const float* w_high; const float* w_mlp; int64_t ld_w;
    const float* att_vec[4];
    const float* ln_weight[4];
    const float* ln_bias[4];
    const float* att_mix;
    float* d_params;
    const float* post_scale; int64_t ld_post_scale;
    int32_t post_relu;
    int32_t n_channels;
    const float* ps; int64_t ld_ps;
    const float* ss; int64_t ld_ss;
    const float* deg;
    float* g_struc; int64_t ld_g_struc;
    const float* g_struc_scale;
    acm_dropout_t post_drop;
    acm_reduce_list_t* defer;
    const float* head_stats; int64_t ld_head_stats;
    const float* out; int64_t ld_out;
    const acm_csr_t* next_a;
    const float* next_xg; int64_t ld_next_xg;
    const float* next_row_scale;
    float* next_agg; int64_t ld_next_agg;
    const float* proj_dz; int64_t ld_proj_dz;
    const float* proj_w_low; const float* proj_w_high; const float* proj_w_mlp; int64_t proj_ld_w;
    int32_t proj_f;
    float* proj_d_w;
} acm_conv_agg_bwd_t;

int acm_conv_agg_bwd_workspace_bytes(int64_t n_rows, int f_in, int f_out, size_t* bytes);
int acm_conv_agg_bwd(int64_t n_rows, const acm_conv_agg_bwd_t* p,
                     void* workspace, size_t workspace_bytes, acm_stream_t stream);

typedef struct {
    int32_t f_in, f_pad, f_out;
    int32_t layernorm;
    float   scale;
    const float* xg; int64_t ld_xg;
    const float* xs; int64_t ld_xs;
    const float* w_low; const float* w_high; const float* w_mlp; int64_t ld_w;
    const float* att_vec[4];
    const float* ln_weight[4];
    const float* ln_bias[4];
    const float* att_mix;
    float* out; int64_t ld_out;
    float* pre; int64_t ld_pre;
    float* att;
    float* zlh; int64_t ld_zlh;
    float* zi;  int64_t ld_zi;
    const float* post_scale; int64_t ld_post_scale;
    int32_t post_relu;
    const float* row_scale;
    acm_dropout_t post_drop;
    int32_t n_channels;
    const float* ps; int64_t ld_ps;
    const float* ss; int64_t ld_ss;
    const float* deg;
} acm_conv_acmii_fwd_t;

int acm_conv_acmii_fwd_workspace_bytes(const acm_csr_t* a_low, size_t* bytes);
int acm_conv_acmii_fwd(const acm_csr_t* a_low, const acm_conv_acmii_fwd_t* p,
                       void* workspace, size_t workspace_bytes, acm_stream_t stream);

typedef struct {
    int32_t f_in;
    const void* table;
    const float* g_low;  int64_t ld_g_low;
    const float* g_high; int64_t ld_g_high;
    const float* g_mlp;  int64_t ld_g_mlp;
    const float* x; int64_t ld_x;
    int64_t self_offset;
    const float* row_scale;
    float* d_w_low; float* d_w_high; float* d_w_mlp; int64_t ld_dw;
    acm_reduce_list_t* defer;
} acm_conv_acmii_bwd_t;

int acm_acmii_table_bytes(int64_t n_rows, size_t* bytes);
int acm_acmii_table(int64_t n_rows, int f_in, const float* x, int64_t ld_x, const float* w_low, const float* w_high,
                    int64_t ld_w, void* table, size_t table_bytes, acm_stream_t stream);
int acm_conv_acmii_v_fwd(const acm_csr_t* a_low, const acm_conv_acmii_fwd_t* p, const void* table,
                         void* workspace, size_t workspace_bytes, acm_stream_t stream);
int acm_conv_acmii_v_bwd_workspace_bytes(const acm_csr_t* a_low, size_t* bytes);
int acm_conv_acmii_v_bwd(const acm_csr_t* a_low, const acm_conv_acmii_bwd_t* p,
                         void* workspace, size_t workspace_bytes, acm_stream_t stream);

int acm_nll_loss_workspace_bytes(int64_t n_rows, size_t* bytes);
int acm_nll_loss(int64_t n_rows, int n_classes, const float* logits, int64_t ld_logits,
                 const int64_t* labels, const float* row_weight,
                 float* loss, float* dlogits, int64_t ld_dlogits,
                 void* workspace, size_t workspace_bytes, acm_reduce_list_t* defer, acm_stream_t stream);

int acm_eval_metrics_workspace_bytes(int64_t n_rows, int n_sets, size_t* bytes);
int acm_eval_metrics(int64_t n_rows, int n_classes, const float* logits, int64_t ld_logits, const int64_t* labels,
                     const float* weights, int64_t ld_weights, int n_sets, int loss_set, float* out,
                     void* workspace, size_t workspace_bytes, acm_stream_t stream);

typedef struct {
    int32_t n_classes;
    const int64_t* labels;
    const float*   row_weight;
    float* loss;
    float* dlogits; int64_t ld_dlogits;
} acm_loss_t;

int acm_conv_fwd_tail_workspace_bytes(int64_t n_rows, int f_out, int n_channels, size_t* bytes);
int acm_conv_fwd_tail(const acm_csr_t* a_low, const acm_conv_fwd_t* fwd, const acm_loss_t* loss,
                      const acm_conv_bwd_local_t* bwd, void* workspace, size_t workspace_bytes,
                      void* tail_workspace, size_t tail_workspace_bytes, acm_stream_t stream);

typedef struct {
// ... 69 lines not shown
```

Before: 50.71 billion edges/s.

## Keep layer-1 hidden private: skip writing out, store dropout bits, recompute in backward

```diff
diff --git a/acm_gnn_amd/_lib.py b/acm_gnn_amd/_lib.py
--- a/acm_gnn_amd/_lib.py
+++ b/acm_gnn_amd/_lib.py
@@ -9,7 +9,7 @@
 
 ACM_OK = 0
 STATUS_NAMES = {1: "ACM_EINVAL", 2: "ACM_ESHAPE", 3: "ACM_EHIP", 4: "ACM_EUNSUPPORTED", 5: "ACM_ENOMEM"}
-ABI_VERSION = 28
+ABI_VERSION = 29
 
 EXPORTED_SYMBOLS = (
     "acm_version", "acm_last_error", "acm_tuning_get", "acm_tuning_set", "acm_csr_create", "acm_csr_transpose", "acm_csr_slice_rows",
@@ -116,7 +116,8 @@
                 ("next_zlh", C.c_void_p), ("ld_next_zlh", C.c_int64), ("next_zi", C.c_void_p), ("ld_next_zi", C.c_int64),
                 ("agg_given", C.c_int32), ("reserved0", C.c_int32),
                 ("agg_copy", C.c_void_p), ("ld_agg_copy", C.c_int64), ("xs_copy", C.c_void_p), ("ld_xs_copy", C.c_int64),
-                ("next_x", C.c_void_p), ("ld_next_x", C.c_int64), ("next_drop", Dropout)]
+                ("next_x", C.c_void_p), ("ld_next_x", C.c_int64), ("next_drop", Dropout),
+                ("post_keep", C.c_void_p), ("ld_post_keep", C.c_int64)]
 
 
 class ConvAggBwd(C.Structure):
@@ -139,7 +140,8 @@
                 ("next_row_scale", C.c_void_p), ("next_agg", C.c_void_p), ("ld_next_agg", C.c_int64),
                 ("proj_dz", C.c_void_p), ("ld_proj_dz", C.c_int64),
                 ("proj_w_low", C.c_void_p), ("proj_w_high", C.c_void_p), ("proj_w_mlp", C.c_void_p), ("proj_ld_w", C.c_int64),
-                ("proj_f", C.c_int32), ("proj_d_w", C.c_void_p)]
+                ("proj_f", C.c_int32), ("proj_d_w", C.c_void_p),
+                ("post_keep", C.c_void_p), ("ld_post_keep", C.c_int64)]
 
 
 class ConvAcmiiFwd(C.Structure):
@@ -321,6 +323,13 @@
         return _lib
 
 
+def capability(name):
+    try:
+        return int(C.c_int32.in_dll(load(), name).value)
+    except (ValueError, AttributeError, TypeError):
+        return 0
+
+
 def check(status, what=""):
     if status != ACM_OK:
         msg = load().acm_last_error().decode(errors="replace")
diff --git a/acm_gnn_amd/csrc/acm_conv_agg.hip b/acm_gnn_amd/csrc/acm_conv_agg.hip
--- a/acm_gnn_amd/csrc/acm_conv_agg.hip
+++ b/acm_gnn_amd/csrc/acm_conv_agg.hip
@@ -584,7 +584,17 @@
     ACM_REQUIRE(a && p, ACM_EINVAL, "acm_conv_agg_fwd: NULL argument");
     int st = check_common(p, "acm_conv_agg_fwd");
     if (st != ACM_OK) return st;
-    ACM_REQUIRE((p->xg || p->agg_given) && p->out && p->agg && p->att, ACM_EINVAL, "acm_conv_agg_fwd: NULL tensor pointer");
+    ACM_REQUIRE((p->xg || p->agg_given) && p->agg && p->att, ACM_EINVAL, "acm_conv_agg_fwd: NULL tensor pointer");
+    if (!p->out) {
+        ACM_REQUIRE(p->next_f >= 1 && p->agg_given, ACM_EINVAL,
+                    "acm_conv_agg_fwd: out is NULL without a fused next projection (next_f) over a given agg (agg_given)");
+        ACM_REQUIRE(!(p->post_drop.p > 0.f) || (p->post_keep && p->ld_post_keep >= 4), ACM_EINVAL,
+                    "acm_conv_agg_fwd: out is NULL under dropout without post_keep (ld_post_keep >= 4)");
+        ACM_REQUIRE(p->n_channels == 3 && p->f_pad == 8 && p->f_out == 64 && !p->post_scale && (acm_tuning().rows16 & ACM_ROWS16_EPI) != 0 &&
+                        a->n_rows * (p->ld_post_keep > 64 ? p->ld_post_keep : 64) < (int64_t)INT32_MAX, ACM_EUNSUPPORTED,
+                    "acm_conv_agg_fwd: out is NULL outside the sixteen-rows-per-wave stage that carries the next projection "
+                    "(three channels, f_pad 8, f_out 64, no post_scale, acm_tuning_t.rows16 bit 1)");
+    }
     ACM_REQUIRE((p->agg_given || (((uintptr_t)p->xg) % 16 == 0 && (p->ld_xg * 4) % 16 == 0 && p->ld_xg >= p->f_pad)) &&
                     ((uintptr_t)p->agg) % 16 == 0 && (p->ld_agg * 4) % 16 == 0 && p->ld_agg >= p->f_pad &&
                     ((uintptr_t)p->att) % 16 == 0, ACM_EINVAL,
@@ -650,6 +660,7 @@
         if (st == ACM_OK) return next_done ? ACM_OK : next_projection(a, p, stream);
         if (st > 0) return st;
     }
+    ACM_REQUIRE(p->out, ACM_EUNSUPPORTED, "acm_conv_agg_fwd: out is NULL and the sixteen-rows-per-wave stage did not take the call");
     int grid = (int)((a->n_rows + 15) / 16);
     if (grid > 2048) grid = 2048;
     const CsrView cv = acm_view(a);
@@ -699,6 +710,12 @@
     }
     ACM_REQUIRE(((uintptr_t)p->agg) % 16 == 0 && (p->ld_agg * 4) % 16 == 0 && p->ld_agg >= p->f_pad, ACM_EINVAL,
                 "acm_conv_agg_bwd: agg rows must be 16-byte aligned and f_pad long");
+    if (p->proj_dz && !p->out) {
+        ACM_REQUIRE(p->head_stats && p->post_relu && !p->post_scale && (!(p->post_drop.p > 0.f) || (p->post_keep && p->ld_post_keep >= 4)),
+                    ACM_EINVAL, "acm_conv_agg_bwd: proj_dz without out needs head_stats, post_relu, no post_scale and (under dropout) post_keep");
+        ACM_REQUIRE(p->n_channels == 3 && p->f_pad == 8 && p->f_out == 64, ACM_EUNSUPPORTED,
+                    "acm_conv_agg_bwd: proj_dz without out: three channels, f_pad 8, f_out 64 only");
+    }
     size_t need = 0;
     acm_conv_agg_bwd_workspace_bytes(n_rows, p->f_in, p->f_out, &need);
     ACM_REQUIRE(workspace && workspace_bytes >= need, ACM_ENOMEM, "acm_conv_agg_bwd: workspace %zu B < required %zu B",
diff --git a/acm_gnn_amd/csrc/acm_conv_agg16.hip b/acm_gnn_amd/csrc/acm_conv_agg16.hip
--- a/acm_gnn_amd/csrc/acm_conv_agg16.hip
+++ b/acm_gnn_amd/csrc/acm_conv_agg16.hip
@@ -7,8 +7,9 @@
 #define ACM_E16_NEXT_LDS (64 * 8)
 
 
-template <int NC, int FP, bool LN, bool NEXT>
+template <int NC, int FP, bool LN, bool NEXT, bool NOOUT>
 __device__ __forceinline__ void epi16_body(const acm_conv_agg_fwd_t& p, int n_rows) {
+    static_assert(!NOOUT || NEXT, "without `out` the row must be consumed by the next layer's projection");
     constexpr int KB = FP / 4;
     __shared__ __attribute__((aligned(16))) float ulds[NC * 64 + (NEXT ? ACM_E16_NEXT_LDS : 0)];
     const int lane = threadIdx.x & 63, m = lane & 15, g = lane >> 4;
@@ -204,18 +205,27 @@
                 o[t] *= s;
             }
         }
+        unsigned kw = 0;
         if (dc.on) {
 #pragma unroll
             for (int r = 0; r < 4; ++r) {
                 unsigned w[4];
                 acm_philox7(dc, row, 4 * g + r, w);
 #pragma unroll
-                for (int t = 0; t < 4; ++t) o[t][r] *= (w[t] >= dc.thresh) ? dc.inv_keep : 0.f;
+                for (int t = 0; t < 4; ++t) {
+                    const bool keep = w[t] >= dc.thresh;
+                    o[t][r] *= keep ? dc.inv_keep : 0.f;
+                    if (NOOUT) kw |= keep ? (1u << (4 * t + r)) : 0u;
+                }
             }
         }
         if (valid) {
-#pragma unroll
-            for (int t = 0; t < 4; ++t) *reinterpret_cast<f32x4*>(p.out + rr * ld_out + 16 * t + 4 * g) = o[t];
+            if (!NOOUT) {
+#pragma unroll
+                for (int t = 0; t < 4; ++t) *reinterpret_cast<f32x4*>(p.out + rr * ld_out + 16 * t + 4 * g) = o[t];
+            } else if (dc.on) {
+                p.post_keep[(size_t)rr * p.ld_post_keep + g] = (uint16_t)kw;
+            }
         }
         if (NEXT) {
             const float* nlds = ulds + NC * 64;
@@ -246,9 +256,9 @@
     }
 }
 
-template <int NC, int FP, bool LN, bool NEXT>
+template <int NC, int FP, bool LN, bool NEXT, bool NOOUT = false>
 __global__ __launch_bounds__(256) void agg_epi16_kernel(acm_conv_agg_fwd_t p, int n_rows) {
-    epi16_body<NC, FP, LN, NEXT>(p, n_rows);
+    epi16_body<NC, FP, LN, NEXT, NOOUT>(p, n_rows);
 }
 
 #define ACM_B16_TS 68
@@ -266,9 +276,10 @@
     static_assert(TOTAL * 4 <= 64 * 1024, "static LDS of one workgroup");
 };
 
-template <int NC, int FP, bool LN, bool OUT_MASK, bool PROJ, bool GATHER>
+template <int NC, int FP, bool LN, bool OUT_MASK, bool PROJ, bool GATHER, bool RECOMP_OUT>
 __device__ __forceinline__ void bwd16_body(const acm_conv_agg_bwd_t& p, int n_rows, float* __restrict__ partial, const GatherRole* gr) {
     using L = B16Lds<NC, FP, PROJ>;
+    static_assert(!RECOMP_OUT || (NC == 3 && PROJ && OUT_MASK), "the rebuilt `out` tile: three channels, the carried projection backward");
     constexpr int KB = L::KB, PS = L::PS;
     __shared__ __attribute__((aligned(16))) float lds[L::TOTAL];
     const int lane = threadIdx.x & 63, m = lane & 15, g = lane >> 4, wv = threadIdx.x >> 6;
@@ -341,11 +352,21 @@
     int base = wave * 16;
     float nP[KB], nx[KB];
     f32x4 ngo[4], nou[4], nst[NC];
+    constexpr int IA = 3 * NC, QA = IA >> 2;
+    static_assert(!RECOMP_OUT || ((IA + 2) >> 2) == QA, "alpha_0..2 in one 16-byte piece of head_stats");
+    f32x4 pst = {0.f, 0.f, 0.f, 0.f};
+    unsigned pkw = 0xFFFFu;
+    const bool drop_on = p.post_drop.p > 0.f;
+    const unsigned ld_pk = (unsigned)p.ld_post_keep;
 #define ACM_B16_LOAD(BASE)                                                                              \
     do {                                                                                                \
         const unsigned r2 = (unsigned)min((BASE) + m, n_rows - 1);                                      \
         _Pragma("unroll") for (int kb = 0; kb < KB; ++kb)                                               \
             nP[kb] = p.agg[r2 * ld_agg + 4 * kb + g], nx[kb] = p.xs[r2 * ld_xs + 4 * kb + g];           \
+        if (RECOMP_OUT) {                                                                               \
+            pst = *reinterpret_cast<const f32x4*>(p.head_stats + r2 * ld_hs + 4 * QA);                  \
+            if (drop_on) pkw = p.post_keep[r2 * ld_pk + g];                                             \
+        }                                                                                               \
     } while (0)
 #pragma unroll
     for (int kb = 0; kb < KB; ++kb) nP[kb] = nx[kb] = 0.f;
@@ -362,10 +383,11 @@
 #pragma unroll
             for (int t = 0; t < 4; ++t) {
                 if (!PROJ) ngo[t] = *reinterpret_cast<const f32x4*>(p.grad_out + r1 * ld_go + 16 * t + 4 * g);
-                if (out_mask || PROJ) nou[t] = *reinterpret_cast<const f32x4*>(p.out + r1 * ld_out + 16 * t + 4 * g);
-            }
-#pragma unroll
-            for (int q = 0; q < NC; ++q) nst[q] = *reinterpret_cast<const f32x4*>(p.head_stats + r1 * ld_hs + 4 * q);
+                if ((out_mask || PROJ) && !RECOMP_OUT) nou[t] = *reinterpret_cast<const f32x4*>(p.out + r1 * ld_out + 16 * t + 4 * g);
+            }
+#pragma unroll
+            for (int q = 0; q < NC; ++q)
+                nst[q] = (RECOMP_OUT && q == QA) ? pst : *reinterpret_cast<const f32x4*>(p.head_stats + r1 * ld_hs + 4 * q);
             if (NC == 4) dgs = p.deg[r1];
             if (PROJ) {
 #pragma unroll
@@ -377,6 +399,7 @@
                 }
             }
         }
+        const unsigned kw = pkw;
         ACM_B16_LOAD(base + nwaves * 16);
         const int gq = acm_opaque(g), mq = acm_opaque(m);
 #pragma unroll
@@ -405,7 +428,40 @@
         }
         f32x4 dO[4];
         const float gate = valid ? post_gain : 0.f;
-        if (PROJ) {
+        if (RECOMP_OUT) {
+            const float a0 = nst[QA][IA & 3] * p.scale, a1 = nst[QA][(IA + 1) & 3] * p.scale, a2 = nst[QA][(IA + 2) & 3] * p.scale;
+            const float lo_post = p.post_relu ? 0.f : -INFINITY;
+#pragma unroll
+            for (int c = 0; c < 3; ++c) {
+                const float lo = c < 2 ? lo_a : lo_m;
+#pragma unroll
+                for (int t = 0; t < 4; ++t)
+#pragma unroll
+                    for (int r = 0; r < 4; ++r) D[RECOMP ? 0 : c][t][r] = fmaxf(D[RECOMP ? 0 : c][t][r], lo);
+            }
+#pragma unroll
+            for (int t = 0; t < 4; ++t) {
+                f32x4 o4;
+#pragma unroll
+                for (int r = 0; r < 4; ++r) {
+                    float o = fmaxf(fmaf(a2, D[RECOMP ? 0 : 2][t][r], fmaf(a1, D[RECOMP ? 0 : 1][t][r], a0 * D[0][t][r])), lo_post);
+                    if (drop_on) o *= ((kw >> (4 * t + r)) & 1u) ? post_gain : 0.f;
+                    o4[r] = o;
+                    const float4 wa = *reinterpret_cast<const float4*>(pw + (16 * t + 4 * gq + r) * 8);
+                    const float2 wb = *reinterpret_cast<const float2*>(pw + (16 * t + 4 * gq + r) * 8 + 4);
+                    float v = dzr[0] * wa.x;
+                    v = fmaf(dzr[1], wa.y, v), v = fmaf(dzr[2], wa.z, v), v = fmaf(dzr[3], wa.w, v);
+                    v = fmaf(dzr[4], wb.x, v), v = fmaf(dzr[5], wb.y, v);
+                    dO[t][r] = (o != 0.f) ? v * gate : 0.f;
+                }
+                *reinterpret_cast<f32x4*>(gt + mq * ACM_B16_TS + 16 * t + 4 * gq) = o4;
+            }
+#pragma unroll
+            for (int s = 0; s < 4; ++s)
+#pragma unroll
+                for (int t = 0; t < 4; ++t)
+                    acc2[t] = __builtin_amdgcn_mfma_f32_16x16x4f32(dza[s], gt[(4 * gq + s) * ACM_B16_TS + 16 * t + mq], acc2[t], 0, 0, 0);
+        } else if (PROJ) {
 #pragma unroll
             for (int t = 0; t < 4; ++t) *reinterpret_cast<f32x4*>(gt + mq * ACM_B16_TS + 16 * t + 4 * gq) = nou[t];
 #pragma unroll
@@ -628,14 +684,14 @@
     }
 }
 
-template <int NC, int FP, bool LN, bool OUT_MASK, bool PROJ>
+template <int NC, int FP, bool LN, bool OUT_MASK, bool PROJ, bool RECOMP_OUT = false>
 __global__ __launch_bounds__(256) __attribute__((amdgpu_waves_per_eu(2, 2))) void agg_bwd16_kernel(acm_conv_agg_bwd_t p, int n_rows, float* __restrict__ partial) {
-    bwd16_body<NC, FP, LN, OUT_MASK, PROJ, false>(p, n_rows, partial, nullptr);
+    bwd16_body<NC, FP, LN, OUT_MASK, PROJ, false, RECOMP_OUT>(p, n_rows, partial, nullptr);
 }
-template <int NC, bool LN, bool PROJ>
+template <int NC, bool LN, bool PROJ, bool RECOMP_OUT = false>
 __global__ __launch_bounds__(512) __attribute__((amdgpu_waves_per_eu(2, 2))) void agg_bwd16_gather_kernel(acm_conv_agg_bwd_t p, int n_rows, float* __restrict__ partial,
                                                                                                    GatherRole gr) {
-    bwd16_body<NC, 8, LN, true, PROJ, true>(p, n_rows, partial, &gr);
+    bwd16_body<NC, 8, LN, true, PROJ, true, RECOMP_OUT>(p, n_rows, partial, &gr);
 }
 
 }
@@ -654,6 +710,15 @@
     const bool next = p->next_f > 0;
     int grid = (int)((n_rows + 63) / 64);
     if (grid > 1024) grid = 1024;
+    if (!p->out) {
+        if (NC != 3 || FP != 8 || !next || p->post_scale || (p->post_drop.p > 0.f && (!p->post_keep || p->ld_post_keep < 4))) return -1;
+        if (n_rows * p->ld_post_keep >= (int64_t)INT32_MAX) return -1;
+        if (p->layernorm) hipLaunchKernelGGL((agg_epi16_kernel<3, 8, true, true, true>), dim3(grid), dim3(256), 0, s, *p, (int)n_rows);
+        else hipLaunchKernelGGL((agg_epi16_kernel<3, 8, false, true, true>), dim3(grid), dim3(256), 0, s, *p, (int)n_rows);
+        ACM_CHECK_HIP(hipGetLastError());
+        *next_done = true;
+        return ACM_OK;
+    }
 #define ACM_E16_L(NCv, FPv)                                                                                                   \
     do {                                                                                                                     \
         if (p->layernorm) {                                                                                                  \
@@ -685,12 +750,14 @@
     if ((NC != 3 && NC != 4) || (FP != 4 && FP != 8 && FP != 16) || p->f_out != 64 || !p->head_stats ||
         !(acm_tuning().rows16 & ACM_ROWS16_BWD))
         return 0;
-    const bool out_mask = p->out != nullptr && p->post_relu && !p->post_scale;
+    const bool proj = p->proj_dz != nullptr;
+    const bool recomp = proj && !p->out && NC == 3 && FP == 8 && p->post_relu && !p->post_scale &&
+                        (!(p->post_drop.p > 0.f) || (p->post_keep && p->ld_post_keep >= 4 && n_rows * p->ld_post_keep < (int64_t)INT32_MAX));
+    const bool out_mask = (p->out != nullptr || recomp) && p->post_relu && !p->post_scale;
     const bool no_post = !p->post_relu && !p->post_scale && !(p->post_drop.p > 0.f);
     if (!out_mask && !no_post) return 0;
-    const bool proj = p->proj_dz != nullptr;
     if ((proj || gr) && (FP != 8 || !out_mask)) return 0;
-    if (proj && (!p->out || p->proj_f < 1 || p->proj_f > 2 || !p->proj_w_low || !p->proj_w_high || !p->proj_w_mlp || !p->proj_d_w ||
+    if (proj && ((!p->out && !recomp) || p->proj_f < 1 || p->proj_f > 2 || !p->proj_w_low || !p->proj_w_high || !p->proj_w_mlp || !p->proj_d_w ||
                  p->ld_proj_dz < 3 * p->proj_f || p->proj_ld_w < p->proj_f || n_rows * p->ld_proj_dz >= (int64_t)INT32_MAX))
         return 0;
     for (const void* q : {(const void*)(proj ? nullptr : p->grad_out), (const void*)p->out, (const void*)p->head_stats,
@@ -732,7 +799,15 @@
             else hipLaunchKernelGGL((agg_bwd16_kernel<NCv, 8, false, true, true>), dim3(grid), dim3(256), 0, s, q, (int)n_rows, partial);                     \
         }                                                                                                                         \
     } while (0)
-    if (proj || gr) {
+    if (recomp) {
+        if (gr) {
+            if (ln) hipLaunchKernelGGL((agg_bwd16_gather_kernel<3, true, true, true>), dim3(grid), dim3(512), 0, s, q, (int)n_rows, partial, *gr);
+            else hipLaunchKernelGGL((agg_bwd16_gather_kernel<3, false, true, true>), dim3(grid), dim3(512), 0, s, q, (int)n_rows, partial, *gr);
+        } else {
+            if (ln) hipLaunchKernelGGL((agg_bwd16_kernel<3, 8, true, true, true, true>), dim3(grid), dim3(256), 0, s, q, (int)n_rows, partial);
+            else hipLaunchKernelGGL((agg_bwd16_kernel<3, 8, false, true, true, true>), dim3(grid), dim3(256), 0, s, q, (int)n_rows, partial);
+        }
+    } else if (proj || gr) {
         if (NC == 3) ACM_B16_CARRY(3);
         else ACM_B16_CARRY(4);
     } else if (NC == 3) {
diff --git a/acm_gnn_amd/csrc/acm_csr.cpp b/acm_gnn_amd/csrc/acm_csr.cpp
--- a/acm_gnn_amd/csrc/acm_csr.cpp
+++ b/acm_gnn_amd/csrc/acm_csr.cpp
@@ -24,6 +24,7 @@
 }
 
 extern "C" int acm_version(void) { return ACM_ABI_VERSION; }
+extern "C" const int32_t acm_cap_private_hidden = 1;
 extern "C" const char* acm_last_error(void) { return g_err; }
 
 namespace {
diff --git a/acm_gnn_amd/functional/__init__.py b/acm_gnn_amd/functional/__init__.py
--- a/acm_gnn_amd/functional/__init__.py
+++ b/acm_gnn_amd/functional/__init__.py
@@ -1,8 +1,8 @@
 from .. import _lib, tuning
 from ..graph import CsrGraph, FilterOperators, SparseFeatures, _device_ctx, _require_cuda, _stream
 from ._launch import KernelTimer, _Timed, set_kernel_timer
-from ._context import (CallContext, DeferredReductions, InputPipeline, Tape, TapeBroken, _ambient,
-                       deferred_reductions, deferred_reductions_as, fused_loss_tail, input_pipeline, on_tape)
+from ._context import (CallContext, DeferredReductions, InputPipeline, PrivateHidden, Tape, TapeBroken, _ambient,
+                       _private_of, private_hidden_enabled, deferred_reductions, deferred_reductions_as, fused_loss_tail, input_pipeline, on_tape)
 from .ops import (DropoutState, _drop_spec, agg_pad_width, cast_bf16, dropout, eval_metrics, eval_metrics_buffers,
                   gemm, gemm_drop_supported, gemm_split, masked_nll, mm, nll_loss_and_grad, proj3, proj_bwd,
                   proj_bwd_supported, proj_fwd, spmm, spmm_v)
diff --git a/acm_gnn_amd/functional/_context.py b/acm_gnn_amd/functional/_context.py
--- a/acm_gnn_amd/functional/_context.py
+++ b/acm_gnn_amd/functional/_context.py
@@ -83,12 +83,14 @@
 
 
 class CallContext:
-    __slots__ = ("defer", "tail", "pipe", "next_proj", "pre_proj", "hidden_private")
+    __slots__ = ("defer", "tail", "pipe", "next_proj", "pre_proj", "hidden_private", "hidden_private_next", "private_out")
 
     def __init__(self, defer=None, tail=None, pipe=None):
         self.defer, self.tail, self.pipe = defer, tail, pipe
         self.next_proj = self.pre_proj = None
         self.hidden_private = None
+        self.hidden_private_next = False
+        self.private_out = None
 
     @classmethod
     def from_ambient(cls):
@@ -417,6 +419,35 @@
         self._host_steps = self.state.host_steps
 
 
+class PrivateHidden:
+    __slots__ = ("placeholder", "_make", "real")
+    _NAN = {}
+
+    def __init__(self, n, f, dev, make):
+        nan = self._NAN.get(dev)
+        if nan is None:
+            nan = self._NAN[dev] = torch.full((1,), float("nan"), dtype=_F32, device=dev)
+        self.placeholder, self._make, self.real = nan.expand(n, f), make, None
+
+    def is_placeholder(self, x):
+        ph = self.placeholder
+        return isinstance(x, torch.Tensor) and x.data_ptr() == ph.data_ptr() and x.shape == ph.shape and x.stride() == ph.stride()
+
+    def materialize(self):
+        if self.real is None:
+            self.real = self._make()
+        return self.real
+
+
+def _private_of(call, x):
+    priv = getattr(call, "private_out", None)
+    return priv if (priv is not None and priv.is_placeholder(x)) else None
+
+
+def private_hidden_enabled():
+    return bool(tuning.HOST.rewrites & tuning.REWRITE_PRIVATE_HIDDEN) and _lib.capability("acm_cap_private_hidden") != 0
+
+
 def _next_proj_request(call, f, dev, row_local_only=False):
     nxt, call.next_proj = call.next_proj, None
     if nxt is None or not row_local_only or not (tuning.kernel()["rows16"] & tuning.ROWS16_EPI):
diff --git a/acm_gnn_amd/functional/_conv_shared.py b/acm_gnn_amd/functional/_conv_shared.py
--- a/acm_gnn_amd/functional/_conv_shared.py
+++ b/acm_gnn_amd/functional/_conv_shared.py
@@ -5,7 +5,7 @@
 from .. import _lib
 from .. import functional as _pkg
 from ..graph import SparseFeatures
-from ._context import _call_or_ambient, _sum_over_ranks
+from ._context import _call_or_ambient, _private_of, _sum_over_ranks
 from ._launch import _F32, _Timed, _as_f32c, _vp, launch
 from .ops import _drop_now, _drop_spec, cast_bf16, spmm
 
@@ -214,7 +214,7 @@
     ctx.call = _call_or_ambient(call)
     ctx.in_drop = in_drop if (in_drop is not None and in_drop[0] > 0) else None
     sparse_x = isinstance(x, SparseFeatures)
-    if not sparse_x:
+    if not sparse_x and _private_of(ctx.call, x) is None:
         x = _as_f32c(x, "input")
     n, f = x.shape[0], w_low.shape[1]
     if post_scale is not None:
diff --git a/acm_gnn_amd/functional/conv_agg.py b/acm_gnn_amd/functional/conv_agg.py
--- a/acm_gnn_amd/functional/conv_agg.py
+++ b/acm_gnn_amd/functional/conv_agg.py
@@ -4,7 +4,7 @@
 
 from .. import _lib, tuning
 from .. import functional as _pkg
-from ._context import _call_or_ambient, _next_proj_request
+from ._context import PrivateHidden, _call_or_ambient, _next_proj_request, private_hidden_enabled
 from ._conv_shared import _NO_GRADS, _conv_prologue, _flat_views, _gathered_input, _grads, _head_params, _k3_setup, \
     _narrow_tables, _pack_head, _reduce_replicated, _set_head, _set_post, _struc_grad, _struc_rows, _unpack_head
 from ._launch import EUNSUPPORTED, _F32, _as_f32c, _vp, _workspace, launch
@@ -31,7 +31,6 @@
             s_local, s_gath = _struc_rows(ops, struc_low, n)
         vecs, lnw, lnb, mix = _head_params(cfg, (v_low, v_high, v_mlp, v_struc), att_mix, (lnw_low, lnw_high, lnw_mlp, lnw_struc),
                                            (lnb_low, lnb_high, lnb_mlp, lnb_struc))
-        out = torch.empty(n, f, dtype=_F32, device=dev)
         att = torch.empty(n, 4, dtype=_F32, device=dev)
         p = _lib.ConvAggFwd()
         p.f_in, p.f_pad, p.f_out = f_in, fp, f
@@ -46,7 +45,6 @@
             p.agg_copy, p.ld_agg_copy = ctx.pipe.saved[1].data_ptr(), ctx.pipe.saved[1].stride(0)
             p.xs_copy, p.ld_xs_copy = ctx.pipe.saved[0].data_ptr(), ctx.pipe.saved[0].stride(0)
             refill = ctx.pipe.refill_spec(p)
-        p.out, p.ld_out = out.data_ptr(), out.stride(0)
         p.agg, p.ld_agg = agg.data_ptr(), agg.stride(0)
         p.att = att.data_ptr()
         if ops.implicit:
@@ -70,6 +68,41 @@
             p.head_stats, p.ld_head_stats = stats.data_ptr(), stats.stride(0)
         ctx.head_stats = stats
         nxt = _next_proj_request(call, f, dev, row_local_only=f == 64 and (agg_given is not None or four))
+        training = stats is not None
+        private = (nxt is not None and call.hidden_private_next and private_hidden_enabled() and fp == 8 and f == 64 and k == 3
+                   and agg_given is not None and ctx.post_relu and ctx.post_scale is None and not ops.sharded
+                   and (not training or call.defer is not None))
+        ctx.private = None
+        if private:
+            keep = torch.empty(n, 4, dtype=torch.int16, device=dev) if ctx.post_drop is not None else None
+            if keep is not None:
+                p.post_keep, p.ld_post_keep = keep.data_ptr(), keep.stride(0)
+            s_x, s_agg = (ctx.pipe.saved[0], ctx.pipe.saved[1]) if ctx.pipe is not None else (xpad, agg)
+            post, row_offset = (ctx.post_relu, ctx.post_drop), ops.row_offset
+            handle, ws_of = ops.low.handle, ops.low.workspace
+
+            def make(s_x=s_x, s_agg=s_agg):
+                real = torch.empty(n, f, dtype=_F32, device=dev)
+                m = _lib.ConvAggFwd()
+                m.f_in, m.f_pad, m.f_out = f_in, fp, f
+                _set_head(m, cfg, vecs, lnw, lnb, mix)
+                m.xs, m.ld_xs = s_x.data_ptr(), s_x.stride(0)
+                m.w_low, m.w_high, m.w_mlp, m.ld_w = wl.data_ptr(), wh.data_ptr(), wm.data_ptr(), f
+                m.agg, m.ld_agg, m.agg_given = s_agg.data_ptr(), s_agg.stride(0), 1
+                m.out, m.ld_out = real.data_ptr(), real.stride(0)
+                att2 = torch.empty(n, 4, dtype=_F32, device=dev)
+                m.att = att2.data_ptr()
+                _set_post(m, post[0], None, post[1], row_offset)
+                w2 = ws_of(fp)
+                launch("acm_conv_agg_fwd", f"conv_agg_epi/F{f}k{k}i{f_in}/materialise", dev, handle, C.byref(m), _vp(w2), w2.numel() * 4)
+                return real
+
+            priv = ctx.private = call.private_out = PrivateHidden(n, f, dev, make)
+            ctx.post_keep = keep
+            out = priv.placeholder
+        else:
+            out = torch.empty(n, f, dtype=_F32, device=dev)
+            p.out, p.ld_out = out.data_ptr(), out.stride(0)
         if nxt is not None:
             n_w3, n_relu, f2, n_pack = nxt
             n_zlh, _ = _narrow_tables(n, f2, f2, dev, n_pack)
@@ -91,7 +124,8 @@
         ctx.out_mask = bool(ctx.post_relu) and ctx.post_scale is None
         if ctx.pipe is not None:
             xpad, agg = ctx.pipe.saved[0], ctx.pipe.saved[1]
-        ctx.save_for_backward(xpad, agg, wl, wh, wm, *_pack_head(vecs, lnw, lnb, mix), *extra, *((out,) if ctx.out_mask else ()))
+        ctx.save_for_backward(xpad, agg, wl, wh, wm, *_pack_head(vecs, lnw, lnb, mix), *extra,
+                              *((out,) if (ctx.out_mask and not private) else ()))
         ctx.mark_non_differentiable(att)
         return out, att
 
@@ -104,7 +138,8 @@
         four = k == 4
         saved = ctx.saved_tensors
         out_fwd = None
-        if ctx.out_mask:
+        priv = getattr(ctx, "private", None)
+        if ctx.out_mask and priv is None:
             out_fwd, saved = saved[-1], saved[:-1]
         xpad, agg, wl, wh, wm = saved[:5]
         vecs, lnw, lnb, mix = _unpack_head(saved, cfg, 5)
@@ -114,12 +149,17 @@
         if lazy is not None and (grad_out is not lazy["placeholder"] and grad_out.data_ptr() != lazy["placeholder"].data_ptr()):
             raise RuntimeError("acm_conv: the hidden activation marked private (CallContext.hidden_private) received a gradient "
                                "from somewhere else as well")
-        fuse_proj = (lazy is not None and fp == 8 and f == 64 and out_fwd is not None and ctx.post_scale is None
+        fuse_proj = (lazy is not None and fp == 8 and f == 64 and (out_fwd is not None or priv is not None) and ctx.post_scale is None
                      and ctx.head_stats is not None)
         defer = ctx.call.defer
+
+        def hidden(t):
+            return priv.materialize() if (priv is not None and priv.is_placeholder(t)) else t
         if lazy is not None and not fuse_proj:
-            proj_bwd(lazy["x"], lazy["dz"], lazy["w3"], lazy["d_w"], defer=defer, dx_out=lazy["placeholder"])
+            proj_bwd(hidden(lazy["x"]), lazy["dz"], lazy["w3"], lazy["d_w"], defer=defer, dx_out=lazy["placeholder"])
             lazy = None
+        if priv is not None and lazy is None:
+            out_fwd = priv.materialize()
         grad_out = _as_f32c(grad_out, "grad_out")
         nw = 3 * f_in * f
         d_params = torch.empty(nw + 3 * k * f + k * k, dtype=_F32, device=dev)
@@ -143,6 +183,8 @@
         _set_post(q, ctx.post_relu, ctx.post_scale, ctx.post_drop, ops.row_offset)
         if out_fwd is not None:
             q.out, q.ld_out = out_fwd.data_ptr(), out_fwd.stride(0)
+        elif priv is not None and ctx.post_keep is not None:
+            q.post_keep, q.ld_post_keep = ctx.post_keep.data_ptr(), ctx.post_keep.stride(0)
         if four:
             ps, s_local = saved[-2], saved[-1]
             gs = torch.empty(n, f, dtype=_F32, device=dev)
@@ -164,8 +206,11 @@
                     C.byref(q), _vp(ws), ws.numel() * 4, unsupported_ok=lazy is not None or carry)
         if st == EUNSUPPORTED:
             if lazy is not None:
-                proj_bwd(lazy["x"], lazy["dz"], lazy["w3"], lazy["d_w"], defer=defer, dx_out=lazy["placeholder"])
+                proj_bwd(hidden(lazy["x"]), lazy["dz"], lazy["w3"], lazy["d_w"], defer=defer, dx_out=lazy["placeholder"])
                 q.grad_out, q.proj_dz, lazy = grad_out.data_ptr(), None, None
+                if priv is not None:
+                    out_fwd = priv.materialize()
+                    q.out, q.ld_out, q.post_keep = out_fwd.data_ptr(), out_fwd.stride(0), None
             if carry:
                 q.next_a, q.next_xg, q.next_row_scale, q.next_agg = None, None, None, None
                 spmm(ops.low, pipe.table(), out=pipe.agg(), row_scale=ops.row_scale)
diff --git a/acm_gnn_amd/functional/conv_literal.py b/acm_gnn_amd/functional/conv_literal.py
--- a/acm_gnn_amd/functional/conv_literal.py
+++ b/acm_gnn_amd/functional/conv_literal.py
@@ -5,7 +5,7 @@
 from .. import _lib, tuning
 from .. import functional as _pkg
 from ..graph import SparseFeatures
-from ._context import _current_tape, _take_pre_proj
+from ._context import _current_tape, _private_of, _take_pre_proj
 from ._conv_shared import _NO_GRADS, _chan_block, _conv_prologue, _flat_views, _gathered_input, _grads, _head_params, _hop_buffer, \
     _k3_setup, _low_product, _narrow_tables, _pack_head, _reduce_replicated, _set_head, _set_post, _struc_grad, _struc_rows, \
     _unpack_head
@@ -29,6 +29,10 @@
     elif fb != f:
         ldz = -(-(2 * fb + f) // 4) * 4
     pre = _take_pre_proj(call, x, w3, cfg.relu_before) if use_proj else None
+    priv = ctx.private_in = _private_of(call, x) if not sparse_x else None
+    if priv is not None and (pre is None or ctx.in_drop is not None or ctx.hops > 1):
+        x, priv = priv.materialize(), None
+        ctx.private_in = None
     drop_spec = _drop_spec(ctx.in_drop, ops.row_offset) if ctx.in_drop is not None else None
     two_tables = (use_proj or f in (2, 4, 8) or hops > 1) and not sparse_x
     pack4 = four and f == 2 and fb == 2 and two_tables and not ops.sharded and not getattr(ops, "general", False)
@@ -339,13 +343,18 @@
           and w3[0].stride(0) == w3[1].stride(0) == w3[2].stride(0)):
         d_wcat = flat[:nw].view(3, f_in_w, f)
         prod = getattr(ctx, "lazy_producer", None)
+        priv = getattr(ctx, "private_in", None)
         if (prod is not None and f <= 2 and f_in_w == 64 and x.shape[1] == 64 and getattr(prod, "lazy", None) is None
                 and all(w.stride(0) == f and w.is_contiguous() for w in w3)):
             d_x = torch.empty(n, x.shape[1], dtype=_F32, device=dev)
             prod.lazy = dict(dz=dz, w3=w3, d_w=d_wcat, x=x, placeholder=d_x)
         else:
+            if priv is not None:
+                x = priv.materialize()
             d_x = proj_bwd(x, dz, w3, d_wcat, defer=defer)
     else:
+        if getattr(ctx, "private_in", None) is not None:
+            x = ctx.private_in.materialize()
         d_wcat = gemm(x, dz, trans_a=True, col_blocks=3,
                       out=flat[:nw].view(3, f_in_w, f),
                       a_drop=_drop_spec(ctx.in_drop, ops.row_offset) if getattr(ctx, "in_drop_used", False) else None)
diff --git a/acm_gnn_amd/layers.py b/acm_gnn_amd/layers.py
--- a/acm_gnn_amd/layers.py
+++ b/acm_gnn_amd/layers.py
@@ -129,7 +129,8 @@
         if isinstance(input, torch.Tensor) and input.layout != torch.strided:
             input = SparseFeatures.from_torch(input)
         elif (isinstance(input, torch.Tensor) and input_drop is None and not rows_permuted
-                and not (isinstance(adj_low, FilterOperators) and adj_low.sharded)):
+                and not (isinstance(adj_low, FilterOperators) and adj_low.sharded)
+                and AF._private_of(call, input) is None):
             input = self._csr_input(input)
         if isinstance(adj_low, FilterOperators):
             ops = adj_low
diff --git a/acm_gnn_amd/models.py b/acm_gnn_amd/models.py
--- a/acm_gnn_amd/models.py
+++ b/acm_gnn_amd/models.py
@@ -110,9 +110,12 @@
             xx = self._residual(x, adj_low, drop=(p, 2, st, off), call=call,
                                 pipe=call.pipe if (not isinstance(x, SparseFeatures) and piped) else None)
         call.next_proj = self.gcns[1] if self.model_type != "acmgcnpp" else None
-        fea = self.gcns[0](x, adj_low, adj_high, adj_low_unnormalized, post_relu=True, post_drop=(p, 1, st), **kw,
-                           rows_permuted=self._rows_permuted, call=call)
-        call.next_proj = None
+        call.hidden_private_next = self.model_type != "acmgcnpp"
+        try:
+            fea = self.gcns[0](x, adj_low, adj_high, adj_low_unnormalized, post_relu=True, post_drop=(p, 1, st), **kw,
+                               rows_permuted=self._rows_permuted, call=call)
+        finally:
+            call.next_proj, call.hidden_private_next = None, False
         if add_fused:
             ops_ = adj_low if isinstance(adj_low, FilterOperators) else None
             xr = x
@@ -127,7 +130,7 @@
         try:
             return self.gcns[1](fea, adj_low, adj_high, adj_low_unnormalized, rows_permuted=self._rows_permuted, call=call)
         finally:
-            call.hidden_private = None
+            call.hidden_private = call.private_out = None
 
     def _forward_snowball(self, x, adj_low, adj_high, fused, call):
         if isinstance(x, SparseFeatures):
@@ -198,9 +201,12 @@
             ones = self._ones_like_hidden(x.shape[0], self.gcns[0].out_features, x.device)
             scale = drop(ones)
         call.next_proj = self.gcns[1] if self.model_type != "acmgcnpp" else None
-        fea = self.gcns[0](x, adj_low, adj_high, adj_low_unnormalized, post_relu=True, post_scale=scale,
-                           rows_permuted=self._rows_permuted, call=call)
-        call.next_proj = None
+        call.hidden_private_next = self.model_type != "acmgcnpp"
+        try:
+            fea = self.gcns[0](x, adj_low, adj_high, adj_low_unnormalized, post_relu=True, post_scale=scale,
+                               rows_permuted=self._rows_permuted, call=call)
+        finally:
+            call.next_proj, call.hidden_private_next = None, False
         if self.model_type == "acmgcnpp":
             fea = fea + xx
         else:
@@ -208,4 +214,4 @@
         try:
             return self.gcns[1](fea, adj_low, adj_high, adj_low_unnormalized, rows_permuted=self._rows_permuted, call=call)
         finally:
-            call.hidden_private = None
+            call.hidden_private = call.private_out = None
diff --git a/acm_gnn_amd/tuning.py b/acm_gnn_amd/tuning.py
--- a/acm_gnn_amd/tuning.py
+++ b/acm_gnn_amd/tuning.py
@@ -5,13 +5,14 @@
 
 KERNEL_KEYS = ("chunk", "wide_form", "bwd_split", "rows16", "agg_fused", "gemm_forms")
 HOST_DEFAULTS = {"rewrites": 15, "implicit": 1, "relabel": -1, "pipeline": 8192, "csr_features": 256, "small_step": 16384}
-HOST_RANGES = {"rewrites": (0, 15), "implicit": (0, 1), "relabel": (-1, 1), "pipeline": (0, 1 << 31), "csr_features": (0, 1 << 31),
+HOST_RANGES = {"rewrites": (0, 31), "implicit": (0, 1), "relabel": (-1, 1), "pipeline": (0, 1 << 31), "csr_features": (0, 1 << 31),
                "small_step": (0, 16384)}
 
 REWRITE_AGG_FIRST = 1
 REWRITE_ACMII_RECOMPUTE = 2
 REWRITE_ACMII_MASK = 4
 REWRITE_AGGW_FUSED = 8
+REWRITE_PRIVATE_HIDDEN = 16
 ROWS16_EPI, ROWS16_BWD, ROWS16_LOCAL = 1, 2, 4
 GEMM_ROWS, GEMM_BX3, GEMM_BX3_WIDE, GEMM_ROWS_ALWAYS = 1, 2, 4, 8
 
diff --git a/include/acm_hip.h b/include/acm_hip.h
--- a/include/acm_hip.h
+++ b/include/acm_hip.h
@@ -8,7 +8,7 @@
 extern "C" {
 #endif
 
-#define ACM_ABI_VERSION 28
+#define ACM_ABI_VERSION 29
 
 typedef enum {
     ACM_OK = 0,
@@ -24,6 +24,7 @@
 
 int acm_version(void);
 const char* acm_last_error(void);
+extern const int32_t acm_cap_private_hidden;
 
 typedef struct {
     int32_t chunk;
@@ -322,6 +323,7 @@
     float* xs_copy;  int64_t ld_xs_copy;
     const float* next_x; int64_t ld_next_x;
     acm_dropout_t next_drop;
+    uint16_t* post_keep; int64_t ld_post_keep;
 } acm_conv_agg_fwd_t;
 
 int acm_conv_agg_fwd(const acm_csr_t* a_low, const acm_conv_agg_fwd_t* p,
@@ -359,6 +361,7 @@
     const float* proj_w_low; const float* proj_w_high; const float* proj_w_mlp; int64_t proj_ld_w;
     int32_t proj_f;
     float* proj_d_w;
+    const uint16_t* post_keep; int64_t ld_post_keep;
 } acm_conv_agg_bwd_t;
 
 int acm_conv_agg_bwd_workspace_bytes(int64_t n_rows, int f_in, int f_out, size_t* bytes);
```

Result: slower. 49.41 billion edges/s (-2.6%).
